# FuxiComputerVision/Nefii

Measured on AMD Instinct MI355X. Metric: training rays/sec (Step-2 material opt), higher is better.
Workload: dtype f16x3; 1 GPU; cfg3; parallelism=dp1, trace_tier=True, bracket_staged_eval=False, split_fp8=False, step_graph=False, cycle_batches=4, trace_prefetch=3, nonfinite_steps=0

## Files before the change

include/nefii_amd.h:

```cpp
#ifndef NEFII_AMD_H
#define NEFII_AMD_H

#include <stddef.h>
#include <stdint.h>

#ifdef __cplusplus
extern "C" {
#endif

#define NEFII_ABI_VERSION 18
#define NEFII_MAX_LAYERS 12
#define NEFII_TILE_ROWS 32
#define NEFII_MAX_WIDTH 512
#define NEFII_MAX_ENC 96
#define NEFII_MAX_LOBES 512

enum { NEFII_ACT_RELU = 0, NEFII_ACT_ELU = 1, NEFII_ACT_SOFTPLUS100 = 2 };
enum { NEFII_HEAD_NONE = 0, NEFII_HEAD_TANH01 = 1, NEFII_HEAD_POW2 = 2, NEFII_HEAD_SIGMOID = 3,
       NEFII_HEAD_RELU = 4, NEFII_HEAD_ABS = 5, NEFII_HEAD_RELU_INIT = 6 };
enum { NEFII_E_ARG = -1, NEFII_E_SHAPE = -2, NEFII_E_UNSUPPORTED = -3 };

typedef struct nefii_layer {
    int32_t k_x, k_e;
    int32_t n_out;
// ... 59 lines not shown
                        float scale, const float *gscale, float *dW, float *db, void *stream);

int nefii_mlp_h16_supported(const nefii_mlp *h_mlp);
int nefii_mlp_x0_width(const nefii_mlp *h_mlp);
int nefii_mlp_forward_f16h(const nefii_mlp *h_mlp, const float *in_a, const float *in_b, const float *in_c,
                           const float *feat, int64_t n, float *out, int out_stride, float *hidden_out, int hid_stride,
                           void *stash16, int stash_stride, float *z_last, void *x0_16, void *stream);
int nefii_mlp_backward_f16h(const nefii_mlp *h_mlp, const float *d_out, int out_stride, const void *stash16,
                            int stash_stride, const float *z_last, int64_t n, void *dz16, int dz_stride,
                            const float *scale, void *stream);
int nefii_mlp_wgrad_f16h(const void *dz16, int dz_stride, const void *x, int x_stride, int x_half, int64_t n, int n_out,
                         int k_in, float scale, const float *gscale, float *dW, float *db, void *stream);

#define NEFII_MAX_WGRAD_ITEMS 12
typedef struct nefii_wgrad_item {
    const void *dz16;
    const void *x;
    float *dW, *db;
    int32_t dz_stride, x_stride, x_half, n_out, k_in;
    float scale;
} nefii_wgrad_item;
int nefii_mlp_wgrad_f16h_batch(const nefii_wgrad_item *h_items, int n_items, int64_t n, const float *gscale, void *stream);

int nefii_encode_inputs(const nefii_mlp *h_mlp, const float *in_a, const float *in_b, const float *in_c,
                        const float *feat, int64_t n, float *out, int width, void *stream);

int nefii_sdf_value_grad(const nefii_mlp *h_mlp, const float *x, int64_t n, float *sdf_out, int out_stride,
                         float *feat_out, int feat_stride, float *grad_out, float *ws, void *stream);
size_t nefii_sdf_value_grad_workspace_bytes(const nefii_mlp *h_mlp, int64_t n);

typedef struct nefii_tracer_params {
    float object_bounding_sphere, sdf_threshold, line_search_step;
    int32_t line_step_iters, sphere_tracing_iters, n_steps, n_rootfind_steps;
    int32_t training;
    int32_t bisect_levels;
    int32_t precision;
    float coarse_tau;
    int32_t coarse_cap;
    int32_t minsdf_group;
    int32_t small_round;
    int32_t trace_tier;
    float tier_kappa;
    float tier_gate;
    float minsdf_lipschitz;
    int32_t unread_misses;
    int32_t split_fp8;
} nefii_tracer_params;
#define NEFII_TRACE_COUNTERS 14
#define NEFII_CNT_SINGLES 0
#define NEFII_CNT_DENSE_ROWS 1
#define NEFII_CNT_BISECT_RAYS 2
#define NEFII_CNT_BISECT_USED 3
#define NEFII_CNT_REFINED 4
#define NEFII_CNT_COARSE_WINDOWS 5
#define NEFII_CNT_SEARCHES 6
#define NEFII_CNT_BISECT_EVALS 7
#define NEFII_CNT_TAU_AUDIT 8
#define NEFII_CNT_COARSE_SINGLES 9
#define NEFII_CNT_REPEATS 10
#define NEFII_CNT_COARSE_SAMPLES 11
#define NEFII_CNT_LIP_AUDIT 12
#define NEFII_CNT_PROBES 13

size_t nefii_sdf_stream_bytes(const nefii_mlp *h_sdf);
int nefii_pack_sdf_stream(const nefii_mlp *h_sdf, void *w_stream, void *stream);

size_t nefii_mlp_stream_bytes(const nefii_mlp *h_mlp);
int nefii_pack_mlp_stream(const nefii_mlp *h_mlp, void *w_stream, void *stream);

int nefii_pack_linear_f16x3_bwd(const float *W, int n_out, int k_in, int x_src0, int x_len, int e_src0, int e_len,
                                float scale, void *w_bwd_f16x3, void *stream);

int nefii_sdf_eval(const nefii_mlp *h_sdf, const float *x, int64_t n, float *sdf_out, void *stream);
int nefii_sdf_eval_coarse(const nefii_mlp *h_sdf, const float *x, int64_t n, float *sdf_out, void *stream);
int nefii_sdf_coarse_supported(const nefii_mlp *h_sdf);
int nefii_sdf_eval_fp8corr(const nefii_mlp *h_sdf, const float *x, int64_t n, float *sdf_out, void *stream);
int nefii_sdf_fp8corr_supported(const nefii_mlp *h_sdf);

size_t nefii_trace_workspace_bytes(int64_t n_rays, const nefii_tracer_params *h_params);
int nefii_trace_max_rounds(const nefii_tracer_params *h_params);
int nefii_trace_rays(const nefii_mlp *h_sdf, const nefii_tracer_params *h_params,
                     const float *origins, const float *dirs, const uint8_t *object_mask, int64_t n_rays,
                     const float *lin_steps, const float *minsdf_steps,
                     float *out_points, uint8_t *out_hit, float *out_dists,
                     void *workspace, size_t workspace_bytes, int32_t *counters, void *stream);

int nefii_trace_rays_rounds(const nefii_mlp *h_sdf, const nefii_tracer_params *h_params,
                            const float *origins, const float *dirs, const uint8_t *object_mask, int64_t n_rays,
                            const float *lin_steps, const float *minsdf_steps,
                            float *out_points, uint8_t *out_hit, float *out_dists,
                            void *workspace, size_t workspace_bytes, int32_t *counters,
                            int round_begin, int round_end, void *stream);
int nefii_trace_rays_groups(const nefii_mlp *h_sdf, const nefii_tracer_params *h_params,
                            const float *origins, const float *dirs, const uint8_t *object_mask,
                            int n_groups, const int64_t *group_begin,
                            const float *lin_steps, const float *minsdf_steps,
                            float *out_points, uint8_t *out_hit, float *out_dists,
                            void *const *workspaces, const size_t *workspace_bytes, int32_t *counters,
                            int round_begin, int round_end, void *const *streams);

#define NEFII_BOUND_GRID_MAX 640
size_t nefii_sdf_bound_grid_workspace_bytes(int G);
int nefii_sdf_bound_grid_build(const nefii_mlp *h_sdf, int G, float radius, float tau, float L_floor, float safety,
                               void *out_cells, void *workspace, void *stream);
int nefii_trace_rays_rounds_grid(const nefii_mlp *h_sdf, const nefii_tracer_params *h_params,
                                 const float *origins, const float *dirs, const uint8_t *object_mask, int64_t n_rays,
                                 const float *lin_steps, const float *minsdf_steps,
                                 float *out_points, uint8_t *out_hit, float *out_dists,
                                 void *workspace, size_t workspace_bytes, int32_t *counters,
                                 int round_begin, int round_end, const void *cells, int G, void *stream);
int nefii_trace_rays_groups_grid(const nefii_mlp *h_sdf, const nefii_tracer_params *h_params,
                                 const float *origins, const float *dirs, const uint8_t *object_mask,
                                 int n_groups, const int64_t *group_begin,
                                 const float *lin_steps, const float *minsdf_steps,
                                 float *out_points, uint8_t *out_hit, float *out_dists,
                                 void *const *workspaces, const size_t *workspace_bytes, int32_t *counters,
                                 int round_begin, int round_end, const void *cells, int G, void *const *streams);

int nefii_sdf_bound_grid_build_vertices(const nefii_mlp *h_sdf, int G, float radius, float tau, float L_floor, float safety,
                                        void *out_cells, void *out_vertex_g, void *out_cell_l, void *workspace, void *stream);
int nefii_trace_rays_rounds_grid_vertices(const nefii_mlp *h_sdf, const nefii_tracer_params *h_params,
                                          const float *origins, const float *dirs, const uint8_t *object_mask, int64_t n_rays,
                                          const float *lin_steps, const float *minsdf_steps,
                                          float *out_points, uint8_t *out_hit, float *out_dists,
                                          void *workspace, size_t workspace_bytes, int32_t *counters,
                                          int round_begin, int round_end, const void *cells, int G,
                                          const void *vertex_g, const void *cell_l, void *stream);
int nefii_trace_rays_groups_grid_vertices(const nefii_mlp *h_sdf, const nefii_tracer_params *h_params,
                                          const float *origins, const float *dirs, const uint8_t *object_mask,
                                          int n_groups, const int64_t *group_begin,
                                          const float *lin_steps, const float *minsdf_steps,
                                          float *out_points, uint8_t *out_hit, float *out_dists,
                                          void *const *workspaces, const size_t *workspace_bytes, int32_t *counters,
                                          int round_begin, int round_end, const void *cells, int G,
                                          const void *vertex_g, const void *cell_l, void *const *streams);

int nefii_trace_rays_rounds_grid_training(const nefii_mlp *h_sdf, const nefii_tracer_params *h_params,
                                          const float *origins, const float *dirs, const uint8_t *object_mask, int64_t n_rays,
                                          const float *lin_steps, const float *minsdf_steps,
                                          float *out_points, uint8_t *out_hit, float *out_dists,
                                          void *workspace, size_t workspace_bytes, int32_t *counters,
                                          int round_begin, int round_end, const void *cells, int G,
                                          const void *vertex_g, const void *cell_l, int grid_training, void *stream);
int nefii_trace_rays_groups_grid_training(const nefii_mlp *h_sdf, const nefii_tracer_params *h_params,
                                          const float *origins, const float *dirs, const uint8_t *object_mask,
                                          int n_groups, const int64_t *group_begin,
                                          const float *lin_steps, const float *minsdf_steps,
                                          float *out_points, uint8_t *out_hit, float *out_dists,
                                          void *const *workspaces, const size_t *workspace_bytes, int32_t *counters,
                                          int round_begin, int round_end, const void *cells, int G,
                                          const void *vertex_g, const void *cell_l, int grid_training,
                                          void *const *streams);

int nefii_trace_profile_enable(int on);
int nefii_trace_profile_read(double *h_eval_ms, int *h_n_eval, double *h_span_ms);
int nefii_trace_profile_launches(float *h_ms, int cap);

int nefii_camera_rays(const float *uv, const float *pose, const float *intrinsics, int batch, int64_t samples,
                      float *out_dirs, float *out_origins, void *stream);


int nefii_sg_render_forward(const float *lgtSGs, int n_lobes, const float *specular, const float *roughness,
                            const float *albedo, const float *normal, const float *view, int64_t n,
                            float *rgb, float *spec_rgb, float *diff_rgb, void *stream);
int nefii_sg_render_backward(const float *lgtSGs, int n_lobes, const float *specular, const float *roughness,
                             const float *albedo, const float *normal, const float *view, int64_t n,
                             const float *d_rgb, const float *d_spec, const float *d_diff,
                             float *g_albedo, float *g_roughness, float *g_specular, float *g_lgtSGs, void *stream);

int nefii_env_radiance_forward(const float *lgtSGs, int n_lobes, const float *dirs, int64_t n, float eps,
                               float *rgb, void *stream);
int nefii_env_radiance_backward(const float *lgtSGs, int n_lobes, const float *dirs, int64_t n, float eps,
                                const float *d_rgb, float *g_lgtSGs, void *stream);

int64_t nefii_envfit_workspace_bytes(int64_t n, int n_lobes);
int nefii_envfit_loss_grad(const float *lgtSGs, int n_lobes, const float *dirs, const float *target, int64_t n, float eps,
                           void *workspace, float *loss, float *g_lgtSGs, float *rgb, void *stream);
int nefii_envfit_adam(float *lgtSGs, float *exp_avg, float *exp_avg_sq, int n_lobes, const float *dirs,
                      const float *target, int64_t n, float eps, double lr, double beta1, double beta2,
                      double adam_eps, int64_t step0, int iters, void *workspace, float *losses, void *stream);

int64_t nefii_mcubes_workspace_bytes(int nx, int ny, int nz);
int nefii_mcubes_count(const float *vol, int nx, int ny, int nz, float level, void *workspace, int64_t *counts,
                       void *stream);
int nefii_mcubes_emit(const float *vol, int nx, int ny, int nz, float level, float origin_x, float origin_y,
                      float origin_z, float spacing_x, float spacing_y, float spacing_z, void *workspace, float *verts,
                      int64_t max_verts, int *faces, int64_t max_tris, void *stream);

int nefii_mcubes_classify_bricks(const void *cells, int G, float radius, int nx, int ny, int nz, const double *frame,
                                 float level, int B, uint8_t *out_active, void *stream);
int nefii_mcubes_sparse_count(const float *vals, const int *slot_map, int n_slots, int nx, int ny, int nz, int B,
                              const int *active_list, int n_active, float level, int *counts, void *stream);
int nefii_mcubes_sparse_emit(const float *vals, const int *slot_map, int n_slots, int nx, int ny, int nz, int B,
                             const int *active_list, int n_active, float level, float origin_x, float origin_y,
                             float origin_z, float spacing_x, float spacing_y, float spacing_z, const int64_t *offsets,
                             int64_t *vert_keys, float *vert_pos, int64_t max_verts, int64_t *face_cell, int64_t *face_keys,
                             int64_t max_tris, void *stream);

int nefii_mis_sample(const float *lgtSGs, int n_lobes, const float *roughness, const float *normal, const float *view,
                     const float *uniforms, int64_t n, float *wi, float *own_pdf, float *pdf_table, void *stream);

int64_t nefii_envlight_table_bytes(int height, int width);
int nefii_envlight_build(const float *map, int height, int width, void *table, void *stream);
int nefii_envlight_mis_sample(const float *map, const void *table, int height, int width, int coord,
                              const float *roughness, const float *normal, const float *view, const float *uniforms,
                              int64_t n, float *wi, float *own_pdf, float *pdf_table, float *light, void *stream);
int nefii_envlight_radiance(const float *map, int height, int width, int coord, const float *dirs, int64_t n,
                            float *rgb, void *stream);
int nefii_envlight_pdf(const void *table, int height, int width, int coord, const float *dirs, int64_t n, float *pdf,
                       void *stream);

int nefii_envlight_bounce_sample(const float *map, const void *table, int height, int width, int coord,
                                 const float *specular, const float *roughness, const float *albedo,
                                 const float *normal, const float *view, const float *uniforms, int64_t m, float *wo,
                                 float *weight, float *mix_pdf, void *stream);

int nefii_envlight_mis_sample_rot(const float *map, const void *table, int height, int width, int coord,
                                  const float *rot, const int *rot_identity, int A, const float *roughness,
                                  const float *normal, const float *view, const float *uniforms, int64_t n, float *wi,
                                  float *own_pdf, float *pdf_table, float *light, void *stream);
int nefii_envlight_bounce_sample_rot(const float *map, const void *table, int height, int width, int coord,
                                     const float *rot, const int *rot_identity, int A, const int *rot_index,
                                     const float *specular, const float *roughness, const float *albedo,
                                     const float *normal, const float *view, const float *uniforms, int64_t m,
                                     float *wo, float *weight, float *mix_pdf, void *stream);
int nefii_envlight_radiance_rot(const float *map, int height, int width, int coord, const float *rot,
                                const int *rot_identity, int A, const int *rot_index, const float *dirs, int64_t n,
                                float *rgb, void *stream);
int nefii_envlight_pdf_rot(const void *table, int height, int width, int coord, const float *rot,
                           const int *rot_identity, int A, const int *rot_index, const float *dirs, int64_t n,
                           float *pdf, void *stream);

int nefii_denoise_atrous(const void *guides0, const void *guides1, const void *in, void *out, int n_signals, int height,
                         int width, int step, float sigma_n, float sigma_x, float sigma_c_level, void *stream);

int nefii_mesh_sdf_query(const double *node_box, int64_t n_leaves_pow2, const double *tris ,
                         int64_t n_tris, int leaf_size, const double *points, int64_t n_points, int want_sign, double *out,
                         void *stream);

int nefii_mesh_cc_init(int32_t *parent, int64_t n_verts, int32_t *flags, void *stream);
int nefii_mesh_cc_round(const int32_t *faces, int64_t n_faces, int32_t *parent, int64_t n_verts, int32_t *flags,
                        void *stream);

int nefii_mesh_cluster_quadrics(const float *verts, int64_t n_verts, const int32_t *faces, int64_t n_faces,
                                const int32_t *cluster, const int32_t *corners, const int64_t *seg, const double *centre,
                                int64_t n_clusters, double h, double eps, double clamp, float *pos, int32_t *flags,
                                void *stream);

int64_t nefii_image_metrics_workspace_bytes(int B, int H, int W, int C, int levels);
int nefii_image_metrics(const float *x, const float *y, int B, int H, int W, int C, int levels, const double *window,
                        double c1, double c2, void *workspace, double *stats, double *sq_err, void *stream);

int nefii_mc_shade_forward(const float *specular, const float *roughness, const float *albedo, const float *normal,
                           const float *view, const float *wi, const float *own_pdf, const float *pdf_table,
                           const float *light, const float *visibility, const float *indirect, int64_t n,
                           float *rgb, float *spec_rgb, float *diff_rgb, void *stream);
int nefii_mc_shade_backward(const float *specular, const float *roughness, const float *albedo, const float *normal,
                            const float *view, const float *wi, const float *own_pdf, const float *pdf_table,
                            const float *light, const float *visibility, const float *indirect, int64_t n,
                            const float *d_rgb, const float *d_spec, const float *d_diff, float *g_light,
                            float *g_indirect, float *g_albedo, float *g_roughness, float *g_specular, void *stream);

typedef struct nefii_loss_params {
    float idr_rgb_weight, sg_rgb_weight, mask_weight, alpha, normalsmooth_weight, background_rgb_weight;
    int32_t loss_type;
    int32_t env_loss_type;
    int32_t r_patch;
    int32_t reserved;
} nefii_loss_params;
int nefii_idr_loss(const nefii_loss_params *h_params, const float *idr_rgb, const float *sg_rgb, const float *rgb_gt,
                   const uint8_t *network_object_mask, const uint8_t *object_mask, const float *sdf_output,
                   const float *normals, int64_t n, float *losses, float *d_idr_rgb, float *d_sg_rgb, void *stream);

#define NEFII_PATCH_WINDOW 11
typedef struct nefii_patch_loss_params {
    float idr_ssim_weight, sg_ssim_weight, roughnesssmooth_weight;
    int32_t r_patch;
    float window[NEFII_PATCH_WINDOW];
    int32_t reserved;
} nefii_patch_loss_params;
int64_t nefii_idr_patch_loss_workspace_bytes(const nefii_patch_loss_params *h_params, int64_t n);
int nefii_idr_patch_loss(const nefii_patch_loss_params *h_params, const float *idr_rgb, const float *sg_rgb,
                         const float *rgb_gt, const uint8_t *network_object_mask, const uint8_t *object_mask,
                         const float *roughness, const float *normals, int64_t n, void *workspace, float *losses,
                         float *d_idr_rgb, float *d_sg_rgb, float *d_roughness, void *stream);

#define NEFII_MAX_ROW_BLOCKS 12
typedef struct nefii_row_block {
    const float *src;
    float *dst;
    int32_t cols;
    int32_t src_row_stride;
    float fill;
    int32_t reserved;
} nefii_row_block;
int nefii_assemble_rows(const nefii_row_block *h_blocks, int n_blocks, const int64_t *where, int64_t n_src, int64_t rows,
                        void *stream);
int nefii_gather_rows(const nefii_row_block *h_blocks, int n_blocks, const int64_t *where, int64_t n_src, int64_t rows,
                      void *stream);

int nefii_prepare_hits(const float *points, const float *ray_dirs, const float *grad, const float *feat_src, int feat_cols,
                       const int64_t *where, int64_t n, int64_t rows, float *pts_out, float *view_out, float *nrm_out,
                       float *feat_out, void *stream);

int nefii_material_head_global(const float *rough_param, const float *spec_param, int n_spec, int fake_rough, int fake_spec,
                               float *rough_out, float *spec_out, void *stream);
// ... 12 lines not shown
```

nefii_amd/_lib.py:

```python
import ctypes
import os

HERE = os.path.dirname(os.path.abspath(__file__))
LIB_PATH = os.environ.get('NEFII_LIB_PATH', os.path.join(HERE, 'csrc', 'libnefii_hip.so'))

MAX_LAYERS = 12
TILE_ROWS = 32
MAX_WIDTH = 512
MAX_ENC = 96
ABI_VERSION = 18
TRACE_COUNTERS = 14
(CNT_SINGLES, CNT_DENSE_ROWS, CNT_BISECT_RAYS, CNT_BISECT_USED, CNT_REFINED, CNT_COARSE_WINDOWS, CNT_SEARCHES, CNT_BISECT_EVALS,
 CNT_TAU_AUDIT, CNT_COARSE_SINGLES, CNT_REPEATS, CNT_COARSE_SAMPLES, CNT_LIP_AUDIT, CNT_PROBES) = range(TRACE_COUNTERS)
CNT_WORK = [CNT_SINGLES, CNT_DENSE_ROWS, CNT_BISECT_RAYS, CNT_REFINED, CNT_COARSE_WINDOWS, CNT_COARSE_SINGLES, CNT_COARSE_SAMPLES]
CNT_MAXIMA = [CNT_TAU_AUDIT, CNT_LIP_AUDIT]
TRACE_WS_FLOAT_ARRAYS = 13
TRACE_ITER_SHIFT = 20

ACT_RELU, ACT_ELU, ACT_SOFTPLUS100 = 0, 1, 2
HEAD_NONE, HEAD_TANH01, HEAD_POW2, HEAD_SIGMOID, HEAD_RELU, HEAD_ABS, HEAD_RELU_INIT = range(7)

c_float_p = ctypes.c_void_p


class Layer(ctypes.Structure):
    _fields_ = [('k_x', ctypes.c_int32), ('k_e', ctypes.c_int32), ('n_out', ctypes.c_int32),
                ('n_pad', ctypes.c_int32), ('w_fwd', ctypes.c_void_p), ('w_bwd', ctypes.c_void_p),
                ('bias', ctypes.c_void_p), ('w_f16x3', ctypes.c_void_p), ('w_bwd_f16x3', ctypes.c_void_p)]


class Mlp(ctypes.Structure):
    _fields_ = [('n_layers', ctypes.c_int32), ('act', ctypes.c_int32), ('head', ctypes.c_int32),
                ('enc_freqs', ctypes.c_int32 * 3), ('feat_width', ctypes.c_int32), ('reserved', ctypes.c_int32),
                ('w_stream', ctypes.c_void_p), ('layer', Layer * MAX_LAYERS)]


class TracerParams(ctypes.Structure):
    _fields_ = [('object_bounding_sphere', ctypes.c_float), ('sdf_threshold', ctypes.c_float),
                ('line_search_step', ctypes.c_float), ('line_step_iters', ctypes.c_int32),
                ('sphere_tracing_iters', ctypes.c_int32), ('n_steps', ctypes.c_int32),
                ('n_rootfind_steps', ctypes.c_int32), ('training', ctypes.c_int32), ('bisect_levels', ctypes.c_int32),
                ('precision', ctypes.c_int32), ('coarse_tau', ctypes.c_float), ('coarse_cap', ctypes.c_int32),
                ('minsdf_group', ctypes.c_int32), ('small_round', ctypes.c_int32), ('trace_tier', ctypes.c_int32),
                ('tier_kappa', ctypes.c_float), ('tier_gate', ctypes.c_float), ('minsdf_lipschitz', ctypes.c_float),
                ('unread_misses', ctypes.c_int32), ('split_fp8', ctypes.c_int32)]


class PackSource(ctypes.Structure):
    _fields_ = [('W', ctypes.c_void_p), ('bias', ctypes.c_void_p), ('n_out', ctypes.c_int32), ('k_in', ctypes.c_int32),
                ('x_src0', ctypes.c_int32), ('x_len', ctypes.c_int32), ('e_src0', ctypes.c_int32), ('e_len', ctypes.c_int32),
                ('scale', ctypes.c_float), ('skip_f32', ctypes.c_int32)]


class WgradItem(ctypes.Structure):
    _fields_ = [('dz16', ctypes.c_void_p), ('x', ctypes.c_void_p), ('dW', ctypes.c_void_p), ('db', ctypes.c_void_p),
                ('dz_stride', ctypes.c_int32), ('x_stride', ctypes.c_int32), ('x_half', ctypes.c_int32),
                ('n_out', ctypes.c_int32), ('k_in', ctypes.c_int32), ('scale', ctypes.c_float)]


MAX_WGRAD_ITEMS = 12


class RowBlock(ctypes.Structure):
    _fields_ = [('src', ctypes.c_void_p), ('dst', ctypes.c_void_p), ('cols', ctypes.c_int32), ('src_row_stride', ctypes.c_int32),
                ('fill', ctypes.c_float), ('reserved', ctypes.c_int32)]


MAX_ROW_BLOCKS = 12


class LossParams(ctypes.Structure):
    _fields_ = [('idr_rgb_weight', ctypes.c_float), ('sg_rgb_weight', ctypes.c_float), ('mask_weight', ctypes.c_float),
                ('alpha', ctypes.c_float), ('normalsmooth_weight', ctypes.c_float),
                ('background_rgb_weight', ctypes.c_float), ('loss_type', ctypes.c_int32),
                ('env_loss_type', ctypes.c_int32), ('r_patch', ctypes.c_int32), ('reserved', ctypes.c_int32)]


PATCH_WINDOW = 11


class PatchLossParams(ctypes.Structure):
    _fields_ = [('idr_ssim_weight', ctypes.c_float), ('sg_ssim_weight', ctypes.c_float),
                ('roughnesssmooth_weight', ctypes.c_float), ('r_patch', ctypes.c_int32),
                ('window', ctypes.c_float * PATCH_WINDOW), ('reserved', ctypes.c_int32)]


P = ctypes.c_void_p
I = ctypes.c_int
I64 = ctypes.c_int64
F = ctypes.c_float
D = ctypes.c_double

SIGNATURES = {
    'nefii_abi_version': (I, []),
    'nefii_padded_width': (I, [I]),
    'nefii_pack_linear': (I, [P, P, I, I, I, I, I, I, F, P, P, P, P]),
    'nefii_pack_linear_f16x3': (I, [P, I, I, I, I, I, I, F, P, P]),
    'nefii_pack_linear_f16x3_bwd': (I, [P, I, I, I, I, I, I, F, P, P]),
    'nefii_pack_mlp': (I, [ctypes.POINTER(Mlp), ctypes.POINTER(PackSource), P]),
    'nefii_mlp_forward': (I, [ctypes.POINTER(Mlp), P, P, P, P, I64, P, I, P, I, P, I, P]),
    'nefii_mlp_backward': (I, [ctypes.POINTER(Mlp), P, I, P, I, I64, P, I, P]),
    'nefii_mlp_wgrad': (I, [P, I, P, I, I64, I, I, F, P, P, P]),
    'nefii_mlp_forward_f16': (I, [ctypes.POINTER(Mlp), P, P, P, P, I64, P, I, P, I, P, I, I, P]),
    'nefii_mlp_grad_scale': (I, [P, I64, P, P]),
    'nefii_mlp_grad_scale_head': (I, [P, I, P, I, I64, I, I, P, P]),
    'nefii_mlp_backward_f16': (I, [ctypes.POINTER(Mlp), P, I, P, I, I64, P, I, P, P]),
    'nefii_mlp_wgrad_f16': (I, [P, I, P, I, I64, I, I, F, P, P, P, P]),
    'nefii_mlp_h16_supported': (I, [ctypes.POINTER(Mlp)]),
    'nefii_mlp_x0_width': (I, [ctypes.POINTER(Mlp)]),
    'nefii_mlp_forward_f16h': (I, [ctypes.POINTER(Mlp), P, P, P, P, I64, P, I, P, I, P, I, P, P, P]),
    'nefii_mlp_backward_f16h': (I, [ctypes.POINTER(Mlp), P, I, P, I, P, I64, P, I, P, P]),
    'nefii_mlp_wgrad_f16h': (I, [P, I, P, I, I, I64, I, I, F, P, P, P, P]),
    'nefii_mlp_wgrad_f16h_batch': (I, [ctypes.POINTER(WgradItem), I, I64, P, P]),
    'nefii_encode_inputs': (I, [ctypes.POINTER(Mlp), P, P, P, P, I64, P, I, P]),
    'nefii_sdf_value_grad': (I, [ctypes.POINTER(Mlp), P, I64, P, I, P, I, P, P, P]),
    'nefii_sdf_value_grad_workspace_bytes': (ctypes.c_size_t, [ctypes.POINTER(Mlp), I64]),
    'nefii_sdf_stream_bytes': (ctypes.c_size_t, [ctypes.POINTER(Mlp)]),
    'nefii_pack_sdf_stream': (I, [ctypes.POINTER(Mlp), P, P]),
    'nefii_mlp_stream_bytes': (ctypes.c_size_t, [ctypes.POINTER(Mlp)]),
    'nefii_pack_mlp_stream': (I, [ctypes.POINTER(Mlp), P, P]),
    'nefii_sdf_eval': (I, [ctypes.POINTER(Mlp), P, I64, P, P]),
    'nefii_sdf_eval_coarse': (I, [ctypes.POINTER(Mlp), P, I64, P, P]),
    'nefii_sdf_coarse_supported': (I, [ctypes.POINTER(Mlp)]),
    'nefii_sdf_eval_fp8corr': (I, [ctypes.POINTER(Mlp), P, I64, P, P]),
    'nefii_sdf_fp8corr_supported': (I, [ctypes.POINTER(Mlp)]),
    'nefii_trace_workspace_bytes': (ctypes.c_size_t, [I64, ctypes.POINTER(TracerParams)]),
    'nefii_trace_max_rounds': (I, [ctypes.POINTER(TracerParams)]),
    'nefii_trace_rays': (I, [ctypes.POINTER(Mlp), ctypes.POINTER(TracerParams), P, P, P, I64, P, P, P, P, P, P,
                             ctypes.c_size_t, P, P]),
    'nefii_trace_rays_rounds': (I, [ctypes.POINTER(Mlp), ctypes.POINTER(TracerParams), P, P, P, I64, P, P, P, P, P, P,
                                    ctypes.c_size_t, P, I, I, P]),
    'nefii_trace_rays_groups': (I, [ctypes.POINTER(Mlp), ctypes.POINTER(TracerParams), P, P, P, I, P, P, P, P, P, P, P, P,
                                    P, I, I, P]),
    'nefii_sdf_bound_grid_workspace_bytes': (ctypes.c_size_t, [I]),
    'nefii_sdf_bound_grid_build': (I, [ctypes.POINTER(Mlp), I, F, F, F, F, P, P, P]),
    'nefii_trace_rays_rounds_grid': (I, [ctypes.POINTER(Mlp), ctypes.POINTER(TracerParams), P, P, P, I64, P, P, P, P, P, P,
                                         ctypes.c_size_t, P, I, I, P, I, P]),
    'nefii_trace_rays_groups_grid': (I, [ctypes.POINTER(Mlp), ctypes.POINTER(TracerParams), P, P, P, I, P, P, P, P, P, P, P, P,
                                         P, I, I, P, I, P]),
    'nefii_sdf_bound_grid_build_vertices': (I, [ctypes.POINTER(Mlp), I, F, F, F, F, P, P, P, P, P]),
    'nefii_trace_rays_rounds_grid_vertices': (I, [ctypes.POINTER(Mlp), ctypes.POINTER(TracerParams), P, P, P, I64, P, P, P, P, P,
                                                  P, ctypes.c_size_t, P, I, I, P, I, P, P, P]),
    'nefii_trace_rays_groups_grid_vertices': (I, [ctypes.POINTER(Mlp), ctypes.POINTER(TracerParams), P, P, P, I, P, P, P, P, P,
                                                  P, P, P, P, I, I, P, I, P, P, P]),
    'nefii_trace_rays_rounds_grid_training': (I, [ctypes.POINTER(Mlp), ctypes.POINTER(TracerParams), P, P, P, I64, P, P, P, P, P,
                                                  P, ctypes.c_size_t, P, I, I, P, I, P, P, I, P]),
    'nefii_trace_rays_groups_grid_training': (I, [ctypes.POINTER(Mlp), ctypes.POINTER(TracerParams), P, P, P, I, P, P, P, P, P,
                                                  P, P, P, P, I, I, P, I, P, P, I, P]),
    'nefii_trace_profile_enable': (I, [I]),
    'nefii_trace_profile_read': (I, [ctypes.POINTER(ctypes.c_double), ctypes.POINTER(I), ctypes.POINTER(ctypes.c_double)]),
    'nefii_trace_profile_launches': (I, [ctypes.POINTER(ctypes.c_float), I]),
    'nefii_idr_loss': (I, [ctypes.POINTER(LossParams), P, P, P, P, P, P, P, I64, P, P, P, P]),
    'nefii_idr_patch_loss_workspace_bytes': (I64, [ctypes.POINTER(PatchLossParams), I64]),
    'nefii_idr_patch_loss': (I, [ctypes.POINTER(PatchLossParams), P, P, P, P, P, P, P, I64, P, P, P, P, P, P]),
    'nefii_camera_rays': (I, [P, P, P, I, I64, P, P, P]),
    'nefii_assemble_rows': (I, [ctypes.POINTER(RowBlock), I, P, I64, I64, P]),
    'nefii_gather_rows': (I, [ctypes.POINTER(RowBlock), I, P, I64, I64, P]),
    'nefii_prepare_hits': (I, [P, P, P, P, I, P, I64, I64, P, P, P, P, P]),
    'nefii_material_head_global': (I, [P, P, I, I, I, P, P, P]),
    'nefii_material_head_global_backward': (I, [P, P, I, I, I, P, P, P, P, P]),
    'nefii_sg_render_forward': (I, [P, I, P, P, P, P, P, I64, P, P, P, P]),
    'nefii_sg_render_backward': (I, [P, I, P, P, P, P, P, I64, P, P, P, P, P, P, P, P]),
    'nefii_env_radiance_forward': (I, [P, I, P, I64, F, P, P]),
    'nefii_env_radiance_backward': (I, [P, I, P, I64, F, P, P, P]),
    'nefii_envfit_workspace_bytes': (I64, [I64, I]),
    'nefii_envfit_loss_grad': (I, [P, I, P, P, I64, F, P, P, P, P, P]),
    'nefii_envfit_adam': (I, [P, P, P, I, P, P, I64, F, D, D, D, D, I64, I, P, P, P]),
    'nefii_mcubes_workspace_bytes': (I64, [I, I, I]),
    'nefii_mcubes_count': (I, [P, I, I, I, F, P, P, P]),
    'nefii_mcubes_emit': (I, [P, I, I, I, F, F, F, F, F, F, F, P, P, I64, P, I64, P]),
    'nefii_mcubes_classify_bricks': (I, [P, I, F, I, I, I, ctypes.POINTER(D), F, I, P, P]),
    'nefii_mcubes_sparse_count': (I, [P, P, I, I, I, I, I, P, I, F, P, P]),
    'nefii_mcubes_sparse_emit': (I, [P, P, I, I, I, I, I, P, I, F, F, F, F, F, F, F, P, P, P, I64, P, P, I64, P]),
    'nefii_mis_sample': (I, [P, I, P, P, P, P, I64, P, P, P, P]),
    'nefii_envlight_table_bytes': (I64, [I, I]),
    'nefii_envlight_build': (I, [P, I, I, P, P]),
    'nefii_envlight_mis_sample': (I, [P, P, I, I, I, P, P, P, P, I64, P, P, P, P, P]),
    'nefii_envlight_bounce_sample': (I, [P, P, I, I, I, P, P, P, P, P, P, I64, P, P, P, P]),
    'nefii_envlight_radiance': (I, [P, I, I, I, P, I64, P, P]),
    'nefii_envlight_pdf': (I, [P, I, I, I, P, I64, P, P]),
    'nefii_envlight_mis_sample_rot': (I, [P, P, I, I, I, P, P, I, P, P, P, P, I64, P, P, P, P, P]),
    'nefii_envlight_bounce_sample_rot': (I, [P, P, I, I, I, P, P, I, P, P, P, P, P, P, P, I64, P, P, P, P]),
    'nefii_envlight_radiance_rot': (I, [P, I, I, I, P, P, I, P, P, I64, P, P]),
    'nefii_envlight_pdf_rot': (I, [P, I, I, I, P, P, I, P, P, I64, P, P]),
    'nefii_denoise_atrous': (I, [P, P, P, P, I, I, I, I, F, F, F, P]),
    'nefii_image_metrics_workspace_bytes': (I64, [I, I, I, I, I]),
    'nefii_image_metrics': (I, [P, P, I, I, I, I, I, ctypes.POINTER(D), D, D, P, P, P, P]),
    'nefii_mesh_sdf_query': (I, [P, I64, P, I64, I, P, I64, I, P, P]),
    'nefii_mesh_cc_init': (I, [P, I64, P, P]),
    'nefii_mesh_cc_round': (I, [P, I64, P, I64, P, P]),
    'nefii_mesh_cluster_quadrics': (I, [P, I64, P, I64, P, P, P, P, I64, D, D, D, P, P, P]),
    'nefii_mc_shade_forward': (I, [P] * 11 + [I64, P, P, P, P]),
    'nefii_mc_shade_backward': (I, [P] * 11 + [I64] + [P] * 9),
    'nefii_mfma_sustained_probe': (I, [I, ctypes.POINTER(ctypes.c_float), ctypes.POINTER(ctypes.c_double), P]),
    'nefii_mfma_sustained_probe_chains': (I, [I, I, ctypes.POINTER(ctypes.c_float), ctypes.POINTER(ctypes.c_double), P]),
}

_lib = None


class NefiiLibraryError(RuntimeError):
    pass


def lib():
    global _lib
    if _lib is not None:
        return _lib
    if not os.path.exists(LIB_PATH):
        raise NefiiLibraryError(
            'libnefii_hip.so is not built (%s missing). Run `python -m nefii_amd.build`. '
            'There is no CPU/PyTorch fallback for the hot path.' % LIB_PATH)
    import torch
    try:
        handle = ctypes.CDLL(LIB_PATH)
    except OSError as e:
        raise NefiiLibraryError('cannot load %s: %s' % (LIB_PATH, e))
    for name, (res, args) in SIGNATURES.items():
        try:
            fn = getattr(handle, name)
        except AttributeError:
            raise NefiiLibraryError('%s does not export %s' % (LIB_PATH, name))
        fn.restype = res
        fn.argtypes = args
    if handle.nefii_abi_version() != ABI_VERSION:
        raise NefiiLibraryError('ABI version mismatch')
    _lib = handle
    return _lib


def check(rc, what):
    if rc != 0:
        raise RuntimeError('%s failed with status %d (%s)' % (
            what, rc, {-1: 'bad argument', -2: 'bad shape', -3: 'unsupported'}.get(rc, 'hipError_t')))
```

nefii_amd/csrc/nefii_tracer.hip:

```cpp
#include <cstdlib>
#include <vector>

#include "mlp_tile.h"
#include "hip_check.h"

using namespace nefii;

namespace {

enum Phase : int { PH_DONE = 0, PH_TRACE = 1, PH_SAMPLER = 2, PH_BISECT = 3, PH_MINSDF = 4, PH_SAMPLER_C = 5, PH_MINSDF_C = 6,
                   PH_SAMPLER_X = 7 };
constexpr int PH_POST = 100, PH_WAIT = -1;
constexpr int NCNT = NEFII_TRACE_COUNTERS;
constexpr int NEAR_PROBES = 6;
enum Kind : int { Q_START = 0, Q_END = 1, Q_MID = 2 };
enum Walk : int { WALK_NONE = 0, WALK_BEGIN = 1, WALK_AUDIT = 2 };

constexpr int TRACE_WS_FLOAT_ARRAYS = 13, TRACE_ITER_SHIFT = 20;
struct RayState {
    float *t_s, *t_e, *cur_s, *cur_e, *nxt_s, *nxt_e, *t_min, *t_max, *res_s, *res_e, *lo, *hi, *mid;
    int *flags;
    float *big;
    unsigned *singles;
    unsigned *dense;
    unsigned *tri;
    unsigned *cdense;
    unsigned *refine;
    unsigned *csingles;
    int *block_live;
    unsigned *crefine;
    unsigned char *ord;
};
constexpr int CREF_CAP = 76;

constexpr int F_PHASE = 0x7;
constexpr int F_LIVE_S = 1 << 3, F_LIVE_E = 1 << 4, F_PEND_S = 1 << 5, F_PEND_E = 1 << 6;
constexpr int F_STEPPED = 1 << 7;
constexpr int F_SPH = 1 << 8, F_SAMP = 1 << 9, F_HIT = 1 << 10;
constexpr int F_OWN = 1 << 11;
constexpr int F_IT_SHIFT = 12, F_IT_MASK = 0xFF;
constexpr int F_K_SHIFT = TRACE_ITER_SHIFT, F_K_MASK = 0xF;
constexpr int F_WIN_SHIFT = 24, F_WIN_MASK = 0x7;
enum SamplerWin : int {
    SW_WHOLE_ROW = 0,
    SW_WINDOW_1 = 1, SW_WINDOW_2 = 2, SW_WINDOW_3 = 3, SW_WINDOW_4 = 4,
    SW_STAGE1 = 5, SW_STAGE2 = 6,
    SW_GRID = 7
};
enum MinSdfWin : int {
    MW_ROW_IN = 0,
    MW_SECOND = 1,
    MW_STAGE1 = 2, MW_STAGE2 = 3,
    MW_ENTER = 4,
    MW_SHARED = 5
};
__device__ __forceinline__ int win_of(int fl) { return (fl >> F_WIN_SHIFT) & F_WIN_MASK; }
__device__ __forceinline__ int with_win(int fl, int w) { return (fl & ~(F_WIN_MASK << F_WIN_SHIFT)) | (w << F_WIN_SHIFT); }
constexpr int CWIN_STAGE1 = 4;
constexpr int F_CRS_S = 1 << 27, F_CRS_E = 1 << 28, F_AUD_S = 1 << 29, F_AUD_E = 1 << 30;
__host__ __device__ __forceinline__ int coarse_window(int n_steps) { return (n_steps + 3) >> 2; }

__device__ __forceinline__ float fmul(float a, float b) { return __fmul_rn(a, b); }
__device__ __forceinline__ float fadd(float a, float b) { return __fadd_rn(a, b); }
__device__ __forceinline__ float fsub(float a, float b) { return __fsub_rn(a, b); }

struct Params {
    nefii_tracer_params p;
    int64_t n;
    const float *o, *d;
    const uint8_t *obj;
    const float *lin, *steps;
    float *out_pts, *out_dist;
    uint8_t *out_hit;
    int *counters;
    int levels, tri_nodes;
    float tau;
    int cap;
    int chunk;
    float chunk_gate;
    int window;
    float tier_band;
    float tier_gate;
    float lip;
    int share;
    int stage_bracket;
    int miss_argmin;
    const unsigned *cells;
    int grid_n;
    float grid_inv_h;
    const unsigned short *vert_g, *cell_l;
    float grid_h;
    int grid_training;
    int walk_wave;
    RayState s;
};

__host__ __device__ __forceinline__ int stage1_count(int ns) { return coarse_window(ns); }
__host__ __device__ __forceinline__ int stage1_pos(int ns, int j) { return (j * (ns - 1)) / (stage1_count(ns) - 1); }
__device__ __forceinline__ bool staged_bracket(const Params &P, int64_t r) {
    return P.lip > 0.f && P.stage_bracket && (!P.p.training || P.obj[r] == 0);
}
__device__ __forceinline__ int minsdf_row(const Params &P, int64_t r) {
    const int g = P.p.minsdf_group;
    return g > 0 ? (int)(r / g) : 0;
}

__device__ __forceinline__ float minsdf_step(const Params &P, int64_t r, int i) {
    const int g = P.p.minsdf_group;
    return P.steps[(g > 0 ? (r / g) * (int64_t)P.p.n_steps : 0) + i];
}

struct Emit {
    bool qs, qe;
    bool cs, ce;
    bool qt, qd;
    int nc, cwin;
    unsigned dense_which;
    int consumed;
    int n_alg;
    int n_ref;
    unsigned cmask[4];
    int n_rep;
    bool ref_coarse;
    int walk, walk_from;
    __device__ __forceinline__ void mark(int i) {
#pragma unroll
        for (int w = 0; w < 4; ++w) cmask[w] |= (i >> 5) == w ? 1u << (i & 31) : 0u;
    }
    __device__ __forceinline__ bool marked(int i) const {
        unsigned word = 0u;
#pragma unroll
        for (int w = 0; w < 4; ++w) word = (i >> 5) == w ? cmask[w] : word;
        return (word >> (i & 31)) & 1u;
    }
    __device__ __forceinline__ void clear_marks() { cmask[0] = cmask[1] = cmask[2] = cmask[3] = 0u; }
};
enum Total : int { T_SINGLES, T_DENSE, T_TRI, T_CONSUMED, T_REFINE, T_CWINDOWS, T_ALG, T_CSINGLES, T_REP, T_CREFINE, N_TOTALS };
enum List : int { L_SINGLES, L_DENSE, L_TRI, L_REFINE, L_CDENSE, L_CSINGLES, L_CREFINE, N_LISTS };

__device__ __forceinline__ void append_queries(const Params &P, int round, unsigned ray, const Emit &e) {
    __shared__ int wtot[N_TOTALS][4];
    __shared__ int base[N_LISTS];
    const bool qs = e.qs && !e.cs, qe = e.qe && !e.ce, qcs = e.qs && e.cs, qce = e.qe && e.ce;
    const int nc = e.nc, n_ref = e.n_ref;
    const bool ref_coarse = e.ref_coarse;
    const int lane = threadIdx.x & 63, wave = threadIdx.x >> 6;
    const unsigned long long bs = __ballot(qs), be = __ballot(qe), bt = __ballot(e.qt), bd = __ballot(e.qd);
    const unsigned long long bcs = __ballot(qcs), bce = __ballot(qce);
    const unsigned long long lt = (1ull << lane) - 1ull;
    int cons = e.consumed, alg = e.n_alg, rep = e.n_rep;
#pragma unroll
    for (int o = 32; o > 0; o >>= 1) cons += __shfl_xor(cons, o), alg += __shfl_xor(alg, o), rep += __shfl_xor(rep, o);
    int incl = ref_coarse ? 0 : n_ref;
    int incl2 = ref_coarse ? n_ref : 0;
#pragma unroll
    for (int o = 1; o < 64; o <<= 1) {
        const int t = __shfl_up(incl, o), t2 = __shfl_up(incl2, o);
        if (lane >= o) incl += t, incl2 += t2;
    }
    const int wref = __shfl(incl, 63), wref2 = __shfl(incl2, 63);
    int cincl = nc;
#pragma unroll
    for (int o = 1; o < 64; o <<= 1) {
        const int t = __shfl_up(cincl, o);
        if (lane >= o) cincl += t;
    }
    const int wcoarse = __shfl(cincl, 63);
    if (lane == 0) {
        wtot[T_SINGLES][wave] = __popcll(bs) + __popcll(be);
        wtot[T_DENSE][wave] = __popcll(bd);
        wtot[T_TRI][wave] = __popcll(bt);
        wtot[T_CONSUMED][wave] = cons;
        wtot[T_REFINE][wave] = wref;
        wtot[T_CWINDOWS][wave] = wcoarse;
        wtot[T_ALG][wave] = alg;
        wtot[T_CSINGLES][wave] = __popcll(bcs) + __popcll(bce);
        wtot[T_REP][wave] = rep;
        wtot[T_CREFINE][wave] = wref2;
    }
    __syncthreads();
    if (threadIdx.x == 0) {
        int t[N_TOTALS];
        for (int i = 0; i < N_TOTALS; ++i) t[i] = wtot[i][0] + wtot[i][1] + wtot[i][2] + wtot[i][3];
        int *cnt = P.counters + round * NCNT;
        base[L_SINGLES] = t[T_SINGLES] ? atomicAdd(&cnt[NEFII_CNT_SINGLES], t[T_SINGLES]) : 0;
        base[L_DENSE] = t[T_DENSE] ? atomicAdd(&cnt[NEFII_CNT_DENSE_ROWS], t[T_DENSE]) : 0;
        base[L_TRI] = t[T_TRI] ? atomicAdd(&cnt[NEFII_CNT_BISECT_RAYS], t[T_TRI]) : 0;
        if (t[T_CONSUMED]) atomicAdd(&cnt[NEFII_CNT_BISECT_USED], t[T_CONSUMED]);
        base[L_REFINE] = t[T_REFINE] ? atomicAdd(&cnt[NEFII_CNT_REFINED], t[T_REFINE]) : 0;
        base[L_CDENSE] = t[T_CWINDOWS] ? atomicAdd(&cnt[NEFII_CNT_COARSE_WINDOWS], t[T_CWINDOWS]) : 0;
        if (t[T_ALG]) atomicAdd(&cnt[NEFII_CNT_SEARCHES], t[T_ALG]);
        if (t[T_TRI]) atomicAdd(&cnt[NEFII_CNT_BISECT_EVALS], t[T_TRI] * P.tri_nodes);
        base[L_CSINGLES] = t[T_CSINGLES] ? atomicAdd(&cnt[NEFII_CNT_COARSE_SINGLES], t[T_CSINGLES]) : 0;
        if (t[T_REP]) atomicAdd(&cnt[NEFII_CNT_REPEATS], t[T_REP]);
        base[L_CREFINE] = t[T_CREFINE] ? atomicAdd(&cnt[NEFII_CNT_COARSE_SAMPLES], t[T_CREFINE]) : 0;
    }
    __syncthreads();
    int off_s = base[L_SINGLES], off_d = base[L_DENSE], off_t = base[L_TRI], off_r = base[L_REFINE], off_c = base[L_CDENSE],
        off_cs = base[L_CSINGLES], off_r2 = base[L_CREFINE];
    for (int w = 0; w < wave; ++w) {
        off_r2 += wtot[T_CREFINE][w];
        off_s += wtot[T_SINGLES][w];
        off_d += wtot[T_DENSE][w];
        off_t += wtot[T_TRI][w];
        off_r += wtot[T_REFINE][w];
        off_c += wtot[T_CWINDOWS][w];
        off_cs += wtot[T_CSINGLES][w];
    }
    if (qs) P.s.singles[off_s + __popcll(bs & lt)] = (ray << 2) | Q_START;
    if (qe) P.s.singles[off_s + __popcll(bs) + __popcll(be & lt)] = (ray << 2) | Q_END;
    if (qcs) P.s.csingles[off_cs + __popcll(bcs & lt)] = (ray << 2) | Q_START;
    if (qce) P.s.csingles[off_cs + __popcll(bcs) + __popcll(bce & lt)] = (ray << 2) | Q_END;
    if (e.qd) P.s.dense[off_d + __popcll(bd & lt)] = (ray << 1) | e.dense_which;
    if (e.qt) P.s.tri[off_t + __popcll(bt & lt)] = ray;
    for (int k = 0; k < nc; ++k)
        P.s.cdense[off_c + cincl - nc + k] = ((unsigned)(e.cwin + k) << 29) | (ray << 1) | e.dense_which;
    if (n_ref > 0) {
        size_t o = ref_coarse ? (size_t)off_r2 + incl2 - n_ref : (size_t)off_r + incl - n_ref;
        unsigned *list = ref_coarse ? P.s.crefine : P.s.refine;
#pragma unroll
        for (int w = 0; w < 4; ++w) {
            unsigned mbits = e.cmask[w];
            while (mbits) {
                const int bit = __ffs(mbits) - 1;
                mbits &= mbits - 1;
                list[o++] = (ray << 7) | (unsigned)(32 * w + bit);
            }
        }
    }
    __syncthreads();
}

__device__ __forceinline__ float tri_depth(float lo, float hi, int j) {
    const unsigned k = (unsigned)j + 1u;
    const int level = 31 - __clz(k);
    float mid = fmul(fadd(lo, hi), 0.5f);
    for (int b = level - 1; b >= 0; --b) {
        if ((k >> b) & 1u) lo = mid; else hi = mid;
        mid = fmul(fadd(lo, hi), 0.5f);
    }
    return mid;
}

__device__ __forceinline__ void finish(const Params &P, int64_t r, float dist, bool hit) {
    const float ox = P.o[r * 3], oy = P.o[r * 3 + 1], oz = P.o[r * 3 + 2];
    const float dx = P.d[r * 3], dy = P.d[r * 3 + 1], dz = P.d[r * 3 + 2];
    P.out_dist[r] = dist;
    P.out_hit[r] = hit ? 1 : 0;
    P.out_pts[r * 3] = fadd(ox, fmul(dist, dx));
    P.out_pts[r * 3 + 1] = fadd(oy, fmul(dist, dy));
    P.out_pts[r * 3 + 2] = fadd(oz, fmul(dist, dz));
}

__global__ __launch_bounds__(128) void minsdf_order_kernel(Params P) {
    const int ns = P.p.n_steps, i = threadIdx.x;
    if (i >= ns) return;
    const float *st = P.steps + (size_t)blockIdx.x * ns;
    const float si = st[i];
    int rank = 0;
    for (int j = 0; j < ns; ++j) {
        const float sj = st[j];
        rank += (sj < si || (sj == si && j < i)) ? 1 : 0;
    }
    P.s.ord[(size_t)blockIdx.x * ns + rank] = (unsigned char)i;
}


__device__ __forceinline__ int init_ray(const Params &P, int64_t r, int round, int &fl, Emit &e) {
    const bool tier = P.tier_band > 0.f;
    const float ox = P.o[r * 3], oy = P.o[r * 3 + 1], oz = P.o[r * 3 + 2];
    const float dx = P.d[r * 3], dy = P.d[r * 3 + 1], dz = P.d[r * 3 + 2];
    const float b = fadd(fadd(fmul(dx, ox), fmul(dy, oy)), fmul(dz, oz));
    const float nrm = sqrtf(fadd(fadd(fmul(ox, ox), fmul(oy, oy)), fmul(oz, oz)));
    const float rad = P.p.object_bounding_sphere;
    const float under = fsub(fmul(b, b), fsub(fmul(nrm, nrm), fmul(rad, rad)));
    const bool sph = under > 0.f;
    float t0 = 0.f, t1 = 0.f;
    if (sph) {
        const float sq = sqrtf(under);
        t0 = fmaxf(fsub(-sq, b), 0.01f);
        t1 = fmaxf(fsub(sq, b), 0.01f);
    }
    P.s.t_s[r] = t0;
    P.s.t_e[r] = t1;
    P.s.t_min[r] = t0;
    P.s.t_max[r] = t1;
    P.s.nxt_s[r] = 0.f;
    P.s.nxt_e[r] = 0.f;
    P.s.cur_s[r] = 0.f;
    P.s.cur_e[r] = 0.f;
    fl = PH_TRACE;
    if (!sph) return PH_TRACE;
    fl |= F_SPH | F_LIVE_S | F_LIVE_E | F_PEND_S | F_PEND_E;
    e.qs = e.qe = true;
    e.cs = tier && t0 > 0.01f;
    e.ce = tier && t1 > 0.01f;
    fl |= (e.cs ? F_CRS_S : 0) | (e.ce ? F_CRS_E : 0);
    P.s.flags[r] = fl;
    return PH_WAIT;
}

__device__ __forceinline__ void begin_stage1(const Params &P, int64_t r, int from, int stage_code, int &fl, Emit &e) {
    float *v = P.s.big + (size_t)r * P.p.n_steps;
    for (int i = from; i < P.p.n_steps; ++i) v[i] = __builtin_inff();
    e.nc = 1;
    e.cwin = CWIN_STAGE1;
    fl = with_win(fl, stage_code);
}

__device__ __forceinline__ bool grid_bounds(const Params &P, int64_t r, float t, float &lo, float &hi) {
    const float rad = P.p.object_bounding_sphere, g = (float)P.grid_n;
    const float ox = P.o[r * 3], oy = P.o[r * 3 + 1], oz = P.o[r * 3 + 2];
    const float dx = P.d[r * 3], dy = P.d[r * 3 + 1], dz = P.d[r * 3 + 2];
    const float fx = fmul(fadd(fadd(ox, fmul(t, dx)), rad), P.grid_inv_h);
    const float fy = fmul(fadd(fadd(oy, fmul(t, dy)), rad), P.grid_inv_h);
    const float fz = fmul(fadd(fadd(oz, fmul(t, dz)), rad), P.grid_inv_h);
    lo = -__builtin_inff(), hi = __builtin_inff();
    if (!(fx >= 0.f && fx < g && fy >= 0.f && fy < g && fz >= 0.f && fz < g)) return false;
    const unsigned w = P.cells[((size_t)(int)fx * P.grid_n + (size_t)(int)fy) * P.grid_n + (size_t)(int)fz];
    lo = (float)__builtin_bit_cast(_Float16, (unsigned short)(w & 0xFFFFu));
    hi = (float)__builtin_bit_cast(_Float16, (unsigned short)(w >> 16));
    return true;
}

__device__ __forceinline__ bool grid_corner_bounds(const Params &P, int64_t r, float t, float &lo, float &hi) {
    const float rad = P.p.object_bounding_sphere, g = (float)P.grid_n;
    const float ox = P.o[r * 3], oy = P.o[r * 3 + 1], oz = P.o[r * 3 + 2];
    const float dx = P.d[r * 3], dy = P.d[r * 3 + 1], dz = P.d[r * 3 + 2];
    const float px = fadd(ox, fmul(t, dx)), py = fadd(oy, fmul(t, dy)), pz = fadd(oz, fmul(t, dz));
    const float fx = fmul(fadd(px, rad), P.grid_inv_h), fy = fmul(fadd(py, rad), P.grid_inv_h), fz = fmul(fadd(pz, rad), P.grid_inv_h);
    lo = -__builtin_inff(), hi = __builtin_inff();
    if (!(fx >= 0.f && fx < g && fy >= 0.f && fy < g && fz >= 0.f && fz < g)) return false;
    const int ci = (int)fx, cj = (int)fy, ck = (int)fz;
    const size_t V = (size_t)P.grid_n + 1;
    const float L = (float)__builtin_bit_cast(_Float16, P.cell_l[((size_t)ci * P.grid_n + (size_t)cj) * P.grid_n + (size_t)ck]);
    unsigned short gc[8];
#pragma unroll
    for (int c = 0; c < 4; ++c) {
        const unsigned short *row = P.vert_g + ((size_t)(ci + (c >> 1)) * V + (size_t)(cj + (c & 1))) * V + (size_t)ck;
        gc[2 * c] = row[0];
        gc[2 * c + 1] = row[1];
    }
    float ex2[2], ey2[2], ez2[2];
#pragma unroll
    for (int a = 0; a < 2; ++a) {
        const float ex = fsub(px, fadd(-rad, fmul((float)(ci + a), P.grid_h)));
        const float ey = fsub(py, fadd(-rad, fmul((float)(cj + a), P.grid_h)));
        const float ez = fsub(pz, fadd(-rad, fmul((float)(ck + a), P.grid_h)));
        ex2[a] = fmul(ex, ex), ey2[a] = fmul(ey, ey), ez2[a] = fmul(ez, ez);
    }
#pragma unroll
    for (int c = 0; c < 8; ++c) {
        const float v = (float)__builtin_bit_cast(_Float16, gc[c]);
        const float dist = fadd(sqrtf(fadd(fadd(ex2[c >> 2], ey2[(c >> 1) & 1]), ez2[c & 1])), 1e-6f);
        const float reach = fadd(fmul(L, dist), fadd(fmul(fabsf(v), 0x1p-11f), 0x1p-25f));
        lo = fmaxf(lo, fsub(v, reach));
        hi = fminf(hi, fadd(v, reach));
    }
    lo = fsub(lo, P.tau);
    hi = fadd(hi, P.tau);
    return true;
}

__device__ __forceinline__ void begin_grid_bracket(const Params &P, int64_t r, int round, int from, int &fl, Emit &e) {
    const int ns = P.p.n_steps;
    float *v = P.s.big + (size_t)r * ns;
    const float a = P.s.t_s[r], rng = fsub(P.s.t_e[r], a);
    const bool obj = P.obj[r] != 0;
    int j1 = ns;
    float U = __builtin_inff(), lo0 = 0.f;
    for (int i = 0; i < ns; ++i) {
        float lo, hi;
        if (i < from)
            lo = hi = v[i];
        else
            grid_bounds(P, r, fadd(a, fmul(P.lin[i], rng)), lo, hi);
        if (hi < -P.tau && j1 == ns) j1 = i;
        U = fminf(U, hi);
        if (i == 0) lo0 = lo;
        if (i >= from) v[i] = lo;
    }
    bool front_only = obj && j1 < ns && lo0 > 0.f;
    bool sign_only = front_only || !P.miss_argmin;
    float lim = sign_only ? 0.f : fmaxf(0.f, fadd(U, P.tau));
    int last = front_only ? j1 : ns - 1;
    if (P.vert_g) {
        for (int i = from; i <= last; ++i) {
            const float lb = v[i];
            if (fsub(lb, 1e-6f) > lim) continue;
            float lo, hi;
            if (!grid_corner_bounds(P, r, fadd(a, fmul(P.lin[i], rng)), lo, hi)) continue;
            v[i] = fmaxf(lb, lo);
            if (i == 0) lo0 = v[i];
            U = fminf(U, hi);
            if (hi < -P.tau && i < j1) {
                j1 = i;
                if (obj && lo0 > 0.f) break;
            }
        }
        front_only = obj && j1 < ns && lo0 > 0.f;
        sign_only = front_only || !P.miss_argmin;
        lim = sign_only ? 0.f : fmaxf(0.f, fadd(U, P.tau));
        last = front_only ? j1 : ns - 1;
    }
    int k = 0, n_near = 0, probe = -1;
    unsigned probe_h = ~0u;
    for (int i = from; i < ns; ++i) {
        const float lb = v[i];
        v[i] = __builtin_inff();
        if (i > last) continue;
        if (!(fsub(lb, 1e-6f) > lim)) {
            e.mark(i);
            ++k;
        } else if (n_near < NEAR_PROBES && !(fsub(lb, 1e-6f) > fadd(lim, fmul(2.f, P.tau)))) {
            e.mark(i);
            ++k, ++n_near;
        } else {
            const unsigned h = ((unsigned)r * 2654435761u) ^ ((unsigned)(i + 1) * 0x9E3779B1u);
            const unsigned hh = (h ^ (h >> 15)) * 0x85EBCA6Bu;
            if (hh < probe_h) probe_h = hh, probe = i;
        }
    }
    if (probe >= 0) {
        e.mark(probe);
        ++k, ++n_near;
    }
    if (n_near > 0) atomicAdd(P.counters + round * NCNT + NEFII_CNT_PROBES, n_near);
    if (k > 0 && k <= CREF_CAP) {
        e.n_ref = k;
        e.ref_coarse = true;
        fl = with_win(fl, SW_GRID);
    } else {
        e.clear_marks();
        e.nc = 4;
    }
}

__device__ __forceinline__ void grid_audit(const Params &P, int64_t r, int round) {
    const int ns = P.p.n_steps;
    const float *v = P.s.big + (size_t)r * ns;
    const float a = P.s.t_s[r], rng = fsub(P.s.t_e[r], a);
    float worst = 0.f;
    int n_corner = 0;
    for (int i = 0; i < ns; ++i) {
        if (!(v[i] < __builtin_inff())) continue;
// ... 93 lines not shown
    }
    const float lim2 = fadd(lim, fmul(2.f, P.tau));
    bool act[2] = {false, false}, surv[2] = {false, false}, near[2] = {false, false};
    unsigned long long S[2] = {0ull, 0ull}, N[2] = {0ull, 0ull}, Sel[2] = {0ull, 0ull};
#pragma unroll
    for (int p = 0; p < 2; ++p) {
        if (p && !two) continue;
        const int i = 64 * p + lane;
        const float x = fsub(lb[p], 1e-6f);
        act[p] = in[p] && i >= from && i <= last;
        surv[p] = act[p] && !(x > lim);
        near[p] = act[p] && !surv[p] && !(x > lim2);
        S[p] = __ballot(surv[p]);
        N[p] = __ballot(near[p]);
        if (in[p] && i >= from) v[i] = inf;
    }
    unsigned hh[2] = {~0u, ~0u};
#pragma unroll
    for (int p = 0; p < 2; ++p) {
        if (p && !two) continue;
        const int i = 64 * p + lane;
        const int before = (p ? __popcll(N[0]) : 0) + __popcll(N[p] & lt);
        const bool sel = near[p] && before < NEAR_PROBES;
        Sel[p] = __ballot(sel);
        if (act[p] && !surv[p] && !sel) {
            const unsigned h = ((unsigned)r * 2654435761u) ^ ((unsigned)(i + 1) * 0x9E3779B1u);
            hh[p] = (h ^ (h >> 15)) * 0x85EBCA6Bu;
        }
    }
    const unsigned hmin = wave_umin(hh[0] < hh[1] ? hh[0] : hh[1]);
    const unsigned long long P0 = __ballot(hh[0] == hmin), P1 = __ballot(hh[1] == hmin);
    const int probe = hmin != ~0u ? first_sample(P0, P1, -1) : -1;
    GridMarks g;
    g.m0 = S[0] | Sel[0] | (probe >= 0 && probe < 64 ? 1ull << probe : 0ull);
    g.m1 = S[1] | Sel[1] | (probe >= 64 ? 1ull << (probe - 64) : 0ull);
    g.k = __popcll(g.m0) + __popcll(g.m1);
    const int n_near = __popcll(Sel[0]) + __popcll(Sel[1]) + (probe >= 0 ? 1 : 0);
    if (lane == 0 && n_near > 0) atomicAdd(P.counters + round * NCNT + NEFII_CNT_PROBES, n_near);
    return g;
}

__device__ __forceinline__ void wave_grid_audit(const Params &P, int64_t r, int round) {
    const int ns = P.p.n_steps, lane = threadIdx.x & 63;
    const unsigned long long lt = (1ull << lane) - 1ull;
    const float *v = P.s.big + (size_t)r * ns;
    const float a = P.s.t_s[r], rng = fsub(P.s.t_e[r], a);
    const bool two = ns > 64;
    float x[2] = {0.f, 0.f}, t[2] = {0.f, 0.f}, lo[2] = {0.f, 0.f}, hi[2] = {0.f, 0.f};
    bool el[2] = {false, false};
    unsigned long long E[2] = {0ull, 0ull};
#pragma unroll
    for (int p = 0; p < 2; ++p) {
        if (p && !two) continue;
        const int i = 64 * p + lane;
        if (i < ns) x[p] = v[i];
        if (i < ns && x[p] < __builtin_inff()) {
            t[p] = fadd(a, fmul(P.lin[i], rng));
            el[p] = grid_bounds(P, r, t[p], lo[p], hi[p]);
        }
        E[p] = __ballot(el[p]);
    }
    float worst = 0.f;
#pragma unroll
    for (int p = 0; p < 2; ++p) {
        if (p && !two) continue;
        if (!el[p]) continue;
        const int before = (p ? __popcll(E[0]) : 0) + __popcll(E[p] & lt);
        if (P.vert_g && before < CREF_CAP) {
            float lo_c, hi_c;
            grid_corner_bounds(P, r, t[p], lo_c, hi_c);
            lo[p] = fmaxf(lo[p], lo_c), hi[p] = fminf(hi[p], hi_c);
        }
        worst = fmaxf(worst, fmaxf(fsub(fsub(lo[p], P.tau), x[p]), fsub(x[p], fadd(hi[p], P.tau))));
    }
    worst = wave_fmax(worst);
    if (lane == 0 && worst > 0.f) atomicMax(P.counters + round * NCNT + NEFII_CNT_LIP_AUDIT, __float_as_int(worst));
}

__device__ __forceinline__ void serve_grid_walks(const Params &P, int64_t r, int round, int &fl, Emit &e) {
    const int lane = threadIdx.x & 63;
    unsigned long long pending = __ballot(e.walk != WALK_NONE);
    while (pending) {
        const int src = __ffsll(pending) - 1;
        pending &= pending - 1;
        const int64_t rr = __builtin_amdgcn_readfirstlane((int)(r - lane) + src);
        const int kind = __builtin_amdgcn_readfirstlane(__shfl(e.walk, src));
        const int from = __builtin_amdgcn_readfirstlane(__shfl(e.walk_from, src));
        if (kind == WALK_AUDIT) {
            wave_grid_audit(P, rr, round);
            continue;
        }
        const GridMarks g = wave_grid_bracket(P, rr, round, from);
        if (lane == src) {
            if (g.k > 0 && g.k <= CREF_CAP) {
                e.cmask[0] = (unsigned)g.m0, e.cmask[1] = (unsigned)(g.m0 >> 32);
                e.cmask[2] = (unsigned)g.m1, e.cmask[3] = (unsigned)(g.m1 >> 32);
                e.n_ref = g.k;
                e.ref_coarse = true;
                fl = with_win(fl, SW_GRID);
            } else {
                e.clear_marks();
                e.nc = 4;
            }
            P.s.flags[r] = fl;
        }
    }
    e.walk = WALK_NONE;
}

__device__ __forceinline__ void begin_coarse_bracket(const Params &P, int64_t r, int round, int from, bool in_mask, int &fl, Emit &e) {
    if (P.cells && P.lip > 0.f && P.stage_bracket && (!P.p.training || (P.grid_training && in_mask))) {
        if (P.walk_wave)
            e.walk = WALK_BEGIN, e.walk_from = from;
        else
            begin_grid_bracket(P, r, round, from, fl, e);
    } else if (staged_bracket(P, r)) {
        begin_stage1(P, r, from, SW_STAGE1, fl, e);
    } else if ((P.window & 1) && in_mask) {
        e.nc = 1;
        fl = with_win(fl, SW_WINDOW_1);
    } else {
        e.nc = 4;
    }
}

__device__ __forceinline__ int end_trace(const Params &P, int64_t r, int round, int &fl, Emit &e, float t_s, float t_e,
                                         float cur_s, float cur_e, bool live_s, int it) {
    const bool coarse = P.tau > 0.f;
    const bool hit = t_s < t_e;
    fl = (fl & F_SPH) | (hit ? F_HIT : 0) | (live_s ? F_SAMP : 0) | ((it & F_K_MASK) << F_K_SHIFT);
    P.s.t_s[r] = t_s;
    P.s.t_e[r] = t_e;
    if (!live_s) {
        P.s.mid[r] = t_s;
        return PH_POST;
    }
    const bool go_coarse = coarse && 0.5f * (cur_s + cur_e + (t_e - t_s)) > 3.f * P.tau;
    if (go_coarse && P.chunk > 0 && P.obj[r] != 0 &&
        cur_s <= P.chunk_gate * (float)(P.chunk - 1) * (t_e - t_s) / (float)(P.p.n_steps - 1)) {
        fl |= PH_SAMPLER_X;
        e.n_ref = P.chunk;
        e.cmask[0] = (1u << P.chunk) - 1u;
    } else {
        fl |= go_coarse ? PH_SAMPLER_C : PH_SAMPLER;
        e.qd = !go_coarse;
        if (go_coarse) begin_coarse_bracket(P, r, round, 0, P.obj[r] != 0, fl, e);
    }
    e.n_alg = 1;
    e.dense_which = 0;
    P.s.flags[r] = fl;
    return PH_WAIT;
}

__device__ __forceinline__ int step_trace(const Params &P, int64_t r, int round, int &fl, Emit &e) {
    const nefii_tracer_params &tp = P.p;
    const bool tier = P.tier_band > 0.f;
    const float thr = tp.sdf_threshold;
    float t_s = P.s.t_s[r], t_e = P.s.t_e[r];
    float cur_s = P.s.cur_s[r], cur_e = P.s.cur_e[r];
    float nxt_s = P.s.nxt_s[r], nxt_e = P.s.nxt_e[r];
    bool live_s = fl & F_LIVE_S, live_e = fl & F_LIVE_E;
    int it = (fl >> F_IT_SHIFT) & F_IT_MASK, k = (fl >> F_K_SHIFT) & F_K_MASK;
    if (fl & F_PEND_S) nxt_s = P.s.res_s[r];
    if (fl & F_PEND_E) nxt_e = P.s.res_e[r];
    fl &= ~(F_AUD_S | F_AUD_E);
    const bool rep_s = (fl & F_PEND_S) && (fl & F_CRS_S) && !(fabsf(nxt_s) > P.tier_band);
    const bool rep_e = (fl & F_PEND_E) && (fl & F_CRS_E) && !(fabsf(nxt_e) > P.tier_band);
    if (rep_s || rep_e) {
        if (rep_s) e.qs = true, fl = (fl & ~F_CRS_S) | F_AUD_S, ++e.n_rep;
        if (rep_e) e.qe = true, fl = (fl & ~F_CRS_E) | F_AUD_E, ++e.n_rep;
        P.s.flags[r] = fl;
        return PH_WAIT;
    }
    bool wait = false;
    fl &= ~(F_CRS_S | F_CRS_E);
    if (fl & F_STEPPED) {
        const bool bad_s = nxt_s < 0.f, bad_e = nxt_e < 0.f;
        if ((bad_s || bad_e) && k < tp.line_step_iters) {
            const float back = (1.f - tp.line_search_step) / (float)(1 << k);
            fl &= ~(F_PEND_S | F_PEND_E);
            if (bad_s) {
                t_s = fsub(t_s, fmul(back, cur_s));
                e.qs = true;
                e.cs = tier && back * cur_s > P.tier_gate;
                fl |= F_PEND_S | (e.cs ? F_CRS_S : 0);
            }
            if (bad_e) {
                t_e = fadd(t_e, fmul(back, cur_e));
                e.qe = true;
                e.ce = tier && back * cur_e > P.tier_gate;
                fl |= F_PEND_E | (e.ce ? F_CRS_E : 0);
            }
            ++k;
            wait = true;
        } else {
            live_s = live_s && (t_s < t_e);
            live_e = live_e && (t_s < t_e);
        }
    }
    if (!wait) {
        cur_s = live_s ? nxt_s : 0.f;
        if (cur_s <= thr) cur_s = 0.f;
        cur_e = live_e ? nxt_e : 0.f;
        if (cur_e <= thr) cur_e = 0.f;
        live_s = live_s && (cur_s > thr);
        live_e = live_e && (cur_e > thr);
        if (it == tp.sphere_tracing_iters || !(live_s || live_e)) return end_trace(P, r, round, fl, e, t_s, t_e, cur_s, cur_e, live_s, it);
        ++it;
        t_s = fadd(t_s, cur_s);
        t_e = fsub(t_e, cur_e);
        nxt_s = 0.f;
        nxt_e = 0.f;
        k = 0;
        fl &= ~(F_PEND_S | F_PEND_E);
        if (live_s) {
            e.qs = true;
            e.cs = tier && cur_s > P.tier_gate;
            fl |= F_PEND_S | (e.cs ? F_CRS_S : 0);
        }
        if (live_e) {
            e.qe = true;
            e.ce = tier && cur_e > P.tier_gate;
            fl |= F_PEND_E | (e.ce ? F_CRS_E : 0);
        }
        fl |= F_STEPPED;
    }
    fl &= ~(F_LIVE_S | F_LIVE_E | (F_IT_MASK << F_IT_SHIFT) | (F_K_MASK << F_K_SHIFT));
    fl |= (live_s ? F_LIVE_S : 0) | (live_e ? F_LIVE_E : 0) | (it << F_IT_SHIFT) | (k << F_K_SHIFT);
    P.s.t_s[r] = t_s;
    P.s.t_e[r] = t_e;
    P.s.cur_s[r] = cur_s;
    P.s.cur_e[r] = cur_e;
    P.s.nxt_s[r] = nxt_s;
    P.s.nxt_e[r] = nxt_e;
    P.s.flags[r] = fl;
    return PH_WAIT;
}

__device__ __forceinline__ int sampler_leading(const Params &P, int64_t r, int round, int &fl, Emit &e) {
    const int ns = P.p.n_steps;
    float *v = P.s.big + (size_t)r * ns;
    int ind = -1;
    for (int i = 0; i < P.chunk; ++i)
        if (v[i] < 0.f && ind < 0) ind = i;
    if (ind >= 1) {
        for (int i = P.chunk; i < ns; ++i) v[i] = 3.0e38f;
        return PH_SAMPLER;
    }
    fl = (fl & ~F_PHASE) | PH_SAMPLER_C;
    begin_coarse_bracket(P, r, round, P.chunk, true, fl, e);
    e.dense_which = 0;
    P.s.flags[r] = fl;
    return PH_WAIT;
}

template <typename Search>
__device__ __forceinline__ bool staged_walk(const Params &P, int64_t r, int round, int &fl, Emit &e, const float *v, float Llen,
                                            bool stage1, const Search &S) {
    const int ns = P.p.n_steps;
    int *cnt = P.counters + round * NCNT;
    int ja = 0, k = 0, n_near = 0;
    float worst = 0.f;
    int probe = -1;
    unsigned probe_h = ~0u;
    for (int kk = 1; kk < ns - 1; ++kk) {
        if (kk == stage1_pos(ns, ja + 1)) {
            ++ja;
            continue;
        }
        const int ia = S.sample(stage1_pos(ns, ja)), ib = S.sample(stage1_pos(ns, ja + 1)), is = S.sample(kk);
        const float sa = S.depth(ia), sb = S.depth(ib), ss = S.depth(is);
        const float lb = fsub(fmaxf(fsub(v[ia], fmul(Llen, fsub(ss, sa))), fsub(v[ib], fmul(Llen, fsub(sb, ss)))), P.tau);
        if (stage1) {
            if (S.skip(kk, v)) continue;
            if (!(fsub(lb, 1e-6f) > S.lim)) {
                e.mark(is);
                ++k;
            } else if (n_near < NEAR_PROBES && !(fsub(lb, 1e-6f) > fadd(S.lim, fmul(2.f, P.tau)))) {
                e.mark(is);
                ++k, ++n_near;
            } else {
                const unsigned h = ((unsigned)r * 2654435761u) ^ ((unsigned)(kk + 1) * 0x9E3779B1u);
                const unsigned hh = (h ^ (h >> 15)) * 0x85EBCA6Bu;
                if (hh < probe_h) probe_h = hh, probe = is;
            }
        } else if (v[is] < __builtin_inff()) {
            worst = fmaxf(worst, fsub(fsub(lb, P.tau), v[is]));
        }
    }
    fl = with_win(fl, 0);
    if (stage1 && probe >= 0) {
        e.mark(probe);
        ++k, ++n_near;
    }
    if (stage1 && n_near > 0) atomicAdd(cnt + NEFII_CNT_PROBES, n_near);
    if (stage1 && k > 0) {
        if (k <= CREF_CAP) {
            e.n_ref = k;
            e.ref_coarse = true;
            fl = with_win(fl, Search::STAGE2);
        } else {
            e.clear_marks();
            e.nc = 4;
            e.dense_which = Search::WHICH;
        }
        P.s.flags[r] = fl;
        return true;
    }
    if (worst > 0.f) atomicMax(cnt + NEFII_CNT_LIP_AUDIT, __float_as_int(worst));
    e.clear_marks();
    return false;
}

struct BracketSearch {
    const float *lin;
    float lim;
    int last;
    static constexpr int STAGE2 = SW_STAGE2;
    static constexpr unsigned WHICH = 0;
    __device__ __forceinline__ int sample(int k) const { return k; }
    __device__ __forceinline__ float depth(int i) const { return lin[i]; }
    __device__ __forceinline__ bool skip(int k, const float *v) const { return k >= last || v[k] < __builtin_inff(); }
};

struct MinSdfSearch {
    const Params &P;
    int64_t r;
    const unsigned char *ord;
    float lim;
    static constexpr int STAGE2 = MW_STAGE2;
    static constexpr unsigned WHICH = 1;
    __device__ __forceinline__ int sample(int k) const { return ord[k]; }
    __device__ __forceinline__ float depth(int i) const { return minsdf_step(P, r, i); }
    __device__ __forceinline__ bool skip(int, const float *) const { return false; }
};

__device__ __forceinline__ int sampler_staged(const Params &P, int64_t r, int round, int &fl, Emit &e) {
    const int ns = P.p.n_steps, n1 = stage1_count(ns);
    const float *v = P.s.big + (size_t)r * ns;
    if (win_of(fl) == SW_GRID) {
        if (P.walk_wave)
            e.walk = WALK_AUDIT;
        else
            grid_audit(P, r, round);
        fl = with_win(fl, SW_WHOLE_ROW);
        return PH_SAMPLER_C;
    }
    const float Llen = fmul(P.lip, fsub(P.s.t_e[r], P.s.t_s[r]));
    const bool obj = P.obj[r] != 0;
    float best = __builtin_inff();
    int j1 = ns;
    for (int j = 0; j < n1; ++j) {
        const int i = stage1_pos(ns, j);
        best = fminf(best, v[i]);
        if (v[i] < -P.tau && j1 == ns) j1 = i;
    }
    const bool front_only = obj && j1 < ns && !(v[0] < P.tau);
    const bool sign_only = front_only || !P.miss_argmin;
    const BracketSearch S = {P.lin, sign_only ? 0.f : fmaxf(0.f, fadd(best, P.tau)), front_only ? j1 : ns - 1};
    return staged_walk(P, r, round, fl, e, v, Llen, win_of(fl) == SW_STAGE1, S) ? PH_WAIT : PH_SAMPLER_C;
}

__device__ __forceinline__ int sampler_windows(const Params &P, int64_t r, int round, int &fl, Emit &e) {
// ... 212 lines not shown
    float U = __builtin_inff();
    if (first)
        for (int i = 0; i < ns; ++i)
            if (vc[i] < __builtin_inff()) U = fminf(U, fadd(vc[i], slack(minsdf_step(P, r, i))));
    float lo_a = -__builtin_inff(), s_a = 0.f, lo_b = -__builtin_inff(), s_b = 1.f, worst = 0.f;
    int kb = -1, k = 0, n_near = 0, probe = -1;
    unsigned probe_h = ~0u;
    for (int kk = 0; kk < ns; ++kk) {
        const int is = ord[kk];
        const float ss = minsdf_step(P, r, is);
        float lb;
        if (vc[is] < __builtin_inff()) {
            lb = lo_a = fsub(vc[is], slack(ss));
            s_a = ss;
        } else {
            if (kb < kk) {
                lo_b = -__builtin_inff();
                for (kb = kk + 1; kb < ns; ++kb) {
                    const int ib = ord[kb];
                    if (vc[ib] < __builtin_inff()) {
                        s_b = minsdf_step(P, r, ib);
                        lo_b = fsub(vc[ib], slack(s_b));
                        break;
                    }
                }
            }
            lb = fmaxf(fsub(lo_a, fmul(Llen, fsub(ss, s_a))), fsub(lo_b, fmul(Llen, fsub(s_b, ss))));
        }
        if (!first) {
            if (v[is] < __builtin_inff()) worst = fmaxf(worst, fsub(fsub(lb, P.tau), v[is]));
        } else if (!(fsub(lb, 1e-6f) > U)) {
            e.mark(is);
            ++k;
        } else if (n_near < NEAR_PROBES && !(fsub(lb, 1e-6f) > fadd(U, fmul(2.f, P.tau)))) {
            e.mark(is);
            ++k, ++n_near;
        } else {
            const unsigned h = ((unsigned)r * 2654435761u) ^ ((unsigned)(kk + 1) * 0x9E3779B1u);
            const unsigned hh = (h ^ (h >> 15)) * 0x85EBCA6Bu;
            if (hh < probe_h) probe_h = hh, probe = is;
        }
    }
    if (!first) {
        if (worst > 0.f) atomicMax(cnt + NEFII_CNT_LIP_AUDIT, __float_as_int(worst));
        return true;
    }
    if (probe >= 0) {
        e.mark(probe);
        ++k, ++n_near;
    }
    if (k > stage1_count(ns)) {
        e.clear_marks();
        return false;
    }
    if (n_near > 0) atomicAdd(cnt + NEFII_CNT_PROBES, n_near);
    e.n_ref = k;
    e.ref_coarse = true;
    return true;
}

__device__ __forceinline__ int minsdf_share(const Params &P, int64_t r, int round, int ph, int fl0, int &fl, Emit &e) {
    const int lane = threadIdx.x & 63;
    const int p0 = fl0 & F_PHASE;
    const bool own = fl0 & F_OWN, stage1 = p0 == PH_MINSDF_C && win_of(fl0) == MW_STAGE1;
    const bool ready = own && (p0 == PH_DONE || p0 == PH_MINSDF || (p0 == PH_MINSDF_C && !stage1));
    const bool want = (fl & F_PHASE) == PH_MINSDF_C && win_of(fl) == MW_ENTER;
    unsigned long long mine = ~0ull;
    const int g = P.p.minsdf_group;
    if (g > 0) {
        const int64_t base = r - lane, head = (r / g) * g - base, tail = head + g - 1;
        const int lo = head > 0 ? (int)head : 0, hi = tail < 63 ? (int)tail : 63;
        mine = (hi >= 63 ? ~0ull : (1ull << (hi + 1)) - 1ull) & ~((1ull << lo) - 1ull);
    }
    const unsigned long long donors = __ballot(ready) & mine, busy = __ballot(own && stage1) & mine;
    const unsigned long long free_lanes = __ballot(want && !donors && !busy) & mine;
    if (!want) return ph;
    bool search = !donors && !busy && __ffsll(free_lanes) - 1 == lane;
    if (donors) {
        const int c = __ffsll(donors) - 1;
        if (shared_walk(P, r, r - lane + c, round, e, true))
            fl = (with_win(fl, MW_SHARED) & ~(F_IT_MASK << F_IT_SHIFT)) | (c << F_IT_SHIFT);
        else
            search = true;
    }
    if (search) {
        e.nc = 1;
        e.cwin = CWIN_STAGE1;
        fl = with_win(fl, MW_STAGE1) | F_OWN;
    }
    e.dense_which = 1;
    P.s.flags[r] = fl;
    return PH_WAIT;
}

__device__ __forceinline__ int minsdf_shared(const Params &P, int64_t r, int round, int &fl, Emit &e) {
    const int c = (fl >> F_IT_SHIFT) & F_IT_MASK;
    shared_walk(P, r, r - (threadIdx.x & 63) + c, round, e, false);
    fl = with_win(fl, MW_ROW_IN) & ~(F_IT_MASK << F_IT_SHIFT);
    return PH_MINSDF_C;
}

__device__ __forceinline__ int minsdf_second_stage(const Params &P, int64_t r, int round, int &fl, Emit &e) {
    const int ns = P.p.n_steps;
    const float *v = P.s.big + (size_t)r * ns;
    const int a = (fl >> F_IT_SHIFT) & F_IT_MASK;
    const float lim = v[a] + P.tau;
    int k = 0;
    for (int i = 0; i < ns; ++i)
        if (i != a && v[i] <= lim) {
            e.mark(i);
            ++k;
        }
    fl = with_win(fl, MW_ROW_IN) & ~(F_IT_MASK << F_IT_SHIFT);
    if (k == 0) return PH_MINSDF;
    if (k <= P.cap) e.n_ref = k; else e.qd = true;
    e.dense_which = 1;
    fl = (fl & ~F_PHASE) | PH_MINSDF;
    P.s.flags[r] = fl;
    return PH_WAIT;
}

__device__ __forceinline__ int minsdf_coarse(const Params &P, int64_t r, int round, int &fl, Emit &e) {
    const int ns = P.p.n_steps;
    const float *v = P.s.big + (size_t)r * ns;
    float vmin = v[0];
    int amin = 0;
    for (int i = 1; i < ns; ++i)
        if (v[i] < vmin) {
            vmin = v[i];
            amin = i;
        }
    const float lim = vmin + 2.f * P.tau;
    int k = 0;
    for (int i = 0; i < ns; ++i)
        if (v[i] <= lim) {
            e.mark(i);
            ++k;
        }
    if (k <= 1) return PH_MINSDF;
    if ((P.window & 2) && k >= 4 && ns <= 256) {
        e.clear_marks();
        e.mark(amin);
        e.n_ref = 1;
        fl = (with_win(fl, MW_SECOND) & ~(F_IT_MASK << F_IT_SHIFT)) | (amin << F_IT_SHIFT);
    } else {
        if (k <= P.cap) e.n_ref = k; else e.qd = true;
        e.dense_which = 1;
        fl = (fl & ~F_PHASE) | PH_MINSDF;
    }
    P.s.flags[r] = fl;
    return PH_WAIT;
}

__device__ __forceinline__ int minsdf_exact(const Params &P, int64_t r, int round, int &fl, Emit &e) {
    const int ns = P.p.n_steps;
    const float *v = P.s.big + (size_t)r * ns;
    int amin = 0;
    float vmin = v[0];
    for (int i = 1; i < ns; ++i)
        if (v[i] < vmin) {
            vmin = v[i];
            amin = i;
        }
    const float tmin = P.s.t_min[r], tmax = P.s.t_max[r];
    const float dist = fadd(fmul(minsdf_step(P, r, amin), fsub(tmax, tmin)), tmin);
    finish(P, r, dist, fl & F_HIT);
    P.s.flags[r] = (fl & ~F_PHASE) | PH_DONE;
    return PH_WAIT;
}

__global__ __launch_bounds__(256) void advance_kernel(Params P, int round) {
    const int64_t r = (int64_t)blockIdx.x * blockDim.x + threadIdx.x;
    const bool valid = r < P.n;
    if (round > 0 && P.s.block_live[blockIdx.x] == 0) return;
    Emit e = {};
    int fl = 0, fl0 = 0, ph = PH_WAIT;
    if (valid) {
        fl0 = fl = P.s.flags[r];
        ph = fl & F_PHASE;
        if (round == 0) ph = init_ray(P, r, round, fl, e);
        if (ph == PH_TRACE) ph = step_trace(P, r, round, fl, e);
        if (ph == PH_SAMPLER_X) ph = sampler_leading(P, r, round, fl, e);
        if (ph == PH_SAMPLER_C && win_of(fl) >= SW_STAGE1) ph = sampler_staged(P, r, round, fl, e);
    }
    if (P.walk_wave && P.cells) serve_grid_walks(P, r, round, fl, e);
    if (valid) {
        if (ph == PH_SAMPLER_C && win_of(fl) != SW_WHOLE_ROW) ph = sampler_windows(P, r, round, fl, e);
        if (ph == PH_SAMPLER_C) ph = sampler_coarse(P, r, round, fl, e);
        if (ph == PH_SAMPLER) ph = sampler_exact(P, r, round, fl, e);
        if (ph == PH_BISECT) ph = bisect(P, r, round, fl, e);
        if (ph == PH_POST) ph = post(P, r, round, fl, e);
    }
    if (P.share) ph = minsdf_share(P, r, round, ph, fl0, fl, e);
    if (valid) {
        if (ph == PH_MINSDF_C && win_of(fl) == MW_SHARED) ph = minsdf_shared(P, r, round, fl, e);
        if (ph == PH_MINSDF_C && (win_of(fl) == MW_STAGE1 || win_of(fl) == MW_STAGE2)) ph = minsdf_staged(P, r, round, fl, e);
        if (ph == PH_MINSDF_C && win_of(fl) == MW_SECOND) ph = minsdf_second_stage(P, r, round, fl, e);
        if (ph == PH_MINSDF_C) ph = minsdf_coarse(P, r, round, fl, e);
        if (ph == PH_MINSDF) ph = minsdf_exact(P, r, round, fl, e);
    }
    append_queries(P, round, (unsigned)r, e);
    const int alive = __syncthreads_or(valid && (P.s.flags[r] & F_PHASE) != PH_DONE);
    if (threadIdx.x == 0) P.s.block_live[blockIdx.x] = alive;
}

struct RoundWork {
    int n_single;
    int64_t n_sd, n_sdt, total;
};
__device__ __forceinline__ RoundWork round_work(const Params &P, int round) {
    const int *c = P.counters + round * NCNT;
    RoundWork w;
    w.n_single = c[NEFII_CNT_SINGLES];
    w.n_sd = (int64_t)c[NEFII_CNT_SINGLES] + (int64_t)c[NEFII_CNT_DENSE_ROWS] * P.p.n_steps;
    w.n_sdt = w.n_sd + (int64_t)c[NEFII_CNT_BISECT_RAYS] * P.tri_nodes;
    w.total = w.n_sdt + c[NEFII_CNT_REFINED];
    return w;
}

__device__ __forceinline__ float dense_depth(const Params &P, int64_t r, int i, bool minsdf) {
    if (minsdf) {
        const float tmin = P.s.t_min[r], tmax = P.s.t_max[r];
        return fadd(fmul(minsdf_step(P, r, i), fsub(tmax, tmin)), tmin);
    }
    const float a = P.s.t_s[r];
    return fadd(a, fmul(P.lin[i], fsub(P.s.t_e[r], a)));
}

__device__ __forceinline__ float3 ray_point(const Params &P, int64_t r, float t) {
    return make_float3(fadd(P.o[r * 3], fmul(t, P.d[r * 3])), fadd(P.o[r * 3 + 1], fmul(t, P.d[r * 3 + 1])),
                       fadd(P.o[r * 3 + 2], fmul(t, P.d[r * 3 + 2])));
}

__device__ __forceinline__ void put_point(float *raw, int tid, float px, float py, float pz) {
    float *rw = raw + tid * 9;
    rw[0] = px, rw[1] = py, rw[2] = pz;
    rw[3] = rw[4] = rw[5] = rw[6] = rw[7] = rw[8] = 0.f;
}

template <int ROWS>
__device__ __forceinline__ void load_points_tile(const float *__restrict__ x, int64_t n, float *__restrict__ out, int64_t tile,
                                                 float *raw, float **dest, int tid = threadIdx.x) {
    if (tid >= ROWS) return;
    const int64_t q = tile * ROWS + tid;
    float *rw = raw + tid * 9;
    const bool live = q < n;
    rw[0] = live ? x[q * 3] : 0.f, rw[1] = live ? x[q * 3 + 1] : 0.f, rw[2] = live ? x[q * 3 + 2] : 0.f;
    rw[3] = rw[4] = rw[5] = rw[6] = rw[7] = rw[8] = 0.f;
    dest[tid] = live ? out + q : nullptr;
}

template <int ROWS>
__device__ __forceinline__ void decode_tile(const Params &P, int64_t tile, const RoundWork &W, float *raw, float **dest,
                                            float *old = nullptr) {
    const int tid = threadIdx.x;
    if (tid >= ROWS) return;
    const int ns = P.p.n_steps;
    int64_t q = tile * ROWS + tid;
    float *dst = nullptr;
    float px = 0.f, py = 0.f, pz = 0.f;
    float coarse_v = __builtin_nanf("");
    if (q < W.total) {
        int64_t r;
        float t;
        if (q < W.n_single) {
            const unsigned e = P.s.singles[q];
            r = e >> 2;
            const int kind = e & 3;
            t = kind == Q_START ? P.s.t_s[r] : (kind == Q_END ? P.s.t_e[r] : P.s.mid[r]);
            dst = kind == Q_END ? &P.s.res_e[r] : &P.s.res_s[r];
            if (old && P.tier_band > 0.f && (P.s.flags[r] & (kind == Q_END ? F_AUD_E : F_AUD_S))) coarse_v = *dst;
        } else if (q >= W.n_sdt) {
            const unsigned e = P.s.refine[q - W.n_sdt];
            r = e >> 7;
            const int i = e & 127;
            const int ph = P.s.flags[r] & F_PHASE;
            t = dense_depth(P, r, i, ph == PH_MINSDF || ph == PH_MINSDF_C);
            dst = &P.s.big[(size_t)r * ns + i];
            if (old && ph != PH_SAMPLER_X) coarse_v = *dst;
        } else if (q >= W.n_sd) {
            const int64_t qq = q - W.n_sd;
            const int64_t ti = qq / P.tri_nodes;
            const int j = (int)(qq - ti * P.tri_nodes);
            r = P.s.tri[ti];
            t = tri_depth(P.s.lo[r], P.s.hi[r], j);
            dst = &P.s.big[(size_t)r * ns + j];
        } else {
            const int64_t qq = q - W.n_single;
            const int64_t di = qq / ns;
            const int i = (int)(qq - di * ns);
            const unsigned e = P.s.dense[di];
            r = e >> 1;
            t = dense_depth(P, r, i, e & 1);
            dst = &P.s.big[(size_t)r * ns + i];
        }
        const float3 p = ray_point(P, r, t);
        px = p.x, py = p.y, pz = p.z;
    }
    dest[tid] = dst;
    if (old) old[tid] = coarse_v;
    put_point(raw, tid, px, py, pz);
}

__device__ __forceinline__ int64_t coarse_work(const Params &P, int round, int64_t &n_rows) {
    const int *c = P.counters + round * NCNT;
    n_rows = (int64_t)c[NEFII_CNT_COARSE_WINDOWS] * coarse_window(P.p.n_steps);
    return n_rows + c[NEFII_CNT_COARSE_SINGLES] + c[NEFII_CNT_COARSE_SAMPLES];
}

template <int ROWS>
__device__ __forceinline__ void decode_tile_coarse(const Params &P, int round, int64_t tile, int64_t n_rows, int64_t total,
                                                   float *raw, float **dest, int tid = threadIdx.x) {
    if (tid >= ROWS) return;
    const int ns = P.p.n_steps, cw = coarse_window(ns);
    const int64_t q = tile * ROWS + tid;
    float *dst = nullptr;
    float px = 0.f, py = 0.f, pz = 0.f;
    const int64_t di = q / cw;
    const unsigned e = q < n_rows ? P.s.cdense[di] : 0u;
    int i = (int)(e >> 29) * cw + (int)(q - di * cw);
    if (q < n_rows && (e >> 29) == CWIN_STAGE1) {
        const int j = (int)(q - di * cw);
        const int64_t rr = (e & 0x1FFFFFFFu) >> 1;
        i = j >= stage1_count(ns) ? ns : (e & 1) ? P.s.ord[(size_t)minsdf_row(P, rr) * ns + stage1_pos(ns, j)] : stage1_pos(ns, j);
    }
    const int64_t n_cs = P.counters[round * NCNT + NEFII_CNT_COARSE_SINGLES];
    if (q >= n_rows + n_cs && q < total) {
        const unsigned s = P.s.crefine[q - n_rows - n_cs];
        const int64_t r = s >> 7;
        const int si = (int)(s & 127u);
        const float t = dense_depth(P, r, si, (P.s.flags[r] & F_PHASE) == PH_MINSDF_C);
        dst = &P.s.big[(size_t)r * ns + si];
        const float3 p = ray_point(P, r, t);
        px = p.x, py = p.y, pz = p.z;
    } else if (q >= n_rows && q < total) {
        const unsigned s = P.s.csingles[q - n_rows];
        const int64_t r = s >> 2;
        const bool end = (s & 3) == Q_END;
// ... 1098 lines not shown

namespace nefii {
static int vg_grid(int64_t n, int rows) {
    const int64_t n_tiles = (n + rows - 1) / rows;
    return (int)(n_tiles < 256 ? (n_tiles > 0 ? n_tiles : 1) : 256);
}
static bool vg_enabled() {
    static const bool v = env_int("NEFII_VG_STREAM", 1) != 0;
    return v;
}
size_t value_grad_stream_ws_bytes(const nefii_mlp *m, int64_t n) {
    if (!m || n <= 0 || !m->w_stream || !vg_enabled()) return 0;
    const int ft = vg_shape(m);
    if (!ft) return 0;
    const int rows = ft == 4 ? 64 : 96;
    return (size_t)vg_grid(n, rows) * (m->n_layers - 1) * 8 * (ft * rows / 16) * 64 * sizeof(float4v);
}
int value_grad_stream_launch(const nefii_mlp *m, const float *x, int64_t n, float *sdf_out, int out_stride, float *feat_out,
                             int feat_stride, float *grad_out, float *ws, hipStream_t st) {
    const int ft = m->w_stream && vg_enabled() ? vg_shape(m) : 0;
    if (!ft) return NEFII_E_UNSUPPORTED;
    const int Gw = stream_steps(m) + vg_units_bwd(m);
    if (ft == 4)
        hipLaunchKernelGGL((sdf_value_grad16q_kernel<4, 4>), dim3(vg_grid(n, 64)), dim3(512), 0, st, *m, x, n, sdf_out, out_stride,
                           feat_out, feat_stride, grad_out, reinterpret_cast<float4v *>(ws), vg_stream_offset(m), Gw);
    else
        hipLaunchKernelGGL((sdf_value_grad16q_kernel<6, 2>), dim3(vg_grid(n, 96)), dim3(512), 0, st, *m, x, n, sdf_out, out_stride,
                           feat_out, feat_stride, grad_out, reinterpret_cast<float4v *>(ws), vg_stream_offset(m), Gw);
    HIP_CHECK_LAUNCH();
    return 0;
}
}

static unsigned coarse_d_grid() {
    static const int g = env_int("NEFII_COARSE_D_GRID", 0);
    return (unsigned)(g > 0 ? g : 256);
}
static int coarse_two_groups() {
    static const int v = env_int("NEFII_COARSE_D", 0);
    return v;
}
static int coarse_qt() {
    static const int q = env_int("NEFII_COARSE_QT", 0);
    return q == 4 || q == 6 || q == 8 ? q : 0;
}
static int coarse_rows(int ft) {
    const int q = coarse_qt();
    if (ft == 2) return 96;
    return 16 * (q ? q : 4);
}
static dim3 points_grid(int64_t n, int rows) {
    const int64_t n_tiles = (n + rows - 1) / rows;
    return dim3((int)(n_tiles < 512 ? n_tiles : 512));
}
#define NEFII_COARSE_LAUNCH(KERNEL, KERNEL_D, ft, grid, st, ...)                                                    \
    do {                                                                                                            \
        const int rows_ = coarse_rows(ft);                                                                          \
        if ((ft) == 2)                                                                                              \
            hipLaunchKernelGGL((KERNEL<6, 2>), grid, dim3(512), 0, st, __VA_ARGS__);                                \
        else if (rows_ == 64 && coarse_two_groups())                                                                \
            hipLaunchKernelGGL((KERNEL_D<4>), dim3((grid).x < coarse_d_grid() ? (grid).x : coarse_d_grid()), dim3(512), 0, st, \
                               __VA_ARGS__);                                                                    \
        else if (rows_ == 64)                                                                                       \
            hipLaunchKernelGGL((KERNEL<4, 4>), grid, dim3(512), 0, st, __VA_ARGS__);                                \
        else if (rows_ == 96)                                                                                       \
            hipLaunchKernelGGL((KERNEL<6, 4, false>), grid, dim3(512), 0, st, __VA_ARGS__);                         \
        else                                                                                                        \
            hipLaunchKernelGGL((KERNEL<8, 4, false>), grid, dim3(512), 0, st, __VA_ARGS__);                         \
    } while (0)

extern "C" int nefii_sdf_eval_coarse(const nefii_mlp *h_sdf, const float *x, int64_t n, float *sdf_out, void *stream) {
    if (!h_sdf || h_sdf->n_layers < 1 || h_sdf->n_layers > NEFII_MAX_LAYERS) return NEFII_E_ARG;
    if (!nefii_sdf_coarse_supported(h_sdf)) return NEFII_E_UNSUPPORTED;
    if (n <= 0) return 0;
    if (!x || !sdf_out) return NEFII_E_ARG;
    if (!sdf_net_ok(h_sdf)) return NEFII_E_UNSUPPORTED;
    const int ft = shape16p(h_sdf);
    const dim3 grid = points_grid(n, coarse_rows(ft));
    NEFII_COARSE_LAUNCH(sdf_points_kernel16s, sdf_points_kernel16d, ft, grid, (hipStream_t)stream, *h_sdf, x, n, sdf_out);
    HIP_CHECK_LAUNCH();
    return 0;
}

namespace {
constexpr int GRID_SLAB = 8;

__global__ __launch_bounds__(256) void grid_points_kernel(int G, float radius, float h, int i0, int planes, float *__restrict__ x) {
    const int V = G + 1;
    const int64_t n = (int64_t)planes * V * V;
    for (int64_t q = (int64_t)blockIdx.x * blockDim.x + threadIdx.x; q < n; q += (int64_t)gridDim.x * blockDim.x) {
        const int k = (int)(q % V), j = (int)((q / V) % V), i = i0 + (int)(q / ((int64_t)V * V));
        x[q * 3] = fadd(-radius, fmul((float)i, h));
        x[q * 3 + 1] = fadd(-radius, fmul((float)j, h));
        x[q * 3 + 2] = fadd(-radius, fmul((float)k, h));
    }
}

__device__ __forceinline__ unsigned short half_toward(float x, bool up) {
    const _Float16 hv = (_Float16)x;
    unsigned short bits = __builtin_bit_cast(unsigned short, hv);
    const bool wrong = up ? (float)hv < x : (float)hv > x;
    if (wrong) {
        const bool pos = !(bits & 0x8000u);
        if ((bits & 0x7FFFu) == 0)
            bits = up ? 0x0001u : 0x8001u;
        else
            bits = (unsigned short)(pos == up ? bits + 1 : bits - 1);
    }
    return bits;
}

__global__ __launch_bounds__(256) void grid_cells_kernel(int G, float h, float tau, float l_floor, float safety,
                                                         const float *__restrict__ g, unsigned *__restrict__ cells,
                                                         unsigned short *__restrict__ cell_l) {
    const int V = G + 1;
    const int64_t n = (int64_t)G * G * G;
    const float reach = (float)((double)h * 0.8660254037844386);
    for (int64_t c = (int64_t)blockIdx.x * blockDim.x + threadIdx.x; c < n; c += (int64_t)gridDim.x * blockDim.x) {
        const int k = (int)(c % G), j = (int)((c / G) % G), i = (int)(c / ((int64_t)G * G));
        auto at = [&](int a, int b, int d) { return g[((int64_t)a * V + b) * V + d]; };
        float lo = __builtin_inff(), hi = -__builtin_inff();
        float ux = -__builtin_inff(), uy = ux, uz = ux, dx = __builtin_inff(), dy = dx, dz = dx;
        auto edge = [&](float &u, float &d, float next, float here) {
            const float s = __fdiv_rn(fsub(next, here), h);
            u = fmaxf(u, s), d = fminf(d, s);
        };
        for (int a = i - 1; a <= i + 2; ++a)
            for (int b = j - 1; b <= j + 2; ++b)
                for (int d = k - 1; d <= k + 2; ++d) {
                    if (a < 0 || a > G || b < 0 || b > G || d < 0 || d > G) continue;
                    const float v = at(a, b, d);
                    if (a >= i && a <= i + 1 && b >= j && b <= j + 1 && d >= k && d <= k + 1) lo = fminf(lo, v), hi = fmaxf(hi, v);
                    if (a < i + 2 && a < G) edge(ux, dx, at(a + 1, b, d), v);
                    if (b < j + 2 && b < G) edge(uy, dy, at(a, b + 1, d), v);
                    if (d < k + 2 && d < G) edge(uz, dz, at(a, b, d + 1), v);
                }
        const float sx = fmaxf(fabsf(ux), fabsf(dx)), sy = fmaxf(fabsf(uy), fabsf(dy)), sz = fmaxf(fabsf(uz), fabsf(dz));
        const float slope = fmaxf(fmaxf(sx, sy), sz);
        const float lcell = fmaxf(fmul(safety, slope), l_floor);
        const float slack = fadd(tau, fmul(lcell, reach));
        cells[c] = (unsigned)half_toward(fsub(lo, slack), false) | ((unsigned)half_toward(fadd(hi, slack), true) << 16);
        if (cell_l) {
            const float mx = fadd(sx, fsub(ux, dx)), my = fadd(sy, fsub(uy, dy)), mz = fadd(sz, fsub(uz, dz));
            const float norm = sqrtf(fadd(fadd(fmul(mx, mx), fmul(my, my)), fmul(mz, mz)));
            cell_l[c] = half_toward(fmaxf(fmul(safety, norm), l_floor), true);
        }
    }
}

__global__ __launch_bounds__(256) void grid_vertex_half_kernel(int64_t n, const float *__restrict__ g, unsigned short *__restrict__ out) {
    for (int64_t q = (int64_t)blockIdx.x * blockDim.x + threadIdx.x; q < n; q += (int64_t)gridDim.x * blockDim.x)
        out[q] = __builtin_bit_cast(unsigned short, (_Float16)g[q]);
}
}

extern "C" size_t nefii_sdf_bound_grid_workspace_bytes(int G) {
    if (G < 2 || G > NEFII_BOUND_GRID_MAX) return 0;
    const size_t V = (size_t)G + 1;
    return align256(sizeof(float) * V * V * V) + align256(sizeof(float) * 3 * GRID_SLAB * V * V);
}

extern "C" int nefii_sdf_bound_grid_build(const nefii_mlp *h_sdf, int G, float radius, float tau, float L_floor, float safety,
                                          void *out_cells, void *workspace, void *stream) {
    return nefii_sdf_bound_grid_build_vertices(h_sdf, G, radius, tau, L_floor, safety, out_cells, nullptr, nullptr, workspace, stream);
}

extern "C" int nefii_sdf_bound_grid_build_vertices(const nefii_mlp *h_sdf, int G, float radius, float tau, float L_floor,
                                                   float safety, void *out_cells, void *out_vertex_g, void *out_cell_l,
                                                   void *workspace, void *stream) {
    if (!h_sdf || !out_cells || !workspace || h_sdf->n_layers < 1 || h_sdf->n_layers > NEFII_MAX_LAYERS) return NEFII_E_ARG;
    if (!out_vertex_g != !out_cell_l) return NEFII_E_ARG;
    if (!(radius > 0.f && radius < 1e6f) || !(tau >= 0.f && tau < 1e6f) || !(L_floor > 0.f && L_floor < 1e6f) ||
        !(safety > 0.f && safety < 1e6f))
        return NEFII_E_ARG;
    if (G < 2 || G > NEFII_BOUND_GRID_MAX) return NEFII_E_SHAPE;
    if (!nefii_sdf_coarse_supported(h_sdf) || !sdf_net_ok(h_sdf)) return NEFII_E_UNSUPPORTED;
    hipStream_t st = (hipStream_t)stream;
    const int V = G + 1;
    const float h = (float)(2.0 * (double)radius / (double)G);
    float *g = (float *)workspace;
    float *x = (float *)((char *)workspace + align256(sizeof(float) * (size_t)V * V * V));
    const int ft = shape16p(h_sdf);
    for (int i0 = 0; i0 < V; i0 += GRID_SLAB) {
        const int planes = V - i0 < GRID_SLAB ? V - i0 : GRID_SLAB;
        const int64_t n = (int64_t)planes * V * V;
        hipLaunchKernelGGL(grid_points_kernel, dim3((int)((n + 255) / 256 < 1024 ? (n + 255) / 256 : 1024)), dim3(256), 0, st, G,
                           radius, h, i0, planes, x);
        HIP_CHECK_LAUNCH();
        const dim3 grid = points_grid(n, coarse_rows(ft));
        float *out = g + (size_t)i0 * V * V;
        NEFII_COARSE_LAUNCH(sdf_points_kernel16s, sdf_points_kernel16d, ft, grid, st, *h_sdf, (const float *)x, n, out);
        HIP_CHECK_LAUNCH();
    }
    const int64_t n_cells = (int64_t)G * G * G;
    hipLaunchKernelGGL(grid_cells_kernel, dim3((int)((n_cells + 255) / 256 < 4096 ? (n_cells + 255) / 256 : 4096)), dim3(256), 0,
                       st, G, h, tau, L_floor, safety, (const float *)g, (unsigned *)out_cells, (unsigned short *)out_cell_l);
    HIP_CHECK_LAUNCH();
    if (out_vertex_g) {
        const int64_t n_vert = (int64_t)V * V * V;
        hipLaunchKernelGGL(grid_vertex_half_kernel, dim3((int)((n_vert + 255) / 256 < 4096 ? (n_vert + 255) / 256 : 4096)), dim3(256),
                           0, st, n_vert, (const float *)g, (unsigned short *)out_vertex_g);
        HIP_CHECK_LAUNCH();
    }
    return 0;
}

extern "C" int nefii_sdf_eval_fp8corr(const nefii_mlp *h_sdf, const float *x, int64_t n, float *sdf_out, void *stream) {
    if (!h_sdf || !x || !sdf_out || n < 0) return NEFII_E_ARG;
    if (!nefii_sdf_fp8corr_supported(h_sdf)) return NEFII_E_UNSUPPORTED;
    for (int l = 0; l < h_sdf->n_layers; ++l)
        if (!h_sdf->layer[l].w_f16x3) return NEFII_E_ARG;
    if (n == 0) return 0;
    hipLaunchKernelGGL(sdf_points_kernel16f, points_grid(n, 64), dim3(512), 0, (hipStream_t)stream, *h_sdf, x, n, sdf_out,
                       (const void *)((const char *)h_sdf->w_stream + stream_bytes_1to4(h_sdf)));
    HIP_CHECK_LAUNCH();
    return 0;
}

extern "C" int nefii_sdf_eval(const nefii_mlp *h_sdf, const float *x, int64_t n, float *sdf_out, void *stream) {
    if (!h_sdf || h_sdf->n_layers < 1 || h_sdf->n_layers > NEFII_MAX_LAYERS) return NEFII_E_ARG;
    if (n <= 0) return 0;
    if (!x || !sdf_out) return NEFII_E_ARG;
    if (!sdf_net_ok(h_sdf)) return NEFII_E_UNSUPPORTED;
    for (int l = 0; l < h_sdf->n_layers; ++l)
        if (!h_sdf->layer[l].w_f16x3 || !h_sdf->layer[l].bias) return NEFII_E_ARG;
    const dim3 grid = points_grid(n, TILE_W);
    hipStream_t st = (hipStream_t)stream;
    const int ft = fits16p(h_sdf);
    if (ft == 2)
        hipLaunchKernelGGL(sdf_points_kernel16q<2>, grid, dim3(512), 0, st, *h_sdf, x, n, sdf_out);
    else if (ft && h_sdf->reserved == 1)
        hipLaunchKernelGGL(sdf_points_kernel16q<4>, grid, dim3(512), 0, st, *h_sdf, x, n, sdf_out);
    else if (ft)
        hipLaunchKernelGGL(sdf_points_kernel16p<P16W>, grid, dim3(64 * P16W), 0, st, *h_sdf, x, n, sdf_out);
    else
        hipLaunchKernelGGL(sdf_points_kernel16w, grid, dim3(WG_W), 0, st, *h_sdf, x, n, sdf_out);
    HIP_CHECK_LAUNCH();
    return 0;
}

static int coarse_cap(const nefii_tracer_params *p) {
    if (!(p->coarse_tau > 0.f)) return 0;
    const int c = p->coarse_cap <= 0 ? 64 : p->coarse_cap;
    return c > 100 ? 100 : c;
}

static bool minsdf_staged(const nefii_tracer_params *p) {
    return p->coarse_tau > 0.f && p->minsdf_lipschitz > 0.f && p->n_steps >= 16 && p->n_steps <= 128;
}

static int trace_rounds(const nefii_tracer_params *p) {
    const int trace = 1 + p->sphere_tracing_iters * (1 + p->line_step_iters);
    return trace * (p->coarse_tau > 0.f && p->trace_tier ? 2 : 1);
}

static bool minsdf_share_fits(const nefii_tracer_params *p) {
    return nefii_trace_max_rounds(p) - 1 - trace_rounds(p) >= 6;
}

extern "C" int nefii_trace_max_rounds(const nefii_tracer_params *p) {
    if (!p) return 0;
    const int L = p->bisect_levels >= 1 && p->bisect_levels <= 5 ? p->bisect_levels : 3;
    const int trace = 1 + p->sphere_tracing_iters * (1 + p->line_step_iters);
    return trace + 1 + (p->n_rootfind_steps + L - 1) / L + 1 + 2 +
           (p->coarse_tau > 0.f ? 3 + 3 + 1 + (p->trace_tier ? trace : 0) : 0) + (minsdf_staged(p) ? 1 : 0);
}

extern "C" size_t nefii_trace_workspace_bytes(int64_t n_rays, const nefii_tracer_params *p) {
    if (!p || n_rays <= 0) return 0;
    RayState s;
    size_t bytes = carve(s, nullptr, n_rays, p->n_steps, coarse_cap(p), minsdf_staged(p) ? minsdf_rows(n_rays, p) : 0);
    bytes += align256(sizeof(int) * NCNT * (size_t)nefii_trace_max_rounds(p));
    return bytes;
}

struct TraceJob {
    Params P;
    const nefii_mlp *sdf;
    int precision, rounds, adv_blocks, eval_blocks, eval_blocks_w;
    int pipelined;
    int coarse;
    const void *f8;
    hipStream_t st;
    int32_t *counters;
};

int prepare_job(TraceJob &J, const nefii_mlp *h_sdf, const nefii_tracer_params *h_params, const float *origins,
                const float *dirs, const uint8_t *object_mask, int64_t n_rays, const float *lin_steps,
                const float *minsdf_steps, float *out_points, uint8_t *out_hit, float *out_dists, void *workspace,
                size_t workspace_bytes, int32_t *counters, bool reset, void *stream, const void *cells, int grid_n,
                const void *vertex_g, const void *cell_l, int grid_training) {
    if (!h_sdf || !h_params || !origins || !dirs || !object_mask || !lin_steps || !out_points || !out_hit ||
        !out_dists || !workspace)
        return NEFII_E_ARG;
    if (n_rays <= 0 || n_rays >= (1ll << 29)) return NEFII_E_SHAPE;
    if (h_params->training && !minsdf_steps) return NEFII_E_ARG;
    const int levels = h_params->bisect_levels >= 1 && h_params->bisect_levels <= 5 ? h_params->bisect_levels : 3;
    if (h_params->bisect_levels < 0 || h_params->bisect_levels > 5) return NEFII_E_ARG;
    if (h_params->n_steps < (1 << levels) || h_params->sphere_tracing_iters > 250 || h_params->line_step_iters > 15 ||
        h_params->n_rootfind_steps > 250)
        return NEFII_E_SHAPE;
    if (h_params->sphere_tracing_iters < 0 || h_params->line_step_iters < 0 || h_params->n_rootfind_steps < 0)
        return NEFII_E_SHAPE;
    if (!sdf_net_ok(h_sdf)) return NEFII_E_UNSUPPORTED;
    if (workspace_bytes < nefii_trace_workspace_bytes(n_rays, h_params)) return NEFII_E_SHAPE;
    if (h_params->precision < 0 || h_params->precision > 2) return NEFII_E_ARG;
    if (h_params->precision >= 1)
        for (int l = 0; l < h_sdf->n_layers; ++l)
            if (!h_sdf->layer[l].w_f16x3) return NEFII_E_ARG;
    J.sdf = h_sdf;
    J.st = (hipStream_t)stream;
    J.precision = h_params->precision;
    J.rounds = nefii_trace_max_rounds(h_params);
    J.counters = counters;
    Params &P = J.P;
    P.p = *h_params;
    P.n = n_rays;
    P.o = origins;
    P.d = dirs;
    P.obj = object_mask;
    P.lin = lin_steps;
    P.steps = minsdf_steps ? minsdf_steps : lin_steps;
    if (!minsdf_steps) P.p.minsdf_group = 0;
    P.out_pts = out_points;
    P.out_dist = out_dists;
    P.out_hit = out_hit;
    J.pipelined = h_params->precision == 2 ? fits16p(h_sdf) : 0;
    if (h_params->split_fp8 < 0 || h_params->split_fp8 > 1) return NEFII_E_ARG;
    J.f8 = (h_params->split_fp8 && J.pipelined == 4 && nefii_sdf_fp8corr_supported(h_sdf))
               ? (const void *)((const char *)h_sdf->w_stream + stream_bytes_1to4(h_sdf)) : nullptr;
    J.coarse = h_params->coarse_tau > 0.f && J.pipelined && nefii_sdf_coarse_supported(h_sdf) &&
               n_rays < (1ll << 25) && h_params->n_steps <= 128;
    if (h_params->coarse_tau < 0.f || h_params->coarse_tau > 1.f) return NEFII_E_ARG;
    P.tau = J.coarse ? h_params->coarse_tau : 0.f;
    P.cap = coarse_cap(h_params);
    P.chunk = 0;
    P.chunk_gate = 1e30f;
    P.window = 0;
    P.tier_band = 0.f;
    P.tier_gate = 0.f;
    if (h_params->trace_tier < 0 || h_params->trace_tier > 1 || h_params->tier_kappa < 0.f || h_params->tier_gate < 0.f)
        return NEFII_E_ARG;
    if (J.coarse && h_params->trace_tier) {
        const float kappa = h_params->tier_kappa > 0.f ? h_params->tier_kappa : 2.f;
        const float band = kappa * P.tau, least = P.tau + 2.f * fabsf(h_params->sdf_threshold);
        P.tier_band = band > least ? band : least;
        P.tier_gate = (h_params->tier_gate > 0.f ? h_params->tier_gate : 4.f) * P.tau;
    }
    if (J.coarse && h_params->n_steps >= 16) {
        P.window = env_int("NEFII_SAMPLER_WINDOW", 2 | (n_rays >= 32768 ? 1 : 0)) & 3;
    }
    if (J.coarse) {
        const int c = env_int("NEFII_SAMPLER_CHUNK", 6);
        P.chunk = (c >= 2 && c <= 31 && c <= P.cap && c < h_params->n_steps) ? c : 0;
        P.chunk_gate = env_float("NEFII_SAMPLER_CHUNK_GATE", 1.0f);
    }
    if (h_params->minsdf_lipschitz < 0.f || h_params->minsdf_lipschitz > 1e6f) return NEFII_E_ARG;
    const bool staged = J.coarse && minsdf_staged(h_params);
    P.lip = staged ? h_params->minsdf_lipschitz : 0.f;
    P.share = staged && h_params->training && minsdf_share_fits(h_params) && env_int("NEFII_MINSDF_SHARE", 1) != 0;
    static const int stage_bracket = env_int("NEFII_BRACKET_STAGED", 1) != 0;
    P.stage_bracket = stage_bracket;
    if (h_params->unread_misses < 0 || h_params->unread_misses > 1) return NEFII_E_ARG;
    P.miss_argmin = !(h_params->unread_misses && !h_params->training);
    if (cells && (grid_n < 1 || grid_n > NEFII_BOUND_GRID_MAX)) return NEFII_E_SHAPE;
    P.cells = staged ? (const unsigned *)cells : nullptr;
    P.grid_n = grid_n;
    P.grid_inv_h = (float)((double)grid_n / (2.0 * (double)h_params->object_bounding_sphere));
    if (!vertex_g != !cell_l || (vertex_g && !cells)) return NEFII_E_ARG;
    P.vert_g = P.cells ? (const unsigned short *)vertex_g : nullptr;
    P.cell_l = P.cells ? (const unsigned short *)cell_l : nullptr;
    P.grid_training = grid_training;
    P.grid_h = grid_n > 0 ? (float)(2.0 * (double)h_params->object_bounding_sphere / (double)grid_n) : 0.f;
    P.walk_wave = env_int("NEFII_GRID_WALK_WAVE", 1) != 0;
    const int64_t step_rows = minsdf_staged(h_params) ? minsdf_rows(n_rays, &P.p) : 0;
    size_t off = carve(P.s, (char *)workspace, n_rays, h_params->n_steps, P.cap, step_rows);
    P.counters = (int *)((char *)workspace + off);
    P.levels = levels;
    P.tri_nodes = (1 << levels) - 1;
    if (reset) {
        hipError_t e = hipMemsetAsync(P.counters, 0, sizeof(int) * NCNT * J.rounds, J.st);
        if (e != hipSuccess) return (int)e;
        e = hipMemsetAsync(P.s.flags, 0, sizeof(int) * n_rays, J.st);
        if (e != hipSuccess) return (int)e;
        if (staged && h_params->training) {
            hipLaunchKernelGGL(minsdf_order_kernel, dim3((int)minsdf_rows(n_rays, &P.p)), dim3(128), 0, J.st, P);
            HIP_CHECK_LAUNCH();
        }
    }
    J.adv_blocks = (int)((n_rays + 255) / 256);
    const int64_t max_q = n_rays * (int64_t)h_params->n_steps;
    const int64_t max_tiles = (max_q + TILE - 1) / TILE;
    J.eval_blocks = (int)(max_tiles < 1024 ? max_tiles : 1024);
    const int64_t max_tiles_w = (max_q + TILE_W - 1) / TILE_W;
    static const int eval_grid = env_int("NEFII_EVAL_GRID", 0);
    const int grid_cap = eval_grid > 0 ? eval_grid : 2048;
    J.eval_blocks_w = (int)(max_tiles_w < grid_cap ? max_tiles_w : grid_cap);
    return 0;
}

int launch_round(const TraceJob &J, int r, bool profile) {
    hipStream_t st = J.st;
    hipLaunchKernelGGL(advance_kernel, dim3(J.adv_blocks), dim3(256), 0, st, J.P, r);
    HIP_CHECK_LAUNCH();
    if (r + 1 < J.rounds) {
        hipEvent_t e0 = nullptr, e1 = nullptr;
        if (profile) {
            e0 = prof_event();
            e1 = prof_event();
            (void)hipEventRecord(e0, st);
        }
        const int64_t small_tiles = (J.P.n * 2 + 31) / 32 < 256 ? (J.P.n * 2 + 31) / 32 : 256;
        const dim3 big_grid(J.eval_blocks_w), small_grid((int)(small_tiles < 1 ? 1 : small_tiles));
        auto pair = [&](auto big, auto small, int block, const auto &...args) -> int {
            hipLaunchKernelGGL(big, big_grid, dim3(block), 0, st, args...);
            HIP_CHECK_LAUNCH();
            hipLaunchKernelGGL(small, small_grid, dim3(block), 0, st, args...);
            return 0;
        };
        int rc = 0;
        const bool split = J.precision == 2, q_layout = J.sdf->reserved == 1;
        if (split && J.pipelined == 2)
            rc = pair(eval_kernel16q<6, 2>, eval_kernel16q<2, 2>, 512, J.P, *J.sdf, r);
        else if (split && J.pipelined && q_layout && J.f8)
            rc = pair(eval_kernel16f<4>, eval_kernel16f<2>, 512, J.P, *J.sdf, r, J.f8);
        else if (split && J.pipelined && q_layout && J.P.n <= 1024)
            rc = pair(eval_kernel16q<4, 4>, eval_kernel16q<2, 4, true>, 512, J.P, *J.sdf, r);
        else if (split && J.pipelined && q_layout)
            rc = pair(eval_kernel16q<4, 4>, eval_kernel16q<2, 4>, 512, J.P, *J.sdf, r);
        else if (split && J.pipelined)
            rc = pair(eval_kernel16p<P16W, 2>, eval_kernel16p<P16W, 1>, 64 * P16W, J.P, *J.sdf, r);
        else if (split)
            hipLaunchKernelGGL(eval_kernel16w, big_grid, dim3(WG_W), 0, st, J.P, *J.sdf, r);
        else if (J.precision == 1)
            hipLaunchKernelGGL(eval_kernel16, dim3(J.eval_blocks), dim3(WG), 0, st, J.P, *J.sdf, r);
        else
            hipLaunchKernelGGL(eval_kernel, dim3(J.eval_blocks), dim3(WG), 0, st, J.P, *J.sdf, r);
        if (rc) return rc;
        HIP_CHECK_LAUNCH();
        if (J.coarse) {
            const int ft = J.pipelined == 2 ? 2 : 4, rows = coarse_rows(ft);
            const int64_t t = (J.P.n * (int64_t)(4 * coarse_window(J.P.p.n_steps) + 2) + rows - 1) / rows;
            const dim3 grid((int)(t < J.eval_blocks_w ? t : J.eval_blocks_w));
            NEFII_COARSE_LAUNCH(eval_kernel16s, eval_kernel16d, ft, grid, st, J.P, *J.sdf, r);
            HIP_CHECK_LAUNCH();
        }
        if (profile) (void)hipEventRecord(e1, st);
    }
    return 0;
}

int finish_job(const TraceJob &J) {
    if (J.counters) {
        hipError_t e = hipMemcpyAsync(J.counters, J.P.counters, sizeof(int) * NCNT * J.rounds, hipMemcpyDeviceToDevice, J.st);
        if (e != hipSuccess) return (int)e;
    }
    return 0;
}

extern "C" int nefii_trace_rays_rounds_grid_training(const nefii_mlp *h_sdf, const nefii_tracer_params *h_params,
                                                     const float *origins, const float *dirs, const uint8_t *object_mask,
                                                     int64_t n_rays, const float *lin_steps, const float *minsdf_steps,
                                                     float *out_points, uint8_t *out_hit, float *out_dists, void *workspace,
                                                     size_t workspace_bytes, int32_t *counters, int round_begin, int round_end,
                                                     const void *cells, int G, const void *vertex_g, const void *cell_l,
                                                     int grid_training, void *stream) {
    if (grid_training < 0 || grid_training > 1) return NEFII_E_ARG;
    if (n_rays == 0 && h_sdf && h_params) return 0;
    TraceJob J;
    int rc = prepare_job(J, h_sdf, h_params, origins, dirs, object_mask, n_rays, lin_steps, minsdf_steps, out_points,
                         out_hit, out_dists, workspace, workspace_bytes, counters, round_begin == 0, stream, cells, G, vertex_g,
                         cell_l, grid_training);
    if (rc) return rc;
    if (round_end <= 0 || round_end > J.rounds) round_end = J.rounds;
    if (round_begin < 0 || round_begin >= round_end) return NEFII_E_ARG;
    if (g_prof.on) {
        if (!g_prof.t0) {
            (void)hipEventCreate(&g_prof.t0);
            (void)hipEventCreate(&g_prof.t1);
        }
        (void)hipEventRecord(g_prof.t0, J.st);
    }
    for (int r = round_begin; r < round_end; ++r) {
        rc = launch_round(J, r, g_prof.on);
        if (rc) return rc;
    }
    if (g_prof.on) {
        (void)hipEventRecord(g_prof.t1, J.st);
        g_prof.have_span = true;
    }
    return finish_job(J);
}

extern "C" int nefii_trace_rays_rounds_grid_vertices(const nefii_mlp *h_sdf, const nefii_tracer_params *h_params,
                                                     const float *origins, const float *dirs, const uint8_t *object_mask,
                                                     int64_t n_rays, const float *lin_steps, const float *minsdf_steps,
                                                     float *out_points, uint8_t *out_hit, float *out_dists, void *workspace,
                                                     size_t workspace_bytes, int32_t *counters, int round_begin, int round_end,
                                                     const void *cells, int G, const void *vertex_g, const void *cell_l,
                                                     void *stream) {
    return nefii_trace_rays_rounds_grid_training(h_sdf, h_params, origins, dirs, object_mask, n_rays, lin_steps, minsdf_steps,
                                                 out_points, out_hit, out_dists, workspace, workspace_bytes, counters, round_begin,
                                                 round_end, cells, G, vertex_g, cell_l, 0, stream);
}

extern "C" int nefii_trace_rays_rounds_grid(const nefii_mlp *h_sdf, const nefii_tracer_params *h_params,
                                            const float *origins, const float *dirs, const uint8_t *object_mask,
                                            int64_t n_rays, const float *lin_steps, const float *minsdf_steps,
                                            float *out_points, uint8_t *out_hit, float *out_dists, void *workspace,
                                            size_t workspace_bytes, int32_t *counters, int round_begin, int round_end,
                                            const void *cells, int G, void *stream) {
    return nefii_trace_rays_rounds_grid_vertices(h_sdf, h_params, origins, dirs, object_mask, n_rays, lin_steps, minsdf_steps,
                                                 out_points, out_hit, out_dists, workspace, workspace_bytes, counters, round_begin,
                                                 round_end, cells, G, nullptr, nullptr, stream);
}

extern "C" int nefii_trace_rays_rounds(const nefii_mlp *h_sdf, const nefii_tracer_params *h_params,
                                       const float *origins, const float *dirs, const uint8_t *object_mask,
                                       int64_t n_rays, const float *lin_steps, const float *minsdf_steps,
                                       float *out_points, uint8_t *out_hit, float *out_dists, void *workspace,
                                       size_t workspace_bytes, int32_t *counters, int round_begin, int round_end,
                                       void *stream) {
    return nefii_trace_rays_rounds_grid(h_sdf, h_params, origins, dirs, object_mask, n_rays, lin_steps, minsdf_steps, out_points,
                                        out_hit, out_dists, workspace, workspace_bytes, counters, round_begin, round_end, nullptr,
                                        0, stream);
}

extern "C" int nefii_trace_rays_groups_grid_training(const nefii_mlp *h_sdf, const nefii_tracer_params *h_params,
                                                     const float *origins, const float *dirs, const uint8_t *object_mask,
                                                     int n_groups, const int64_t *group_begin, const float *lin_steps,
                                                     const float *minsdf_steps, float *out_points, uint8_t *out_hit,
                                                     float *out_dists, void *const *workspaces, const size_t *workspace_bytes,
                                                     int32_t *counters, int round_begin, int round_end, const void *cells, int G,
                                                     const void *vertex_g, const void *cell_l, int grid_training,
                                                     void *const *streams) {
    if (grid_training < 0 || grid_training > 1) return NEFII_E_ARG;
    if (n_groups < 1 || n_groups > 16 || !group_begin || !workspaces || !workspace_bytes || !streams) return NEFII_E_ARG;
    if (!h_params) return NEFII_E_ARG;
    TraceJob J[16];
    const int rounds = nefii_trace_max_rounds(h_params);
    if (round_end <= 0 || round_end > rounds) round_end = rounds;
    if (round_begin < 0 || round_begin >= round_end) return NEFII_E_ARG;
    for (int g = 0; g < n_groups; ++g) {
        const int64_t lo = group_begin[g], n = group_begin[g + 1] - lo;
        if (lo < 0 || n <= 0) return NEFII_E_ARG;
        int rc = prepare_job(J[g], h_sdf, h_params, origins + 3 * lo, dirs + 3 * lo, object_mask + lo, n, lin_steps,
                             minsdf_steps, out_points + 3 * lo, out_hit + lo, out_dists + lo, workspaces[g],
                             workspace_bytes[g], counters ? counters + (size_t)g * rounds * NCNT : nullptr,
                             round_begin == 0, streams[g], cells, G, vertex_g, cell_l, grid_training);
        if (rc) return rc;
    }
    for (int r = round_begin; r < round_end; ++r)
        for (int g = 0; g < n_groups; ++g) {
            int rc = launch_round(J[g], r, false);
            if (rc) return rc;
        }
    for (int g = 0; g < n_groups; ++g) {
        int rc = finish_job(J[g]);
        if (rc) return rc;
    }
    return 0;
}

extern "C" int nefii_trace_rays_groups_grid_vertices(const nefii_mlp *h_sdf, const nefii_tracer_params *h_params,
                                                     const float *origins, const float *dirs, const uint8_t *object_mask,
                                                     int n_groups, const int64_t *group_begin, const float *lin_steps,
                                                     const float *minsdf_steps, float *out_points, uint8_t *out_hit,
                                                     float *out_dists, void *const *workspaces, const size_t *workspace_bytes,
                                                     int32_t *counters, int round_begin, int round_end, const void *cells, int G,
                                                     const void *vertex_g, const void *cell_l, void *const *streams) {
    return nefii_trace_rays_groups_grid_training(h_sdf, h_params, origins, dirs, object_mask, n_groups, group_begin, lin_steps,
                                                 minsdf_steps, out_points, out_hit, out_dists, workspaces, workspace_bytes,
                                                 counters, round_begin, round_end, cells, G, vertex_g, cell_l, 0, streams);
}

extern "C" int nefii_trace_rays_groups_grid(const nefii_mlp *h_sdf, const nefii_tracer_params *h_params,
                                            const float *origins, const float *dirs, const uint8_t *object_mask,
                                            int n_groups, const int64_t *group_begin, const float *lin_steps,
                                            const float *minsdf_steps, float *out_points, uint8_t *out_hit,
                                            float *out_dists, void *const *workspaces, const size_t *workspace_bytes,
                                            int32_t *counters, int round_begin, int round_end, const void *cells, int G,
                                            void *const *streams) {
    return nefii_trace_rays_groups_grid_vertices(h_sdf, h_params, origins, dirs, object_mask, n_groups, group_begin, lin_steps,
                                                 minsdf_steps, out_points, out_hit, out_dists, workspaces, workspace_bytes,
                                                 counters, round_begin, round_end, cells, G, nullptr, nullptr, streams);
}

extern "C" int nefii_trace_rays_groups(const nefii_mlp *h_sdf, const nefii_tracer_params *h_params,
                                       const float *origins, const float *dirs, const uint8_t *object_mask,
                                       int n_groups, const int64_t *group_begin, const float *lin_steps,
                                       const float *minsdf_steps, float *out_points, uint8_t *out_hit,
                                       float *out_dists, void *const *workspaces, const size_t *workspace_bytes,
                                       int32_t *counters, int round_begin, int round_end, void *const *streams) {
    return nefii_trace_rays_groups_grid(h_sdf, h_params, origins, dirs, object_mask, n_groups, group_begin, lin_steps,
                                        minsdf_steps, out_points, out_hit, out_dists, workspaces, workspace_bytes, counters,
                                        round_begin, round_end, nullptr, 0, streams);
}

extern "C" int nefii_trace_rays(const nefii_mlp *h_sdf, const nefii_tracer_params *h_params, const float *origins,
                                const float *dirs, const uint8_t *object_mask, int64_t n_rays, const float *lin_steps,
                                const float *minsdf_steps, float *out_points, uint8_t *out_hit, float *out_dists,
                                void *workspace, size_t workspace_bytes, int32_t *counters, void *stream) {
    return nefii_trace_rays_rounds(h_sdf, h_params, origins, dirs, object_mask, n_rays, lin_steps, minsdf_steps,
                                   out_points, out_hit, out_dists, workspace, workspace_bytes, counters, 0, 0, stream);
}

__global__ void camera_rays_kernel(const float *__restrict__ uv, const float *__restrict__ pose,
                                   const float *__restrict__ K, int batch, int64_t samples, float *__restrict__ dirs,
                                   float *__restrict__ origins) {
    const int64_t total = (int64_t)batch * samples;
    for (int64_t i = (int64_t)blockIdx.x * blockDim.x + threadIdx.x; i < total; i += (int64_t)gridDim.x * blockDim.x) {
        const int b = (int)(i / samples);
        const float *Kb = K + b * 16, *Pb = pose + b * 16;
        const float fx = Kb[0], sk = Kb[1], cx = Kb[2], fy = Kb[5], cy = Kb[6];
        const float u = uv[i * 2], v = uv[i * 2 + 1];
        const float x = __fdiv_rn(fsub(fadd(fsub(u, cx), __fdiv_rn(fmul(cy, sk), fy)), __fdiv_rn(fmul(sk, v), fy)), fx);
        const float y = __fdiv_rn(fsub(v, cy), fy);
        float w[3];
        for (int c = 0; c < 3; ++c) {
            const float wc = fadd(fadd(fadd(fmul(Pb[c * 4], x), fmul(Pb[c * 4 + 1], y)), Pb[c * 4 + 2]), Pb[c * 4 + 3]);
            w[c] = fsub(wc, Pb[c * 4 + 3]);
        }
        const float nrm = fmaxf(sqrtf(fadd(fadd(fmul(w[0], w[0]), fmul(w[1], w[1])), fmul(w[2], w[2]))), 1e-12f);
        for (int c = 0; c < 3; ++c) {
            dirs[i * 3 + c] = __fdiv_rn(w[c], nrm);
            origins[i * 3 + c] = Pb[c * 4 + 3];
        }
    }
}

extern "C" int nefii_camera_rays(const float *uv, const float *pose, const float *intrinsics, int batch,
                                 int64_t samples, float *out_dirs, float *out_origins, void *stream) {
    if (!uv || !pose || !intrinsics || !out_dirs || !out_origins) return NEFII_E_ARG;
    const int64_t total = (int64_t)batch * samples;
    if (total <= 0) return 0;
    int blocks = (int)((total + 255) / 256 < 2048 ? (total + 255) / 256 : 2048);
    hipLaunchKernelGGL(camera_rays_kernel, dim3(blocks), dim3(256), 0, (hipStream_t)stream, uv, pose, intrinsics, batch,
                       samples, out_dirs, out_origins);
    HIP_CHECK_LAUNCH();
    return 0;
}
```

nefii_amd/model/implicit_differentiable_renderer.py:

```python
import math
import os

import numpy as np
import torch
import torch.nn as nn

from .. import ops
from ..utils import rend_util
from .ray_tracing import RayTracing
from .sample_network import SampleNetwork
from .sg_envmap_material import EnvmapMaterialNetwork
from .sg_render import render_with_sg


def _params_version(module):
    return tuple((p.data_ptr(), p._version) for p in _plist(module))


_plist = ops.param_list


class ImplicitNetwork(nn.Module):

    def __init__(self, feature_vector_size, d_in, d_out, dims, geometric_init=True, bias=1.0, skip_in=(),
                 weight_norm=True, multires=0, use_last_as_f=False):
        super().__init__()
        if use_last_as_f:
            assert feature_vector_size == dims[-1]
        assert d_in == 3
        self.feature_vector_size = feature_vector_size
        self.cfg = dict(d_in=d_in, d_out=d_out, dims=list(dims), skip_in=list(skip_in), multires=multires,
                        use_last_as_f=use_last_as_f)
        self.specs, self.enc = ops.sdf_specs(self.cfg, feature_vector_size)
        self.num_layers = len(self.specs) + 1
        self.skip_in = skip_in
        self.use_last_as_f = use_last_as_f
        self.weight_norm = weight_norm
        d0 = self.specs[0].k_in
        for l, s in enumerate(self.specs):
            lin = nn.Linear(s.k_in, s.n_out)
            if geometric_init:
                if l == len(self.specs) - 1:
                    nn.init.normal_(lin.weight, mean=np.sqrt(np.pi) / np.sqrt(s.k_in), std=0.0001)
                    nn.init.constant_(lin.bias, -bias)
                else:
                    nn.init.constant_(lin.bias, 0.0)
                    nn.init.normal_(lin.weight, 0.0, np.sqrt(2) / np.sqrt(s.n_out))
                    if multires > 0 and l == 0:
                        nn.init.constant_(lin.weight[:, 3:], 0.0)
                    elif multires > 0 and l in skip_in:
                        nn.init.constant_(lin.weight[:, -(d0 - 3):], 0.0)
            if weight_norm:
                lin = nn.utils.weight_norm(lin)
            setattr(self, 'lin' + str(l), lin)
        self._pm = None
        self._pm_version = None
        self._pm_fit = None
        self._tau = None
        self.coarse_audit_max = 0.0
        self.coarse_audit_events = []
        self._lip = None
        self._grid = None

    def coarse_tau(self, radius=1.0):
        pm = self.packed(f16x3=True)
        if self._tau is None or self._tau[0] != self._pm_version or self._tau[1] != radius:
            self._tau = (self._pm_version, radius, ops.calibrate_coarse_tau(pm, radius))
        return self._tau[2]

    def minsdf_lipschitz(self, radius=1.0):
        self.packed(f16x3=True)
        if self._lip is None or self._lip[0] != self._pm_version or self._lip[1] != radius:
            with torch.no_grad():
                self._lip = (self._pm_version, radius, ops.calibrate_lipschitz(self.gradient, _plist(self)[0].device, radius))
        return self._lip[2]

    def bound_grid(self, radius=1.0, G=None, vertices=False):
        pm = self.packed(f16x3=True)
        tau = self.coarse_tau(radius)
        if not tau > 0.0 or not self.minsdf_lipschitz(radius) > 0.0:
            return (None, None) if vertices else None
        G = int(G or ops.BOUND_GRID_SIZE)
        key = (self._pm_version, radius, tau, G)
        if self._grid is None or self._grid[:4] != key or (vertices and self._grid[5] is None):
            built = ops.build_bound_grid(pm, radius, tau, G, vertices=vertices)
            self._grid = key + (built if vertices else (built, None))
        return self._grid[4:6] if vertices else self._grid[4]

    def note_lipschitz_audit(self, violation, lip_used):
        if violation <= 0.0 or lip_used <= 0.0 or self._lip is None or self._lip[0] != self._pm_version or self._lip[2] <= 0.0:
            return
        import warnings
        warnings.warn('staged min-SDF search of the tracer disabled for this network: a depth lay %.3e below the lower bound '
                      'its claimed Lipschitz constant %.3f gives' % (violation, lip_used))
        self._lip = (self._pm_version, self._lip[1], 0.0)
        self._grid = None
        self.coarse_audit_events.append(('lipschitz_disabled', float(violation), float(lip_used)))

    def note_coarse_audit(self, observed, tau_used, radius=1.0):
        self.coarse_audit_max = max(self.coarse_audit_max, float(observed))
        if self._tau is None or self._tau[0] != self._pm_version or self._tau[2] <= 0.0 or tau_used <= 0.0:
            return
        tau = self._tau[2]
        if observed > tau_used:
            import warnings
            warnings.warn('coarse pass of the tracer disabled for this network: a refined sample differed from its '
                          'single-pass value by %.3e, above the claimed bound %.3e' % (observed, tau_used))
            self._tau = (self._pm_version, self._tau[1], 0.0)
            self.coarse_audit_events.append(('disabled', float(observed), float(tau_used)))
        elif observed * 2.0 > tau:
            self._tau = (self._pm_version, self._tau[1], ops.COARSE_TAU_SAFETY * float(observed))
            self.coarse_audit_events.append(('recalibrated', float(observed), float(tau_used)))

    def effective_weights(self):
        ws, bs = [], []
        for l in range(len(self.specs)):
            lin = getattr(self, 'lin' + str(l))
            if self.weight_norm:
                ws.append(torch._weight_norm(lin.weight_v, lin.weight_g, 0))
            else:
                ws.append(lin.weight)
            bs.append(lin.bias)
        return ws, bs

    def packed(self, f16x3=False):
        ver = _params_version(self)
        dev = _plist(self)[0].device
        if self._pm is None or self._pm.device != dev or (f16x3 and not self._pm.f16x3):
            self._pm = ops.PackedMLP(self.specs, ops.ACT_SOFTPLUS100, ops.HEAD_NONE, self.enc, 0, dev, f16x3=f16x3)
            self._pm_version = None
        if self._pm_version != ver:
            with torch.no_grad():
                ws, bs = self.effective_weights()
                self._pm.pack(ws, bs)
            self._pm_version = ver
        return self._pm

    def _check_frozen(self):
        if torch.is_grad_enabled() and any(p.requires_grad for p in _plist(self)):
            raise NotImplementedError(
                'nefii_amd: differentiating through the SDF network (trainable geometry) is outside the Step-2 '
                'hot path; call IDRNetwork.freeze_geometry() as every shipped Step-2 script does')

    def _trainable(self):
        return torch.is_grad_enabled() and any(p.requires_grad for p in _plist(self))

    def forward(self, input, compute_grad=False):
        x = ops._f32(input)
        if self._trainable():
            ws, bs = self.effective_weights()
            pm = ops.PackedMLP(self.specs, ops.ACT_SOFTPLUS100, ops.HEAD_NONE, self.enc, 0, x.device) \
                if self._pm_fit is None or self._pm_fit.device != x.device else self._pm_fit
            self._pm_fit = pm
            if self.use_last_as_f:
                out, hidden = ops.FusedMLPHiddenFn.apply(pm, x.detach(), *ws, *bs)
                return torch.cat([out, hidden], dim=-1)
            return ops.FusedMLPFn.apply(pm, x.detach(), None, None, None, *ws, *bs)
        out, hidden, _ = ops.mlp_forward(self.packed(), x, None, None, None, want_hidden=self.use_last_as_f)
        if self.use_last_as_f:
            out = torch.cat([out, hidden], dim=-1)
        return out

    def gradient(self, x, no_grad=False):
        self._check_frozen()
        _, _, g = ops.sdf_value_grad(self.packed(), ops._f32(x))
        return g.unsqueeze(1)

    def value_feature_gradient(self, x):
        self._check_frozen()
        out, hidden, g = ops.sdf_value_grad(self.packed(), ops._f32(x), want_feat=self.use_last_as_f)
        if self.use_last_as_f:
            feat = hidden
        elif self.feature_vector_size > 0:
            feat = out[:, 1:].contiguous()
        else:
            feat = None
        return out[:, :1], feat, g


class RenderingNetwork(nn.Module):

    def __init__(self, feature_vector_size, mode, d_in, d_out, dims, weight_norm=True, weight_init=False,
                 multires_view=0, multires_xyz=0, normalize_output=True, clip_output=False, clip_method='relu'):
        super().__init__()
        self.feature_vector_size = feature_vector_size
        self.mode = mode
        self.normalize_output = normalize_output
        self.clip_output = clip_output
        self.clip_method = clip_method
        self.weight_norm = weight_norm
        self.cfg = dict(mode=mode, d_in=d_in, d_out=d_out, dims=list(dims), multires_view=multires_view,
                        multires_xyz=multires_xyz, normalize_output=normalize_output, clip_output=clip_output,
                        clip_method=clip_method)
        self.specs, self.enc, self.head = ops.radiance_specs(self.cfg, feature_vector_size)
        self.num_layers = len(self.specs) + 1
        lins = []
        for l, s in enumerate(self.specs):
            lins.append(nn.Linear(s.k_in, s.n_out))
        if weight_init:
            for lin in lins[:-1]:
                nn.init.kaiming_uniform_(lin.weight, mode='fan_in', nonlinearity='relu')
                nn.init.constant_(lin.bias, 0.0)
            nn.init.constant_(lins[-1].bias, 0.0)
            if normalize_output:
                nn.init.xavier_uniform_(lins[-1].weight, gain=nn.init.calculate_gain('tanh'))
            elif clip_method == 'relu':
                nn.init.kaiming_uniform_(lins[-1].weight, mode='fan_in', nonlinearity='relu')
        for l, lin in enumerate(lins):
            if weight_norm:
                lin = nn.utils.weight_norm(lin)
            setattr(self, 'lin' + str(l), lin)
        self._pm = None
        self.outputs_detached = False
        self._packed_for = None

    def packed(self, device):
        half = ops.mlp_precision() if ops.mlp_precision() in ('f16', 'f16x3') else False
        if self._pm is None or self._pm.device != device or self._pm.half != half:
            self._pm = ops.PackedMLP(self.specs, ops.ACT_RELU, self.head, self.enc, self.feature_vector_size, device,
                                     half=half)
        return self._pm

    def _effective_weights(self):
        ws, bs = [], []
        for l in range(len(self.specs)):
            lin = getattr(self, 'lin' + str(l))
            ws.append(torch._weight_norm(lin.weight_v, lin.weight_g, 0) if self.weight_norm else lin.weight)
            bs.append(lin.bias)
        return ws, bs

    def forward(self, points, normals, view_dirs, feature_vectors=None):
        p, n, v = ops._f32(points), ops._f32(normals), ops._f32(view_dirs)
        if self.mode == 'idr':
            a, b, c = p, v, n
        elif self.mode == 'no_view_dir':
            a, b, c = p, n, None
        else:
            a, b, c = p, v, None
        feat = ops._f32(feature_vectors) if self.feature_vector_size > 0 else None
        pm = self.packed(p.device)
# ... 393 lines not shown
```

nefii_amd/model/ray_tracing.py:

```python
import contextlib
import os

import torch
import torch.nn as nn

from .. import ops


class RayTracing(nn.Module):
    def __init__(self, object_bounding_sphere=1.0, sdf_threshold=5.0e-5, line_search_step=0.5, line_step_iters=1,
                 sphere_tracing_iters=10, n_steps=100, n_rootfind_steps=8, trace_tier=None):
        super().__init__()
        self.object_bounding_sphere = object_bounding_sphere
        self.sdf_threshold = sdf_threshold
        self.sphere_tracing_iters = sphere_tracing_iters
        self.line_step_iters = line_step_iters
        self.line_search_step = line_search_step
        self.n_steps = n_steps
        self.n_rootfind_steps = n_rootfind_steps
        self._net = None
        self.precision = os.environ.get('NEFII_TRACER_PRECISION', 'f16x3w')
        self._lin = None
        self.last_counters = None
        self.counter_sum = None
        self.collect_counters = False
        self.minsdf_steps_override = None
        self._calls = 0
        self.bisect_levels = int(os.environ.get('NEFII_BISECT_LEVELS', '0'))
        self.concurrent = False
        self.adaptive_rounds = True
        self._rounds_state = {}
        self.stream_groups = int(os.environ.get('NEFII_TRACER_GROUPS', '0'))
        self.skip_min_sdf_search = False
        self.draw_when_skipped = False
        self.miss_search = True
        self.steps_per_batch = False
        self.deferred_checks = None
        self.coarse = os.environ.get('NEFII_TRACER_COARSE', '1') != '0'
        self.coarse_tau_override = None
        self.coarse_cap = int(os.environ.get('NEFII_TRACER_COARSE_CAP', '0'))
        self.coarse_min_rays = int(os.environ.get('NEFII_COARSE_MIN_RAYS', '1024'))
        env = os.environ.get('NEFII_TRACE_TIER')
        self.trace_tier = (bool(trace_tier) if trace_tier is not None else self.TIER_DEFAULT) if env is None or env == '' \
            else env != '0'
        self.tier_kappa = float(os.environ.get('NEFII_TIER_KAPPA', '0'))
        self.tier_gate = float(os.environ.get('NEFII_TIER_GATE', '0'))
        self.minsdf_staged = os.environ.get('NEFII_MINSDF_STAGED', '1') != '0'
        self.bracket_staged_eval = os.environ.get('NEFII_BRACKET_STAGED_EVAL', '0') == '1'
        self.bound_grid = os.environ.get('NEFII_BOUND_GRID', '1') != '0'
        self.bound_grid_size = int(os.environ.get('NEFII_BOUND_GRID_SIZE', '0'))
        self.bound_grid_vertices = os.environ.get('NEFII_BOUND_GRID_VERTICES', '1') != '0'
        self.bound_grid_training = os.environ.get('NEFII_BOUND_GRID_TRAINING', '1') != '0'
        self.minsdf_lipschitz_override = None
        self.split_fp8 = os.environ.get('NEFII_SPLIT_FP8', '0') == '1'
        self.retraced_calls = 0

    @staticmethod
    def auto_levels(n_rays, concurrent=False):
        if n_rays >= 131072:
            return 1
        if concurrent or n_rays > 16384:
            return 3
        return 5

    @staticmethod
    def small_round_for(n_rays, concurrent):
        env = os.environ.get('NEFII_SMALL_ROUND')
        if env:
            return int(env)
        return 4096 if concurrent and n_rays > 1024 else 0

    TIER_DEFAULT = False

    def tier_for(self, n_rays=None):
        return bool(self.trace_tier)

    @contextlib.contextmanager
    def enqueued_ahead(self, checks):
        self.deferred_checks, self.concurrent = checks, True
        try:
            yield
        finally:
            self.deferred_checks, self.concurrent = None, False

    def bind(self, implicit_network):
        object.__setattr__(self, '_net', implicit_network)

    def _cfg(self):
        return dict(object_bounding_sphere=self.object_bounding_sphere, sdf_threshold=self.sdf_threshold,
                    line_search_step=self.line_search_step, line_step_iters=self.line_step_iters,
                    sphere_tracing_iters=self.sphere_tracing_iters, n_steps=self.n_steps,
                    n_rootfind_steps=self.n_rootfind_steps)

    def _bounds(self, net, n_rays, frozen, training=True):
        tau, lip, audit, grid, verts = 0.0, 0.0, None, None, None
        if self.coarse and self.precision == 'f16x3w' and (n_rays > self.coarse_min_rays or self.tier_for()) and \
                (frozen or self.coarse_tau_override is not None):
            tau = self.coarse_tau_override if self.coarse_tau_override is not None else \
                net.coarse_tau(self.object_bounding_sphere)
            use_grid = (self.bound_grid_training if training else not self.bracket_staged_eval) and self.bound_grid and \
                frozen and self.coarse_tau_override is None and self.minsdf_lipschitz_override is None
            if tau > 0 and self.minsdf_staged and (training or self.bracket_staged_eval or use_grid):
                lip = self.minsdf_lipschitz_override if self.minsdf_lipschitz_override is not None else \
                    net.minsdf_lipschitz(self.object_bounding_sphere)
                if use_grid:
                    if lip > 0 and self.bound_grid_vertices:
                        grid, verts = net.bound_grid(self.object_bounding_sphere, self.bound_grid_size, vertices=True)
                    elif lip > 0:
                        grid = net.bound_grid(self.object_bounding_sphere, self.bound_grid_size)
                    if grid is None and not training:
                        lip = 0.0
            if tau > 0 and (self.coarse_tau_override is None or (lip > 0 and self.minsdf_lipschitz_override is None)):
                radius, used, lip_used = self.object_bounding_sphere, tau, lip
                check_tau, check_lip = self.coarse_tau_override is None, self.minsdf_lipschitz_override is None

                def audit(v, lip_violation=0.0):
                    if check_tau:
                        net.note_coarse_audit(v, used, radius)
                    if check_lip and not v > used:
                        net.note_lipschitz_audit(lip_violation, lip_used)
        return tau, lip, audit, grid, verts

    def forward(self, sdf, cam_loc, object_mask, ray_directions):
        net = sdf if hasattr(sdf, 'packed') else self._net
        if net is None:
            raise RuntimeError('RayTracing: no ImplicitNetwork bound; call ray_tracer.bind(implicit_network) or '
                               'pass the network as `sdf`')
        B, S, _ = ray_directions.shape
        dirs = ops._f32(ray_directions).reshape(-1, 3)
        origins = ops._f32(cam_loc).unsqueeze(1).expand(B, S, 3).reshape(-1, 3).contiguous()
        dev = dirs.device
        if self._lin is None or self._lin.device != dev or self._lin.numel() != self.n_steps:
            self._lin = torch.linspace(0, 1, steps=self.n_steps).to(dev)
        steps = None
        training = self.training and not self.skip_min_sdf_search and self.miss_search
        if self.training and not self.skip_min_sdf_search and not self.miss_search and \
                isinstance(self.minsdf_steps_override, (list, tuple)):
            self._calls += 1
        if self.training and self.skip_min_sdf_search and self.draw_when_skipped and self.miss_search and \
                self.minsdf_steps_override is None:
            for _ in range(B if (self.steps_per_batch and B > 1) else 1):
                torch.empty(self.n_steps).uniform_(0.0, 1.0)
        group = 0
        if training:
            rows = B if (self.steps_per_batch and B > 1) else 1
            drawn = []
            for _ in range(rows):
                if self.minsdf_steps_override is not None:
                    ov = self.minsdf_steps_override
                    if isinstance(ov, (list, tuple)):
                        ov = ov[self._calls % len(ov)]
                        self._calls += 1
                    drawn.append(ov.reshape(-1))
                else:
                    drawn.append(torch.empty(self.n_steps).uniform_(0.0, 1.0))
            steps = drawn[0] if rows == 1 else torch.stack([d.cpu() for d in drawn])
            if steps.device.type == 'cpu' and dev.type == 'cuda':
                steps = steps.contiguous().pin_memory().to(dev, non_blocking=True)
            else:
                steps = steps.to(dev).contiguous()
            group = S if rows > 1 else 0
        n_rays = dirs.shape[0]
        levels = self.bisect_levels or self.auto_levels(n_rays, self.concurrent)
        frozen = not any(p.requires_grad for p in ops.param_list(net))
        state = None
        if self.adaptive_rounds:
            import math
            state = self._rounds_state.setdefault((training, int(math.log2(n_rays + 1))), ops.TraceRounds())
        deferred = self.deferred_checks
        for attempt in range(3):
            seen = len(net.coarse_audit_events)
            tau, lip, audit, grid, verts = self._bounds(net, n_rays, frozen, training)
            params = ops.make_tracer_params(self._cfg(), training, self.precision, levels, coarse_tau=tau,
                                            coarse_cap=self.coarse_cap, minsdf_group=group,
                                            small_round=self.small_round_for(n_rays, self.concurrent),
                                            trace_tier=self.tier_for(), tier_kappa=self.tier_kappa,
                                            tier_gate=self.tier_gate, minsdf_lipschitz=lip,
                                            unread_misses=0 if self.miss_search else 1, split_fp8=self.split_fp8)
            res = ops.trace_rays(net.packed(f16x3=self.precision.startswith('f16x3')), params, origins, dirs,
                                 object_mask.reshape(-1), self._lin, steps, want_counters=self.collect_counters,
                                 rounds_state=state,
                                 groups=1 if group else (self.stream_groups or 1),
                                 deferred=deferred,
                                 audit=audit, bound_grid=grid, bound_vertices=verts,
                                 bound_grid_training=training and grid is not None)
            if deferred is not None or audit is None or not any(
                    kind in ('disabled', 'lipschitz_disabled') for kind, _, _ in net.coarse_audit_events[seen:]):
                break
            self.retraced_calls += 1
        if self.collect_counters:
            self.last_counters = res[3]
            cur = res[3]
            if self.counter_sum is not None and self.counter_sum.shape[0] != cur.shape[0]:
                n = max(self.counter_sum.shape[0], cur.shape[0])
                pad = lambda t: torch.cat([t, t.new_zeros(n - t.shape[0], t.shape[1])]) if t.shape[0] < n else t
                self.counter_sum, cur = pad(self.counter_sum), pad(cur)
            self.counter_sum = cur.clone() if self.counter_sum is None else ops.sum_counters(self.counter_sum, cur)
        return res[0], res[1], res[2]
```

nefii_amd/ops/tracer.py:

```python
import ctypes

import torch

from .. import _lib
from .._lib import TracerParams
from ._call import _f32, _ptr, call
from ._call import nbytes as _nbytes


def algorithmic_evals(counters, n_steps):
    c = counters.long()
    return (c[..., _lib.CNT_SINGLES] + c[..., _lib.CNT_COARSE_SINGLES] - c[..., _lib.CNT_REPEATS]
            + c[..., _lib.CNT_SEARCHES] * n_steps + c[..., _lib.CNT_BISECT_USED])


def executed_evals(counters, n_steps, tri_nodes=None):
    c = counters.long()
    split = c[..., _lib.CNT_SINGLES] + c[..., _lib.CNT_DENSE_ROWS] * n_steps + c[..., _lib.CNT_BISECT_EVALS] + c[..., _lib.CNT_REFINED]
    coarse = (c[..., _lib.CNT_COARSE_WINDOWS] * ((n_steps + 3) // 4) + c[..., _lib.CNT_COARSE_SINGLES]
              + c[..., _lib.CNT_COARSE_SAMPLES])
    return split, coarse


PRECISIONS = {'f32': 0, 'f16x3': 1, 'f16x3w': 2}


def make_tracer_params(cfg, training, precision='f32', bisect_levels=3, coarse_tau=0.0, coarse_cap=0, minsdf_group=0,
                       small_round=0, trace_tier=0, tier_kappa=0.0, tier_gate=0.0, minsdf_lipschitz=0.0, unread_misses=0,
                       split_fp8=0):
    p = TracerParams()
    p.split_fp8 = 1 if split_fp8 else 0
    p.unread_misses = 1 if unread_misses else 0
    p.minsdf_lipschitz = float(minsdf_lipschitz) if coarse_tau > 0.0 else 0.0
    p.trace_tier = 1 if (trace_tier and coarse_tau > 0.0) else 0
    p.tier_kappa = float(tier_kappa)
    p.tier_gate = float(tier_gate)
    p.minsdf_group = int(minsdf_group)
    p.small_round = int(small_round)
    p.precision = PRECISIONS[precision]
    p.bisect_levels = bisect_levels
    p.coarse_tau = float(coarse_tau)
    p.coarse_cap = int(coarse_cap)
    p.object_bounding_sphere = cfg.get('object_bounding_sphere', 1.0)
    p.sdf_threshold = cfg.get('sdf_threshold', 5.0e-5)
    p.line_search_step = cfg.get('line_search_step', 0.5)
    p.line_step_iters = cfg.get('line_step_iters', 1)
    p.sphere_tracing_iters = cfg.get('sphere_tracing_iters', 10)
    p.n_steps = cfg.get('n_steps', 100)
    p.n_rootfind_steps = cfg.get('n_rootfind_steps', 8)
    p.training = 1 if training else 0
    return p


class TraceRounds:

    def __init__(self):
        self.guess = None


_TRACE_STREAMS = {}
_WORK = _lib.CNT_WORK


_SIDE_STREAMS = {}


def side_stream(dev):
    key = torch.device(dev).index if torch.device(dev).index is not None else torch.cuda.current_device()
    st = _SIDE_STREAMS.get(key)
    if st is None:
        st = _SIDE_STREAMS[key] = torch.cuda.Stream(device=key)
    return st


def _trace_streams(dev, n):
    pool = _TRACE_STREAMS.setdefault(dev, [])
    while len(pool) < n:
        pool.append(torch.cuda.Stream(device=dev))
    return pool[:n]


def sum_counters(a, b=None):
    if b is None:
        out = a.sum(dim=0)
        for col in _lib.CNT_MAXIMA:
            out[..., col] = a[..., col].max(dim=0).values
        return out
    out = a + b
    for col in _lib.CNT_MAXIMA:
        out[..., col] = torch.maximum(a[..., col], b[..., col])
    return out


def _lip_audit_of(host_counters):
    col = host_counters[..., _lib.CNT_LIP_AUDIT].contiguous().view(torch.float32)
    return float(col.max()) if col.numel() else 0.0


def _audit_of(host_counters):
    col = host_counters[..., _lib.CNT_TAU_AUDIT].contiguous().view(torch.float32)
    return float(col.max()) if col.numel() else 0.0


def _chunks_with_work(host, guess):
    if guess >= host.shape[1]:
        return []
    return [g for g in range(host.shape[0]) if int(host[g, guess - 1, _WORK].sum()) > 0]


def _next_guess(host):
    busy = torch.nonzero(host[:, :, _WORK].sum(dim=(0, 2))).flatten()
    return (int(busy[-1]) if busy.numel() else 0) + 3


BOUND_GRID_SIZE = 256
BOUND_GRID_L_FLOOR = 1.0
BOUND_GRID_SAFETY = 1.5


def build_bound_grid(pm_sdf, radius, tau, G=BOUND_GRID_SIZE, l_floor=BOUND_GRID_L_FLOOR, safety=BOUND_GRID_SAFETY,
                     vertices=False):
    dev = pm_sdf.device
    cells = torch.empty(G, G, G, device=dev, dtype=torch.int32)
    ws = torch.empty(_nbytes('nefii_sdf_bound_grid_workspace_bytes', G), device=dev, dtype=torch.uint8)
    if not vertices:
        call('nefii_sdf_bound_grid_build', ctypes.byref(pm_sdf.struct), G, float(radius), float(tau), float(l_floor), float(safety),
             _ptr(cells), _ptr(ws))
        return cells
    vert_g = torch.empty(G + 1, G + 1, G + 1, device=dev, dtype=torch.float16)
    cell_l = torch.empty(G, G, G, device=dev, dtype=torch.float16)
    call('nefii_sdf_bound_grid_build_vertices', ctypes.byref(pm_sdf.struct), G, float(radius), float(tau), float(l_floor),
         float(safety), _ptr(cells), _ptr(vert_g), _ptr(cell_l), _ptr(ws))
    return cells, (vert_g, cell_l)


def trace_rays(pm_sdf, params, origins, dirs, object_mask, lin_steps, minsdf_steps=None, want_counters=False,
               rounds_state=None, groups=1, deferred=None, audit=None, keep_workspace=None, bound_grid=None,
               bound_vertices=None, bound_grid_training=False):
    lib = _lib.lib()
    n = origins.shape[0]
    dev = origins.device
    pts = torch.empty(n, 3, device=dev, dtype=torch.float32)
    hit = torch.empty(n, device=dev, dtype=torch.uint8)
    dist = torch.empty(n, device=dev, dtype=torch.float32)
    rounds = lib.nefii_trace_max_rounds(ctypes.byref(params))
    if audit is not None and rounds_state is None and torch.cuda.is_current_stream_capturing():
        audit = None
    need_cnt = want_counters or rounds_state is not None or audit is not None
    groups = max(1, min(int(groups), n // 64)) if n > 0 else 1
    counters = torch.zeros(groups, rounds, _lib.TRACE_COUNTERS, device=dev, dtype=torch.int32) if need_cnt else None
    if n > 0:
        om = object_mask.to(torch.uint8).contiguous()
        per = -(-n // groups)
        per = -(-per // 64) * 64
        bounds = [(g * per, min(n, (g + 1) * per)) for g in range(groups) if g * per < n]
        cur = torch.cuda.current_stream(dev)
        streams = [cur] if len(bounds) == 1 else _trace_streams(dev, len(bounds))
        if len(bounds) > 1:
            start = cur.record_event()
        work = []
        for g, (lo, hi) in enumerate(bounds):
            with torch.cuda.stream(streams[g]):
                if len(bounds) > 1:
                    streams[g].wait_event(start)
                nbytes = lib.nefii_trace_workspace_bytes(hi - lo, ctypes.byref(params))
                work.append((torch.empty(nbytes, device=dev, dtype=torch.uint8), nbytes))

        if keep_workspace is not None:
            keep_workspace.extend((w, lo, hi - lo) for (w, _), (lo, hi) in zip(work, bounds))
        G = len(bounds)
        begin = (ctypes.c_int64 * (G + 1))(*([lo for lo, _ in bounds] + [n]))
        ws_ptrs = (ctypes.c_void_p * G)(*[w.data_ptr() for w, _ in work])
        ws_bytes = (ctypes.c_size_t * G)(*[b for _, b in work])
        st_ptrs = (ctypes.c_void_p * G)(*[st.cuda_stream for st in streams])
        cells, cells_n = (_ptr(bound_grid), bound_grid.shape[0]) if bound_grid is not None else (None, 0)
        vert_g, cell_l = (None, None) if bound_vertices is None else (_ptr(bound_vertices[0]), _ptr(bound_vertices[1]))
        if bound_vertices is not None and (bound_grid is None or bound_vertices[0].shape[0] != cells_n + 1 or
                                           bound_vertices[1].shape[0] != cells_n):
            raise ValueError('bound_vertices: the arrays of build_bound_grid(vertices=True), with their bound_grid')
        in_training = 1 if bound_grid_training else 0

        def run(sel, r0, r1):
            if len(sel) == G and G > 1:
                b_, w_, wb_, s_, c_ = begin, ws_ptrs, ws_bytes, st_ptrs, counters
                call('nefii_trace_rays_groups_grid_training', ctypes.byref(pm_sdf.struct), ctypes.byref(params), _ptr(origins), _ptr(dirs),
                     _ptr(om), G, b_, _ptr(lin_steps), _ptr(minsdf_steps), _ptr(pts), _ptr(hit), _ptr(dist), w_, wb_,
                     _ptr(c_) if c_ is not None else None, r0, r1, cells, cells_n, vert_g, cell_l, in_training, stream=s_)
                return
            for g in sel:
                lo, hi = bounds[g]
                ws, nbytes = work[g]
                call('nefii_trace_rays_rounds_grid_training', ctypes.byref(pm_sdf.struct), ctypes.byref(params), _ptr(origins[lo:hi]),
                     _ptr(dirs[lo:hi]), _ptr(om[lo:hi]), hi - lo, _ptr(lin_steps), _ptr(minsdf_steps), _ptr(pts[lo:hi]),
                     _ptr(hit[lo:hi]), _ptr(dist[lo:hi]), _ptr(ws), nbytes, _ptr(counters[g]) if counters is not None else None,
                     r0, r1, cells, cells_n, vert_g, cell_l, in_training, stream=streams[g].cuda_stream)

        def join():
            for st in streams:
                if st is not cur:
                    cur.wait_event(st.record_event())

        def pinned_counters():
            ahead = torch.empty(counters.shape, dtype=counters.dtype, pin_memory=True)
            return ahead.copy_(counters, non_blocking=True)

        def tell(host):
            if audit is not None:
                audit(_audit_of(host), _lip_audit_of(host))

        everyone = list(range(G))
        if rounds_state is None:
            run(everyone, 0, 0)
            join()
            if audit is not None:
                if deferred is not None:
                    deferred.append(lambda ahead=pinned_counters(): tell(ahead))
                else:
                    tell(counters.cpu())
        else:
            guess = rounds if rounds_state.guess is None else max(2, min(rounds, rounds_state.guess))
            run(everyone, 0, guess)
            join()

            def settle(host, wait):
                again = _chunks_with_work(host, guess)
                if again:
                    run(again, guess, 0)
                    wait()
                    host = counters.cpu()
                rounds_state.guess = _next_guess(host)
                tell(host)
                return again

            def sync_streams():
                for st in streams:
                    st.synchronize()

            if deferred is not None:
                ahead = pinned_counters()
                deferred.append(lambda: (pts, hit.bool(), dist) if settle(ahead, sync_streams) else None)
            else:
                settle(counters.cpu(), join)
    if want_counters:
        return pts, hit.bool(), dist, sum_counters(counters)
    return pts, hit.bool(), dist


def trace_iterations(kept):
    out = []
    for ws, _lo, n in kept:
        stride = (4 * n + 255) // 256 * 256
        begin = _lib.TRACE_WS_FLOAT_ARRAYS * stride
        flags = ws[begin:begin + 4 * n].view(torch.int32)
        out.append((flags >> _lib.TRACE_ITER_SHIFT) & 0xF)
    return torch.cat(out)


def camera_rays(uv, pose, intrinsics):
    B, S, _ = uv.shape
    dirs = torch.empty(B, S, 3, device=uv.device, dtype=torch.float32)
    orig = torch.empty(B, S, 3, device=uv.device, dtype=torch.float32)
    uv_c, pose_c, k_c = _f32(uv), _f32(pose), _f32(intrinsics)
    call('nefii_camera_rays', _ptr(uv_c), _ptr(pose_c), _ptr(k_c), B, S, _ptr(dirs), _ptr(orig))
    return dirs, orig
```

Baseline: 2.217 million rays/s.

## Certify ray crossings and free stretches from coarse bound-grid blocks to skip SDF evals

Builds a 4x-coarsened fp16 min-bound block grid from the SDF bound grid. During training traces, rays whose sphere-tracing chord can be certified through the block grid skip MLP sphere-tracing steps. Rays whose remaining stretch is certified empty of surface finish early, and a hashed ~1/16 subset is probed with one SDF eval to audit the bound. This removes MLP evaluations per ray but adds grid walks, extra per-thread registers and atomics, and relies on the conservative bound plus margin staying correct.

```diff
diff --git a/include/nefii_amd.h b/include/nefii_amd.h
--- a/include/nefii_amd.h
+++ b/include/nefii_amd.h
@@ -235,6 +235,30 @@
                                           const void *vertex_g, const void *cell_l, int grid_training,
                                           void *const *streams);
 
+#define NEFII_BOUND_GRID_BLOCK 4
+#define NEFII_CERTIFY_MARGIN 1e-4f
+#define NEFII_CERTIFY_COUNTS 4
+int nefii_sdf_bound_grid_block_count(int G);
+int nefii_sdf_bound_grid_blocks(const void *cells, int G, void *out_blocks, void *stream);
+int nefii_trace_rays_rounds_grid_certify(const nefii_mlp *h_sdf, const nefii_tracer_params *h_params,
+                                         const float *origins, const float *dirs, const uint8_t *object_mask, int64_t n_rays,
+                                         const float *lin_steps, const float *minsdf_steps,
+                                         float *out_points, uint8_t *out_hit, float *out_dists,
+                                         void *workspace, size_t workspace_bytes, int32_t *counters,
+                                         int round_begin, int round_end, const void *cells, int G,
+                                         const void *vertex_g, const void *cell_l, int grid_training,
+                                         const void *blocks, int certify, int32_t *certify_counts, void *stream);
+int nefii_trace_rays_groups_grid_certify(const nefii_mlp *h_sdf, const nefii_tracer_params *h_params,
+                                         const float *origins, const float *dirs, const uint8_t *object_mask,
+                                         int n_groups, const int64_t *group_begin,
+                                         const float *lin_steps, const float *minsdf_steps,
+                                         float *out_points, uint8_t *out_hit, float *out_dists,
+                                         void *const *workspaces, const size_t *workspace_bytes, int32_t *counters,
+                                         int round_begin, int round_end, const void *cells, int G,
+                                         const void *vertex_g, const void *cell_l, int grid_training,
+                                         const void *blocks, int certify, int32_t *certify_counts,
+                                         void *const *streams);
+
 int nefii_trace_profile_enable(int on);
 int nefii_trace_profile_read(double *h_eval_ms, int *h_n_eval, double *h_span_ms);
 int nefii_trace_profile_launches(float *h_ms, int cap);
diff --git a/nefii_amd/_lib.py b/nefii_amd/_lib.py
--- a/nefii_amd/_lib.py
+++ b/nefii_amd/_lib.py
@@ -147,6 +147,12 @@
                                                   P, ctypes.c_size_t, P, I, I, P, I, P, P, I, P]),
     'nefii_trace_rays_groups_grid_training': (I, [ctypes.POINTER(Mlp), ctypes.POINTER(TracerParams), P, P, P, I, P, P, P, P, P,
                                                   P, P, P, P, I, I, P, I, P, P, I, P]),
+    'nefii_sdf_bound_grid_block_count': (I, [I]),
+    'nefii_sdf_bound_grid_blocks': (I, [P, I, P, P]),
+    'nefii_trace_rays_rounds_grid_certify': (I, [ctypes.POINTER(Mlp), ctypes.POINTER(TracerParams), P, P, P, I64, P, P, P, P, P,
+                                                 P, ctypes.c_size_t, P, I, I, P, I, P, P, I, P, I, P, P]),
+    'nefii_trace_rays_groups_grid_certify': (I, [ctypes.POINTER(Mlp), ctypes.POINTER(TracerParams), P, P, P, I, P, P, P, P, P,
+                                                 P, P, P, P, I, I, P, I, P, P, I, P, I, P, P]),
     'nefii_trace_profile_enable': (I, [I]),
     'nefii_trace_profile_read': (I, [ctypes.POINTER(ctypes.c_double), ctypes.POINTER(I), ctypes.POINTER(ctypes.c_double)]),
     'nefii_trace_profile_launches': (I, [ctypes.POINTER(ctypes.c_float), I]),
diff --git a/nefii_amd/csrc/nefii_tracer.hip b/nefii_amd/csrc/nefii_tracer.hip
--- a/nefii_amd/csrc/nefii_tracer.hip
+++ b/nefii_amd/csrc/nefii_tracer.hip
@@ -37,6 +37,7 @@
 constexpr int F_LIVE_S = 1 << 3, F_LIVE_E = 1 << 4, F_PEND_S = 1 << 5, F_PEND_E = 1 << 6;
 constexpr int F_STEPPED = 1 << 7;
 constexpr int F_SPH = 1 << 8, F_SAMP = 1 << 9, F_HIT = 1 << 10;
+constexpr int F_CERT = F_STEPPED;
 constexpr int F_OWN = 1 << 11;
 constexpr int F_IT_SHIFT = 12, F_IT_MASK = 0xFF;
 constexpr int F_K_SHIFT = TRACE_ITER_SHIFT, F_K_MASK = 0xF;
@@ -92,6 +93,11 @@
     float grid_h;
     int grid_training;
     int walk_wave;
+    const unsigned short *blocks;
+    int block_n;
+    int certify;
+    int certify_free;
+    int *cert_counts;
     RayState s;
 };
 
@@ -266,7 +272,141 @@
 }
 
 
-__device__ __forceinline__ int init_ray(const Params &P, int64_t r, int round, int &fl, Emit &e) {
+__device__ __forceinline__ bool chord_block_step(const Params &P, float ox, float oy, float oz, float dx, float dy, float dz,
+                                                 float a, float b, float off, float stop, float &na, float &nb, int &looks) {
+    const float inf = __builtin_inff();
+    const float rad = P.p.object_bounding_sphere;
+    const float inv_hb = P.grid_inv_h * (1.f / NEFII_BOUND_GRID_BLOCK), hb = P.grid_h * NEFII_BOUND_GRID_BLOCK;
+    const float ext = (float)P.grid_n * (1.f / NEFII_BOUND_GRID_BLOCK);
+    const int gb = P.block_n;
+    const float fx = fmul(fadd(fadd(ox, fmul(a, dx)), rad), inv_hb);
+    const float fy = fmul(fadd(fadd(oy, fmul(a, dy)), rad), inv_hb);
+    const float fz = fmul(fadd(fadd(oz, fmul(a, dz)), rad), inv_hb);
+    if (!(fx >= 0.f && fx < ext && fy >= 0.f && fy < ext && fz >= 0.f && fz < ext)) return false;
+    int ix = (int)fx, iy = (int)fy, iz = (int)fz;
+    const float sx = dx != 0.f ? hb / fabsf(dx) : inf, sy = dy != 0.f ? hb / fabsf(dy) : inf, sz = dz != 0.f ? hb / fabsf(dz) : inf;
+    float tx = dx > 0.f ? ((float)(ix + 1) - fx) * sx : dx < 0.f ? (fx - (float)ix) * sx : inf;
+    float ty = dy > 0.f ? ((float)(iy + 1) - fy) * sy : dy < 0.f ? (fy - (float)iy) * sy : inf;
+    float tz = dz > 0.f ? ((float)(iz + 1) - fz) * sz : dz < 0.f ? (fz - (float)iz) * sz : inf;
+    const int ux = dx > 0.f ? 1 : -1, uy = dy > 0.f ? 1 : -1, uz = dz > 0.f ? 1 : -1;
+    const float len = fsub(b, a);
+    float in = 0.f;
+    na = inf, nb = -inf;
+    for (int n = 0; n < 3 * NEFII_BOUND_GRID_MAX; ++n) {
+        const float lo = (float)__builtin_bit_cast(_Float16, P.blocks[((size_t)ix * gb + (size_t)iy) * gb + (size_t)iz]);
+        ++looks;
+        if (!(lo > stop)) return false;
+        const float s = fsub(lo, off);
+        const float tn = fminf(tx, fminf(ty, tz));
+        na = fminf(na, fadd(fadd(a, in), s));
+        nb = fmaxf(nb, fsub(fadd(a, fminf(tn, len)), s));
+        if (!(tn < len)) return true;
+        in = tn;
+        if (tx == tn) ix += ux, tx += sx;
+        else if (ty == tn) iy += uy, ty += sy;
+        else iz += uz, tz += sz;
+        if ((unsigned)ix >= (unsigned)gb || (unsigned)iy >= (unsigned)gb || (unsigned)iz >= (unsigned)gb) return false;
+    }
+    return false;
+}
+
+__device__ __forceinline__ bool certify_crossing(const Params &P, float ox, float oy, float oz, float dx, float dy, float dz,
+                                                 float t0, float t1, int &looks) {
+    const float off = fadd(P.tau, NEFII_CERTIFY_MARGIN), stop = fadd(P.p.sdf_threshold, off);
+    float a = t0, b = t1;
+    for (int k = 0; k <= P.p.sphere_tracing_iters; ++k) {
+        if (a >= b) return true;
+        if (k == P.p.sphere_tracing_iters) break;
+        float na, nb;
+        if (!chord_block_step(P, ox, oy, oz, dx, dy, dz, a, b, off, stop, na, nb, looks)) break;
+        a = na;
+        b = nb;
+    }
+    return false;
+}
+
+__device__ __forceinline__ bool grid_bounds(const Params &P, int64_t r, float t, float &lo, float &hi);
+
+template <int EDGE>
+__device__ __forceinline__ bool chord_free(const Params &P, float ox, float oy, float oz, float dx, float dy, float dz, float a,
+                                           float b, float stop, int &looks);
+template <int EDGE>
+__device__ __forceinline__ bool box_free(const Params &P, float ox, float oy, float oz, float dx, float dy, float dz, int ix,
+                                         int iy, int iz, float a, float b, float stop, int &looks) {
+    if constexpr (EDGE == 1) {
+        const unsigned w = P.cells[((size_t)ix * P.grid_n + (size_t)iy) * P.grid_n + (size_t)iz];
+        return (float)__builtin_bit_cast(_Float16, (unsigned short)(w & 0xFFFFu)) > stop;
+    } else {
+        const float lo = (float)__builtin_bit_cast(_Float16, P.blocks[((size_t)ix * P.block_n + (size_t)iy) * P.block_n + (size_t)iz]);
+        if (lo > stop) return true;
+        return chord_free<1>(P, ox, oy, oz, dx, dy, dz, a, b, stop, looks);
+    }
+}
+template <int EDGE>
+__device__ __forceinline__ bool chord_free(const Params &P, float ox, float oy, float oz, float dx, float dy, float dz, float a,
+                                           float b, float stop, int &looks) {
+    const float inf = __builtin_inff();
+    const float rad = P.p.object_bounding_sphere;
+    const float inv_h = P.grid_inv_h * (1.f / EDGE), h = P.grid_h * EDGE;
+    const float ext = (float)P.grid_n * (1.f / EDGE);
+    const int g = EDGE == 1 ? P.grid_n : P.block_n;
+    const float fx = fmul(fadd(fadd(ox, fmul(a, dx)), rad), inv_h);
+    const float fy = fmul(fadd(fadd(oy, fmul(a, dy)), rad), inv_h);
+    const float fz = fmul(fadd(fadd(oz, fmul(a, dz)), rad), inv_h);
+    if (!(fx >= 0.f && fx < ext && fy >= 0.f && fy < ext && fz >= 0.f && fz < ext)) return false;
+    int ix = (int)fx, iy = (int)fy, iz = (int)fz;
+    const float sx = dx != 0.f ? h / fabsf(dx) : inf, sy = dy != 0.f ? h / fabsf(dy) : inf, sz = dz != 0.f ? h / fabsf(dz) : inf;
+    float tx = dx > 0.f ? ((float)(ix + 1) - fx) * sx : dx < 0.f ? (fx - (float)ix) * sx : inf;
+    float ty = dy > 0.f ? ((float)(iy + 1) - fy) * sy : dy < 0.f ? (fy - (float)iy) * sy : inf;
+    float tz = dz > 0.f ? ((float)(iz + 1) - fz) * sz : dz < 0.f ? (fz - (float)iz) * sz : inf;
+    const int ux = dx > 0.f ? 1 : -1, uy = dy > 0.f ? 1 : -1, uz = dz > 0.f ? 1 : -1;
+    const float len = fsub(b, a);
+    float in = 0.f;
+    for (int n = 0; n < 3 * NEFII_BOUND_GRID_MAX; ++n) {
+        const float tn = fminf(tx, fminf(ty, tz));
+        ++looks;
+        if (!box_free<EDGE>(P, ox, oy, oz, dx, dy, dz, ix, iy, iz, fadd(a, in), fadd(a, fminf(tn, len)), stop, looks)) return false;
+        if (!(tn < len)) return true;
+        in = tn;
+        if (tx == tn) ix += ux, tx += sx;
+        else if (ty == tn) iy += uy, ty += sy;
+        else iz += uz, tz += sz;
+        if ((unsigned)ix >= (unsigned)g || (unsigned)iy >= (unsigned)g || (unsigned)iz >= (unsigned)g) return false;
+    }
+    return false;
+}
+
+__device__ __forceinline__ bool certify_free_stretch(const Params &P, int64_t r, float t_s, int &looks) {
+    const float stop = fadd(P.p.sdf_threshold, fadd(P.tau, NEFII_CERTIFY_MARGIN));
+    float lo, hi;
+    ++looks;
+    if (!grid_bounds(P, r, t_s, lo, hi) || !(lo > stop)) return false;
+    const float t_max = P.s.t_max[r];
+    if (!(t_s < t_max)) return false;
+    return chord_free<NEFII_BOUND_GRID_BLOCK>(P, P.o[r * 3], P.o[r * 3 + 1], P.o[r * 3 + 2], P.d[r * 3], P.d[r * 3 + 1],
+                                              P.d[r * 3 + 2], t_s, t_max, stop, looks);
+}
+
+constexpr int F_PROBE = 1 << 11;
+__device__ __forceinline__ int end_free(const Params &P, int64_t r, int round, int &fl, Emit &e, float t_s) {
+    const unsigned h0 = ((unsigned)r * 2654435761u) ^ 0x9E3779B1u, h = (h0 ^ (h0 >> 15)) * 0x85EBCA6Bu;
+    if ((h >> 28) == 0u) {
+        const float u = (float)((h >> 4) & 0xFFFFu) * (1.f / 65536.f);
+        P.s.mid[r] = t_s;
+        P.s.t_s[r] = fadd(t_s, fmul(u, fsub(P.s.t_max[r], t_s)));
+        e.qs = e.cs = true;
+        atomicAdd(P.counters + round * NCNT + NEFII_CNT_PROBES, 1);
+        fl = PH_TRACE | F_SPH | F_PROBE;
+        P.s.flags[r] = fl;
+        return PH_WAIT;
+    }
+    finish(P, r, t_s, false);
+    fl = F_SPH | F_CERT | PH_DONE;
+    P.s.flags[r] = fl;
+    return PH_WAIT;
+}
+
+__device__ __forceinline__ int init_ray(const Params &P, int64_t r, int round, int &fl, Emit &e, int &looks) {
     const bool tier = P.tier_band > 0.f;
     const float ox = P.o[r * 3], oy = P.o[r * 3 + 1], oz = P.o[r * 3 + 2];
     const float dx = P.d[r * 3], dy = P.d[r * 3 + 1], dz = P.d[r * 3 + 2];
@@ -291,6 +431,12 @@
     P.s.cur_e[r] = 0.f;
     fl = PH_TRACE;
     if (!sph) return PH_TRACE;
+    if (P.certify && certify_crossing(P, ox, oy, oz, dx, dy, dz, t0, t1, looks)) {
+        fl = F_SPH | F_CERT;
+        P.s.mid[r] = t0;
+        return PH_POST;
+    }
+    if (P.certify_free && certify_free_stretch(P, r, t0, looks)) return end_free(P, r, round, fl, e, t0);
     fl |= F_SPH | F_LIVE_S | F_LIVE_E | F_PEND_S | F_PEND_E;
     e.qs = e.qe = true;
     e.cs = tier && t0 > 0.01f;
@@ -690,8 +836,20 @@
     return PH_WAIT;
 }
 
-__device__ __forceinline__ int step_trace(const Params &P, int64_t r, int round, int &fl, Emit &e) {
+__device__ __forceinline__ int step_trace(const Params &P, int64_t r, int round, int &fl, Emit &e, int &looks) {
     const nefii_tracer_params &tp = P.p;
+    if (P.certify_free && (fl & F_PROBE)) {
+        const float v = P.s.res_s[r];
+        float lo, hi;
+        if (grid_bounds(P, r, P.s.t_s[r], lo, hi)) {
+            const float worst = fmaxf(fsub(fsub(lo, P.tau), v), fsub(v, fadd(hi, P.tau)));
+            if (worst > 0.f) atomicMax(P.counters + round * NCNT + NEFII_CNT_LIP_AUDIT, __float_as_int(worst));
+        }
+        finish(P, r, P.s.mid[r], false);
+        fl = F_SPH | F_CERT | PH_DONE;
+        P.s.flags[r] = fl;
+        return PH_WAIT;
+    }
     const bool tier = P.tier_band > 0.f;
     const float thr = tp.sdf_threshold;
     float t_s = P.s.t_s[r], t_e = P.s.t_e[r];
@@ -747,6 +905,7 @@
         ++it;
         t_s = fadd(t_s, cur_s);
         t_e = fsub(t_e, cur_e);
+        if (P.certify_free && live_s && t_s < t_e && certify_free_stretch(P, r, t_s, looks)) return end_free(P, r, round, fl, e, t_s);
         nxt_s = 0.f;
         nxt_e = 0.f;
         k = 0;
@@ -1265,9 +1424,24 @@
     return PH_WAIT;
 }
 
+__device__ __forceinline__ void certify_audit(const Params &P, int64_t r, int round) {
+    const int ns = P.p.n_steps;
+    const float *v = P.s.big + (size_t)r * ns;
+    const float tmin = P.s.t_min[r], len = fsub(P.s.t_max[r], tmin);
+    float worst = 0.f;
+    for (int i = 0; i < ns; ++i) {
+        if (!(v[i] < __builtin_inff())) continue;
+        float lo, hi;
+        if (!grid_bounds(P, r, fadd(fmul(minsdf_step(P, r, i), len), tmin), lo, hi)) continue;
+        worst = fmaxf(worst, fmaxf(fsub(fsub(lo, P.tau), v[i]), fsub(v[i], fadd(hi, P.tau))));
+    }
+    if (worst > 0.f) atomicMax(P.counters + round * NCNT + NEFII_CNT_LIP_AUDIT, __float_as_int(worst));
+}
+
 __device__ __forceinline__ int minsdf_exact(const Params &P, int64_t r, int round, int &fl, Emit &e) {
     const int ns = P.p.n_steps;
     const float *v = P.s.big + (size_t)r * ns;
+    if ((fl & F_CERT) && P.cells) certify_audit(P, r, round);
     int amin = 0;
     float vmin = v[0];
     for (int i = 1; i < ns; ++i)
@@ -1287,16 +1461,34 @@
     const bool valid = r < P.n;
     if (round > 0 && P.s.block_live[blockIdx.x] == 0) return;
     Emit e = {};
-    int fl = 0, fl0 = 0, ph = PH_WAIT;
+    int fl = 0, fl0 = 0, ph = PH_WAIT, looks = 0;
     if (valid) {
         fl0 = fl = P.s.flags[r];
         ph = fl & F_PHASE;
-        if (round == 0) ph = init_ray(P, r, round, fl, e);
-        if (ph == PH_TRACE) ph = step_trace(P, r, round, fl, e);
+        if (round == 0) ph = init_ray(P, r, round, fl, e, looks);
+        if (ph == PH_TRACE) ph = step_trace(P, r, round, fl, e, looks);
         if (ph == PH_SAMPLER_X) ph = sampler_leading(P, r, round, fl, e);
         if (ph == PH_SAMPLER_C && win_of(fl) >= SW_STAGE1) ph = sampler_staged(P, r, round, fl, e);
     }
     if (P.walk_wave && P.cells) serve_grid_walks(P, r, round, fl, e);
+    if (P.certify_free && P.cert_counts) {
+        const unsigned long long cert = __ballot(valid && ph == PH_WAIT && (((fl & F_CERT) && (fl & F_PHASE) == PH_DONE && (fl0 & F_PHASE) != PH_DONE && !(fl0 & F_PROBE)) || ((fl & F_PROBE) && !(fl0 & F_PROBE))));
+#pragma unroll
+        for (int o = 32; o > 0; o >>= 1) looks += __shfl_xor(looks, o);
+        if ((threadIdx.x & 63) == 0) {
+            if (cert) atomicAdd(P.cert_counts + 2, __popcll(cert));
+            if (looks > 0) atomicAdd(P.cert_counts + 3, looks);
+        }
+    }
+    if (round == 0 && P.certify && P.cert_counts) {
+        const unsigned long long cert = __ballot(valid && ph == PH_POST && (fl & F_CERT));
+#pragma unroll
+        for (int o = 32; o > 0; o >>= 1) looks += __shfl_xor(looks, o);
+        if ((threadIdx.x & 63) == 0) {
+            if (cert) atomicAdd(P.cert_counts, __popcll(cert));
+            if (looks > 0) atomicAdd(P.cert_counts + 1, looks);
+        }
+    }
     if (valid) {
         if (ph == PH_SAMPLER_C && win_of(fl) != SW_WHOLE_ROW) ph = sampler_windows(P, r, round, fl, e);
         if (ph == PH_SAMPLER_C) ph = sampler_coarse(P, r, round, fl, e);
@@ -2701,6 +2893,42 @@
     for (int64_t q = (int64_t)blockIdx.x * blockDim.x + threadIdx.x; q < n; q += (int64_t)gridDim.x * blockDim.x)
         out[q] = __builtin_bit_cast(unsigned short, (_Float16)g[q]);
 }
+
+__global__ __launch_bounds__(256) void grid_blocks_kernel(int G, int gb, const unsigned *__restrict__ cells,
+                                                          unsigned short *__restrict__ blocks) {
+    constexpr int B = NEFII_BOUND_GRID_BLOCK;
+    const int64_t n = (int64_t)gb * gb * gb;
+    auto key = [](unsigned bits) { return (bits & 0x8000u) ? (~bits & 0xFFFFu) : (bits | 0x8000u); };
+    for (int64_t q = (int64_t)blockIdx.x * blockDim.x + threadIdx.x; q < n; q += (int64_t)gridDim.x * blockDim.x) {
+        const int k0 = (int)(q % gb) * B, j0 = (int)((q / gb) % gb) * B, i0 = (int)(q / ((int64_t)gb * gb)) * B;
+        unsigned best = 0xFFFFu;
+        for (int i = i0; i < i0 + B && i < G; ++i)
+            for (int j = j0; j < j0 + B && j < G; ++j)
+                for (int k = k0; k < k0 + B && k < G; ++k) {
+                    unsigned bits = cells[((int64_t)i * G + j) * G + k] & 0xFFFFu;
+                    if ((bits & 0x7FFFu) > 0x7C00u) bits = 0xFC00u;
+                    const unsigned kk = key(bits);
+                    best = kk < best ? kk : best;
+                }
+        blocks[q] = (unsigned short)((best & 0x8000u) ? (best & 0x7FFFu) : (~best & 0xFFFFu));
+    }
+}
+}
+
+extern "C" int nefii_sdf_bound_grid_block_count(int G) {
+    if (G < 2 || G > NEFII_BOUND_GRID_MAX) return 0;
+    return (G + NEFII_BOUND_GRID_BLOCK - 1) / NEFII_BOUND_GRID_BLOCK;
+}
+
+extern "C" int nefii_sdf_bound_grid_blocks(const void *cells, int G, void *out_blocks, void *stream) {
+    if (!cells || !out_blocks) return NEFII_E_ARG;
+    const int gb = nefii_sdf_bound_grid_block_count(G);
+    if (gb == 0) return NEFII_E_SHAPE;
+    const int64_t n = (int64_t)gb * gb * gb;
+    hipLaunchKernelGGL(grid_blocks_kernel, dim3((int)((n + 255) / 256 < 4096 ? (n + 255) / 256 : 4096)), dim3(256), 0,
+                       (hipStream_t)stream, G, gb, (const unsigned *)cells, (unsigned short *)out_blocks);
+    HIP_CHECK_LAUNCH();
+    return 0;
 }
 
 extern "C" size_t nefii_sdf_bound_grid_workspace_bytes(int G) {
@@ -2838,7 +3066,8 @@
                 const float *dirs, const uint8_t *object_mask, int64_t n_rays, const float *lin_steps,
                 const float *minsdf_steps, float *out_points, uint8_t *out_hit, float *out_dists, void *workspace,
                 size_t workspace_bytes, int32_t *counters, bool reset, void *stream, const void *cells, int grid_n,
-                const void *vertex_g, const void *cell_l, int grid_training) {
+                const void *vertex_g, const void *cell_l, int grid_training, const void *blocks, int certify,
+                int32_t *certify_counts) {
     if (!h_sdf || !h_params || !origins || !dirs || !object_mask || !lin_steps || !out_points || !out_hit ||
         !out_dists || !workspace)
         return NEFII_E_ARG;
@@ -2922,6 +3151,12 @@
     P.grid_training = grid_training;
     P.grid_h = grid_n > 0 ? (float)(2.0 * (double)h_params->object_bounding_sphere / (double)grid_n) : 0.f;
     P.walk_wave = env_int("NEFII_GRID_WALK_WAVE", 1) != 0;
+    if (certify && (!cells || !blocks)) return NEFII_E_ARG;
+    P.blocks = P.cells ? (const unsigned short *)blocks : nullptr;
+    P.block_n = nefii_sdf_bound_grid_block_count(grid_n);
+    P.certify = (certify & 1) && P.blocks && P.block_n > 0 && h_params->training;
+    P.certify_free = (certify & 2) && P.blocks && P.block_n > 0 && !h_params->training && h_params->unread_misses;
+    P.cert_counts = (P.certify || P.certify_free) ? certify_counts : nullptr;
     const int64_t step_rows = minsdf_staged(h_params) ? minsdf_rows(n_rays, &P.p) : 0;
     size_t off = carve(P.s, (char *)workspace, n_rays, h_params->n_steps, P.cap, step_rows);
     P.counters = (int *)((char *)workspace + off);
@@ -3007,6 +3242,41 @@
     return 0;
 }
 
+extern "C" int nefii_trace_rays_rounds_grid_certify(const nefii_mlp *h_sdf, const nefii_tracer_params *h_params,
+                                                    const float *origins, const float *dirs, const uint8_t *object_mask,
+                                                    int64_t n_rays, const float *lin_steps, const float *minsdf_steps,
+                                                    float *out_points, uint8_t *out_hit, float *out_dists, void *workspace,
+                                                    size_t workspace_bytes, int32_t *counters, int round_begin, int round_end,
+                                                    const void *cells, int G, const void *vertex_g, const void *cell_l,
+                                                    int grid_training, const void *blocks, int certify,
+                                                    int32_t *certify_counts, void *stream) {
+    if (grid_training < 0 || grid_training > 1 || certify < 0 || certify > 3) return NEFII_E_ARG;
+    if (n_rays == 0 && h_sdf && h_params) return 0;
+    TraceJob J;
+    int rc = prepare_job(J, h_sdf, h_params, origins, dirs, object_mask, n_rays, lin_steps, minsdf_steps, out_points,
+                         out_hit, out_dists, workspace, workspace_bytes, counters, round_begin == 0, stream, cells, G, vertex_g,
+                         cell_l, grid_training, blocks, certify, certify_counts);
+    if (rc) return rc;
+    if (round_end <= 0 || round_end > J.rounds) round_end = J.rounds;
+    if (round_begin < 0 || round_begin >= round_end) return NEFII_E_ARG;
+    if (g_prof.on) {
+        if (!g_prof.t0) {
+            (void)hipEventCreate(&g_prof.t0);
+            (void)hipEventCreate(&g_prof.t1);
+        }
+        (void)hipEventRecord(g_prof.t0, J.st);
+    }
+    for (int r = round_begin; r < round_end; ++r) {
+        rc = launch_round(J, r, g_prof.on);
+        if (rc) return rc;
+    }
+    if (g_prof.on) {
+        (void)hipEventRecord(g_prof.t1, J.st);
+        g_prof.have_span = true;
+    }
+    return finish_job(J);
+}
+
 extern "C" int nefii_trace_rays_rounds_grid_training(const nefii_mlp *h_sdf, const nefii_tracer_params *h_params,
                                                      const float *origins, const float *dirs, const uint8_t *object_mask,
                                                      int64_t n_rays, const float *lin_steps, const float *minsdf_steps,
@@ -3014,31 +3284,9 @@
                                                      size_t workspace_bytes, int32_t *counters, int round_begin, int round_end,
                                                      const void *cells, int G, const void *vertex_g, const void *cell_l,
                                                      int grid_training, void *stream) {
-    if (grid_training < 0 || grid_training > 1) return NEFII_E_ARG;
-    if (n_rays == 0 && h_sdf && h_params) return 0;
-    TraceJob J;
-    int rc = prepare_job(J, h_sdf, h_params, origins, dirs, object_mask, n_rays, lin_steps, minsdf_steps, out_points,
-                         out_hit, out_dists, workspace, workspace_bytes, counters, round_begin == 0, stream, cells, G, vertex_g,
-                         cell_l, grid_training);
-    if (rc) return rc;
-    if (round_end <= 0 || round_end > J.rounds) round_end = J.rounds;
-    if (round_begin < 0 || round_begin >= round_end) return NEFII_E_ARG;
-    if (g_prof.on) {
-        if (!g_prof.t0) {
-            (void)hipEventCreate(&g_prof.t0);
-            (void)hipEventCreate(&g_prof.t1);
-        }
-        (void)hipEventRecord(g_prof.t0, J.st);
-    }
-    for (int r = round_begin; r < round_end; ++r) {
-        rc = launch_round(J, r, g_prof.on);
-        if (rc) return rc;
-    }
-    if (g_prof.on) {
-        (void)hipEventRecord(g_prof.t1, J.st);
-        g_prof.have_span = true;
-    }
-    return finish_job(J);
+    return nefii_trace_rays_rounds_grid_certify(h_sdf, h_params, origins, dirs, object_mask, n_rays, lin_steps, minsdf_steps,
+                                                out_points, out_hit, out_dists, workspace, workspace_bytes, counters, round_begin,
+                                                round_end, cells, G, vertex_g, cell_l, grid_training, nullptr, 0, nullptr, stream);
 }
 
 extern "C" int nefii_trace_rays_rounds_grid_vertices(const nefii_mlp *h_sdf, const nefii_tracer_params *h_params,
@@ -3075,15 +3323,16 @@
                                         0, stream);
 }
 
-extern "C" int nefii_trace_rays_groups_grid_training(const nefii_mlp *h_sdf, const nefii_tracer_params *h_params,
-                                                     const float *origins, const float *dirs, const uint8_t *object_mask,
-                                                     int n_groups, const int64_t *group_begin, const float *lin_steps,
-                                                     const float *minsdf_steps, float *out_points, uint8_t *out_hit,
-                                                     float *out_dists, void *const *workspaces, const size_t *workspace_bytes,
-                                                     int32_t *counters, int round_begin, int round_end, const void *cells, int G,
-                                                     const void *vertex_g, const void *cell_l, int grid_training,
-                                                     void *const *streams) {
-    if (grid_training < 0 || grid_training > 1) return NEFII_E_ARG;
+extern "C" int nefii_trace_rays_groups_grid_certify(const nefii_mlp *h_sdf, const nefii_tracer_params *h_params,
+                                                    const float *origins, const float *dirs, const uint8_t *object_mask,
+                                                    int n_groups, const int64_t *group_begin, const float *lin_steps,
+                                                    const float *minsdf_steps, float *out_points, uint8_t *out_hit,
+                                                    float *out_dists, void *const *workspaces, const size_t *workspace_bytes,
+                                                    int32_t *counters, int round_begin, int round_end, const void *cells, int G,
+                                                    const void *vertex_g, const void *cell_l, int grid_training,
+                                                    const void *blocks, int certify, int32_t *certify_counts,
+                                                    void *const *streams) {
+    if (grid_training < 0 || grid_training > 1 || certify < 0 || certify > 3) return NEFII_E_ARG;
     if (n_groups < 1 || n_groups > 16 || !group_begin || !workspaces || !workspace_bytes || !streams) return NEFII_E_ARG;
     if (!h_params) return NEFII_E_ARG;
     TraceJob J[16];
@@ -3096,7 +3345,8 @@
         int rc = prepare_job(J[g], h_sdf, h_params, origins + 3 * lo, dirs + 3 * lo, object_mask + lo, n, lin_steps,
                              minsdf_steps, out_points + 3 * lo, out_hit + lo, out_dists + lo, workspaces[g],
                              workspace_bytes[g], counters ? counters + (size_t)g * rounds * NCNT : nullptr,
-                             round_begin == 0, streams[g], cells, G, vertex_g, cell_l, grid_training);
+                             round_begin == 0, streams[g], cells, G, vertex_g, cell_l, grid_training, blocks, certify,
+                             certify_counts);
         if (rc) return rc;
     }
     for (int r = round_begin; r < round_end; ++r)
@@ -3109,6 +3359,20 @@
         if (rc) return rc;
     }
     return 0;
+}
+
+extern "C" int nefii_trace_rays_groups_grid_training(const nefii_mlp *h_sdf, const nefii_tracer_params *h_params,
+                                                     const float *origins, const float *dirs, const uint8_t *object_mask,
+                                                     int n_groups, const int64_t *group_begin, const float *lin_steps,
+                                                     const float *minsdf_steps, float *out_points, uint8_t *out_hit,
+                                                     float *out_dists, void *const *workspaces, const size_t *workspace_bytes,
+                                                     int32_t *counters, int round_begin, int round_end, const void *cells, int G,
+                                                     const void *vertex_g, const void *cell_l, int grid_training,
+                                                     void *const *streams) {
+    return nefii_trace_rays_groups_grid_certify(h_sdf, h_params, origins, dirs, object_mask, n_groups, group_begin, lin_steps,
+                                                minsdf_steps, out_points, out_hit, out_dists, workspaces, workspace_bytes,
+                                                counters, round_begin, round_end, cells, G, vertex_g, cell_l, grid_training,
+                                                nullptr, 0, nullptr, streams);
 }
 
 extern "C" int nefii_trace_rays_groups_grid_vertices(const nefii_mlp *h_sdf, const nefii_tracer_params *h_params,
diff --git a/nefii_amd/model/implicit_differentiable_renderer.py b/nefii_amd/model/implicit_differentiable_renderer.py
--- a/nefii_amd/model/implicit_differentiable_renderer.py
+++ b/nefii_amd/model/implicit_differentiable_renderer.py
@@ -61,6 +61,7 @@
         self.coarse_audit_events = []
         self._lip = None
         self._grid = None
+        self._grid_blocks = None
 
     def coarse_tau(self, radius=1.0):
         pm = self.packed(f16x3=True)
@@ -86,6 +87,15 @@
             built = ops.build_bound_grid(pm, radius, tau, G, vertices=vertices)
             self._grid = key + (built if vertices else (built, None))
         return self._grid[4:6] if vertices else self._grid[4]
+
+    def bound_grid_blocks(self, radius=1.0, G=None):
+        if self._grid is None or self._grid[:4] != (self._pm_version, radius, self.coarse_tau(radius), int(G or ops.BOUND_GRID_SIZE)):
+            self._grid_blocks = None
+            return None
+        cells = self._grid[4]
+        if self._grid_blocks is None or self._grid_blocks[0] is not cells:
+            self._grid_blocks = (cells, ops.build_bound_grid_blocks(cells))
+        return self._grid_blocks[1]
 
     def note_lipschitz_audit(self, violation, lip_used):
         if violation <= 0.0 or lip_used <= 0.0 or self._lip is None or self._lip[0] != self._pm_version or self._lip[2] <= 0.0:
diff --git a/nefii_amd/model/ray_tracing.py b/nefii_amd/model/ray_tracing.py
--- a/nefii_amd/model/ray_tracing.py
+++ b/nefii_amd/model/ray_tracing.py
@@ -51,6 +51,9 @@
         self.bound_grid_size = int(os.environ.get('NEFII_BOUND_GRID_SIZE', '0'))
         self.bound_grid_vertices = os.environ.get('NEFII_BOUND_GRID_VERTICES', '1') != '0'
         self.bound_grid_training = os.environ.get('NEFII_BOUND_GRID_TRAINING', '1') != '0'
+        self.bound_grid_certify = True
+        self.bound_grid_certify_eval = False
+        self.certify_counts = None
         self.minsdf_lipschitz_override = None
         self.split_fp8 = os.environ.get('NEFII_SPLIT_FP8', '0') == '1'
         self.retraced_calls = 0
@@ -177,13 +180,24 @@
                                             trace_tier=self.tier_for(), tier_kappa=self.tier_kappa,
                                             tier_gate=self.tier_gate, minsdf_lipschitz=lip,
                                             unread_misses=0 if self.miss_search else 1, split_fp8=self.split_fp8)
+            blocks = None
+            mode = os.environ.get('NEFII_BOUND_GRID_CERTIFY', '1')
+            parts = 0
+            if training and self.bound_grid_certify and mode != '0':
+                parts = 1
+            mode_eval = os.environ.get('NEFII_BOUND_GRID_CERTIFY_EVAL', '1' if self.bound_grid_certify_eval else '0')
+            if not training and not self.miss_search and mode_eval != '0':
+                parts = 2
+            if parts and grid is not None and (not self.collect_counters or mode == '2'):
+                blocks = net.bound_grid_blocks(self.object_bounding_sphere, self.bound_grid_size)
             res = ops.trace_rays(net.packed(f16x3=self.precision.startswith('f16x3')), params, origins, dirs,
                                  object_mask.reshape(-1), self._lin, steps, want_counters=self.collect_counters,
                                  rounds_state=state,
                                  groups=1 if group else (self.stream_groups or 1),
                                  deferred=deferred,
                                  audit=audit, bound_grid=grid, bound_vertices=verts,
-                                 bound_grid_training=training and grid is not None)
+                                 bound_grid_training=training and grid is not None, bound_grid_certify=blocks,
+                                 certify_counts=self.certify_counts, certify_parts=parts)
             if deferred is not None or audit is None or not any(
                     kind in ('disabled', 'lipschitz_disabled') for kind, _, _ in net.coarse_audit_events[seen:]):
                 break
diff --git a/nefii_amd/ops/tracer.py b/nefii_amd/ops/tracer.py
--- a/nefii_amd/ops/tracer.py
+++ b/nefii_amd/ops/tracer.py
@@ -134,9 +134,23 @@
     return cells, (vert_g, cell_l)
 
 
+BOUND_GRID_BLOCK = 4
+CERTIFY_COUNTS = 4
+
+
+def build_bound_grid_blocks(cells):
+    G = cells.shape[0]
+    gb = _lib.lib().nefii_sdf_bound_grid_block_count(G)
+    if gb <= 0 or tuple(cells.shape) != (G, G, G) or cells.dtype != torch.int32:
+        raise ValueError('build_bound_grid_blocks: cells must be build_bound_grid\'s int32 [G, G, G]')
+    blocks = torch.empty(gb, gb, gb, device=cells.device, dtype=torch.float16)
+    call('nefii_sdf_bound_grid_blocks', _ptr(cells), G, _ptr(blocks))
+    return blocks
+
+
 def trace_rays(pm_sdf, params, origins, dirs, object_mask, lin_steps, minsdf_steps=None, want_counters=False,
                rounds_state=None, groups=1, deferred=None, audit=None, keep_workspace=None, bound_grid=None,
-               bound_vertices=None, bound_grid_training=False):
+               bound_vertices=None, bound_grid_training=False, bound_grid_certify=None, certify_counts=None, certify_parts=3):
     lib = _lib.lib()
     n = origins.shape[0]
     dev = origins.device
@@ -179,21 +193,27 @@
                                            bound_vertices[1].shape[0] != cells_n):
             raise ValueError('bound_vertices: the arrays of build_bound_grid(vertices=True), with their bound_grid')
         in_training = 1 if bound_grid_training else 0
+        blocks, certify = (_ptr(bound_grid_certify), int(certify_parts) & 3) if bound_grid_certify is not None else (None, 0)
+        if certify and (bound_grid is None or bound_grid_certify.shape[0] != -(-cells_n // BOUND_GRID_BLOCK)):
+            raise ValueError('bound_grid_certify: the tensor of build_bound_grid_blocks(bound_grid), with its bound_grid')
+        cert_cnt = _ptr(certify_counts) if certify else None
 
         def run(sel, r0, r1):
             if len(sel) == G and G > 1:
                 b_, w_, wb_, s_, c_ = begin, ws_ptrs, ws_bytes, st_ptrs, counters
-                call('nefii_trace_rays_groups_grid_training', ctypes.byref(pm_sdf.struct), ctypes.byref(params), _ptr(origins), _ptr(dirs),
+                call('nefii_trace_rays_groups_grid_certify', ctypes.byref(pm_sdf.struct), ctypes.byref(params), _ptr(origins), _ptr(dirs),
                      _ptr(om), G, b_, _ptr(lin_steps), _ptr(minsdf_steps), _ptr(pts), _ptr(hit), _ptr(dist), w_, wb_,
-                     _ptr(c_) if c_ is not None else None, r0, r1, cells, cells_n, vert_g, cell_l, in_training, stream=s_)
+                     _ptr(c_) if c_ is not None else None, r0, r1, cells, cells_n, vert_g, cell_l, in_training, blocks,
+                     certify, cert_cnt, stream=s_)
                 return
             for g in sel:
                 lo, hi = bounds[g]
                 ws, nbytes = work[g]
-                call('nefii_trace_rays_rounds_grid_training', ctypes.byref(pm_sdf.struct), ctypes.byref(params), _ptr(origins[lo:hi]),
+                call('nefii_trace_rays_rounds_grid_certify', ctypes.byref(pm_sdf.struct), ctypes.byref(params), _ptr(origins[lo:hi]),
                      _ptr(dirs[lo:hi]), _ptr(om[lo:hi]), hi - lo, _ptr(lin_steps), _ptr(minsdf_steps), _ptr(pts[lo:hi]),
                      _ptr(hit[lo:hi]), _ptr(dist[lo:hi]), _ptr(ws), nbytes, _ptr(counters[g]) if counters is not None else None,
-                     r0, r1, cells, cells_n, vert_g, cell_l, in_training, stream=streams[g].cuda_stream)
+                     r0, r1, cells, cells_n, vert_g, cell_l, in_training, blocks, certify, cert_cnt,
+                     stream=streams[g].cuda_stream)
 
         def join():
             for st in streams:
```

After: 2.258 million rays/s (median of 6 runs). 1.02x the previous value.
